# princeton-nlp/DensePhrases

Hardware: NVIDIA H100
Metric: queries/sec top-10 over PQ96 phrase index (higher is better)
Workload: dtype f32

## Files before the change

### densephrases_b200/_lib.py

```python
import ctypes as C
import os

_HERE = os.path.dirname(os.path.abspath(__file__))
LIB_PATH = os.path.join(_HERE, "lib", "libdph_b200.so")
_lib = None

MEM_HOST, MEM_DEVICE = 0, 1
SCAN_FAST, SCAN_EXACT, SCAN_PAIR, SCAN_SINGLE, SCAN_QUAD = 0, 1, 2, 3, 4

_vp, _i64, _i32, _u64, _f32 = C.c_void_p, C.c_int64, C.c_int, C.c_uint64, C.c_float
_SIGS = {
    "dph_last_error": (C.c_char_p, []),
    "dph_version": (_i32, []),
    "dph_index_create": (_i32, [C.POINTER(_vp), _i32, _i64, _i32, _i32, _i32]),
    "dph_index_free": (None, [_vp]),
    "dph_index_set_stream": (_i32, [_vp, _vp]),
    "dph_index_set_opq": (_i32, [_vp, _vp, _i32]),
    "dph_index_set_centroids": (_i32, [_vp, _vp, _i32]),
    "dph_index_set_pq": (_i32, [_vp, _vp, _i32]),
    "dph_index_gen_centroids": (_i32, [_vp, _u64, _f32]),
    "dph_index_gen_pq": (_i32, [_vp, _u64, _f32]),
    "dph_index_set_shard": (_i32, [_vp, _i64, _i64]),
    "dph_index_set_lists": (_i32, [_vp, _vp, _vp, _vp]),
    "dph_index_set_lists_synthetic": (_i32, [_vp, _vp, _u64]),
    "dph_index_ntotal": (_i64, [_vp]),
    "dph_index_ntotal_local": (_i64, [_vp]),
    "dph_index_d": (_i32, [_vp]),
    "dph_index_nlist": (_i64, [_vp]),
    "dph_index_nprobe": (_i32, [_vp]),
    "dph_index_set_nprobe": (_i32, [_vp, _i32]),
    "dph_index_set_scan_mode": (_i32, [_vp, _i32]),
    "dph_index_set_coarse_tc": (_i32, [_vp, _i32]),
    "dph_index_get_opq": (_i32, [_vp, _vp, _i32]),
    "dph_index_device_bytes": (_i64, [_vp]),
    "dph_index_set_profile": (_i32, [_vp, _i32]),
    "dph_index_last_scan_ms": (_i32, [_vp, C.POINTER(C.c_float)]),
    "dph_index_profile_scan_ms": (_i32, [_vp, _vp, _i32]),
    "dph_index_profile_count": (_i32, [_vp]),
    "dph_index_search": (_i32, [_vp, _vp, _i64, _i32, _vp, _vp, _i32]),
    "dph_index_search_partial": (_i32, [_vp, _vp, _i64, _i32, _vp, _vp, _vp]),
    "dph_index_coarse_local": (_i32, [_vp, _vp, _i64, _vp]),
    "dph_index_search_preassigned": (_i32, [_vp, _vp, _i32, _i64, _i32, _vp, _vp, _vp]),
    "dph_index_record_floats": (_i32, [_vp]),
    "dph_index_coarse_split": (_i32, [_vp, _vp, _i64, _vp]),
    "dph_index_search_assigned": (_i32, [_vp, _vp, _i64, _i32, _vp, _vp, _vp]),
    "dph_merge_shards": (_i32, [_vp, _vp, _vp, _i32, _i64, _i32, _vp, _vp, _vp]),
    "dph_pack_topk": (_i32, [_vp, _vp, _vp, _i64, _i32, _vp, _vp]),
    "dph_merge_shards_packed": (_i32, [_vp, _i32, _i64, _i32, _vp, _vp, _vp]),
    "dph_index_last_flags": (_vp, [_vp]),
    "dph_index_last_probes": (_vp, [_vp]),
    "dph_index_last_coarse": (_vp, [_vp]),
    "dph_index_last_xr": (_vp, [_vp]),
    "dph_index_last_used_pair_mode": (_i32, [_vp]),
    "dph_index_last_group_size": (_i32, [_vp]),
    "dph_index_copy_last": (_i32, [_vp, _i32, _vp, _i64]),
    "dph_index_reconstruct_batch": (_i32, [_vp, _vp, _i64, _vp, _vp, _i32]),
    "dph_encoder_create": (_i32, [C.POINTER(_vp), _i32, _i32, _i32, _i32]),
    "dph_encoder_free": (None, [_vp]),
    "dph_encoder_set_stream": (_i32, [_vp, _vp]),
    "dph_encoder_tower_floats": (_i64, [_vp]),
    "dph_encoder_load_tower": (_i32, [_vp, _i32, _vp, _i32]),
    "dph_encoder_embed_query": (_i32, [_vp, _vp, _vp, _vp, _i32, _i32, _vp, _vp, _i32]),
    "dph_sgemm_nt_seq": (_i32, [_vp, _i64, _vp, _i64, _i64, _vp, _vp]),
    "dph_gemm_tf32_nt": (_i32, [_vp, _vp, _vp, _vp, _vp, _i64, _i64, _i64, _i32, _i32, _vp]),
    "dph_encoder_set_precision": (_i32, [_vp, _i32]),
    "dph_gemm_tf32_set_mode": (_i32, [_i32]),
    "dph_set_tuning": (_i32, [_i32, _i32]),
    "dph_encoder_set_attention": (_i32, [_vp, _i32]),
    "dph_attention_bert": (_i32, [_vp, _vp, _i32, _i32, _vp, _i32, _vp]),
    "dph_index_window_scores": (_i32, [_vp, _vp, _vp, _i64, _i32, _vp, _i32]),
    "dph_index_encode": (_i32, [_vp, _vp, _i64, _vp, _vp, _i32]),
    "dph_index_add_with_ids": (_i32, [_vp, _vp, _i64, _vp, _i32]),
    "dph_index_copy_lists": (_i32, [_vp, _vp, _vp]),
    "dph_index_get_list_len": (_i32, [_vp, _vp]),
    "dph_index_last_add_ms": (_i32, [_vp, _vp]),
    "dph_index_remove_ids": (_i32, [_vp, _vp, _i64, _i64, _i64, _i32, _vp, _vp]),
    "dph_index_sync_list_len": (_i32, [_vp, _vp]),
    "dph_index_last_remove_ms": (_i32, [_vp, _vp]),
    "dph_index_last_remove_tmp_bytes": (_i64, [_vp]),
    "dph_index_train_coarse": (_i32, [_vp, _vp, _i64, _i32, _u64, _i64, _i32, _i32, _vp, _vp]),
    "dph_index_train_pq": (_i32, [_vp, _vp, _i64, _i32, _u64, _i64, _i32, _i32, _i32]),
    "dph_index_encode_pq": (_i32, [_vp, _vp, _i64, _vp, _i32]),
    "dph_index_get_centroids": (_i32, [_vp, _vp, _i32]),
    "dph_index_get_pq": (_i32, [_vp, _vp, _i32]),
    "dph_index_last_train_ms": (_i32, [_vp, _vp]),
}
EXPORTS = tuple(_SIGS)


def lib():
    global _lib
    if _lib is None:
        if not os.path.exists(LIB_PATH):
            raise RuntimeError(f"{LIB_PATH} not built: run `make` (or __graft_entry__.build()). There is no CPU fallback.")
        L = C.CDLL(LIB_PATH)
        for name, (res, args) in _SIGS.items():
            fn = getattr(L, name)
            fn.restype, fn.argtypes = res, args
        _lib = L
    return _lib


def check(rc):
    if rc != 0:
        raise RuntimeError("libdph_b200: " + lib().dph_last_error().decode())
```

### densephrases_b200/csrc/common.cuh

```cuda
#pragma once
#include <cuda_runtime.h>
#include <stdint.h>
#include <stdio.h>
#include <string>

#define DPH_D 768
#define DPH_M 96
#define DPH_KSUB 256
#define DPH_DSUB 8
#define DPH_CODE 96
#define DPH_BLK_VECS 32
#define DPH_BLK_BYTES 3072
#define DPH_NEUTRAL (-3.402823466e+38f)

#define DPH_API extern "C" __attribute__((visibility("default")))
void dph_set_error(const std::string& msg);

#define DPH_CUDA(call)                                                                              \
    do {                                                                                            \
        cudaError_t e__ = (call);                                                                   \
        if (e__ != cudaSuccess) {                                                                   \
            dph_set_error(std::string(#call) + ": " + cudaGetErrorString(e__) + " @" + __FILE__ + ":" + \
                          std::to_string(__LINE__));                                                \
            return 1;                                                                               \
        }                                                                                           \
    } while (0)
#define DPH_CHECK(cond, msg)                                                        \
    do {                                                                            \
        if (!(cond)) { dph_set_error(std::string(msg) + " (" #cond ")"); return 1; } \
    } while (0)
#define DPH_TRY(call)            \
    do {                         \
        int r__ = (call);        \
        if (r__) return r__;     \
    } while (0)

struct DphPerDeviceOnce {
    bool done[64] = {};
    bool first() {
        int d = 0;
        cudaGetDevice(&d);
        d &= 63;
        if (done[d]) return false;
        done[d] = true;
        return true;
    }
};

__device__ __forceinline__ float2 dph_ffma2(float2 a, float2 b, float2 c) { return make_float2(fmaf(a.x, b.x, c.x), fmaf(a.y, b.y, c.y)); }
__device__ __forceinline__ float2 dph_fadd2(float2 a, float2 b) { return make_float2(__fadd_rn(a.x, b.x), __fadd_rn(a.y, b.y)); }

__host__ __device__ __forceinline__ uint64_t dph_mix64(uint64_t x) {
    x += 0x9E3779B97F4A7C15ull;
    x = (x ^ (x >> 30)) * 0xBF58476D1CE4E5B9ull;
    x = (x ^ (x >> 27)) * 0x94D049BB133111EBull;
    return x ^ (x >> 31);
}
__host__ __device__ __forceinline__ uint64_t dph_rnd64(uint64_t seed, uint64_t stream, uint64_t a, uint64_t b) {
    return dph_mix64(dph_mix64(dph_mix64(seed ^ (stream * 0xA24BAED4963EE407ull)) + a) + b);
}
__host__ __device__ __forceinline__ float dph_approx_normal(uint64_t u, float sigma_over_std) {
    int32_t s = (int32_t)(u & 0xFFFF) + (int32_t)((u >> 16) & 0xFFFF) + (int32_t)((u >> 32) & 0xFFFF) + (int32_t)(u >> 48) - 131070;
    return (float)s * sigma_over_std;
}
#define DPH_IH4_STD 37837.227f
enum { DPH_STREAM_CODES = 1, DPH_STREAM_CENTROIDS = 2, DPH_STREAM_PQ = 3 };

__host__ __device__ __forceinline__ uint32_t dph_fkey(float f) {
    uint32_t b;
#ifdef __CUDA_ARCH__
    b = __float_as_uint(f);
#else
    memcpy(&b, &f, 4);
#endif
    return (b & 0x80000000u) ? ~b : (b | 0x80000000u);
}
__host__ __device__ __forceinline__ float dph_fkey_inv(uint32_t k) {
    uint32_t b = (k & 0x80000000u) ? (k & 0x7FFFFFFFu) : ~k;
#ifdef __CUDA_ARCH__
    return __uint_as_float(b);
#else
    float f; memcpy(&f, &b, 4); return f;
#endif
}
__host__ __device__ __forceinline__ uint64_t dph_ckey(float score, uint32_t gidx) {
    return ((uint64_t)dph_fkey(score) << 32) | (uint64_t)(0xFFFFFFFFu - gidx);
}
__host__ __device__ __forceinline__ float dph_ckey_score(uint64_t k) { return dph_fkey_inv((uint32_t)(k >> 32)); }
__host__ __device__ __forceinline__ uint32_t dph_ckey_gidx(uint64_t k) { return 0xFFFFFFFFu - (uint32_t)k; }

__host__ __device__ __forceinline__ int dph_blk_addr(int lane, int m) {
    int seg = m >> 5, s = ((m & 31) - lane) & 31;
    int t = seg * 32 + s;
    return (t >> 4) * 512 + lane * 16 + (t & 15);
}

struct __align__(16) DphSeg {
    long long blk;
    int len;
    unsigned gstart;
    float dis0;
    unsigned wrel;
    unsigned wend;
    int list;
};

struct DphWork {
    long long total_blocks;
};
struct DphPairWork {
    long long total_blocks;
    long long per;
    int total_units;
    int next_unit;
};
#define DPH_QUAD_ITEM_Q 8
struct __align__(16) DphUnit {
    long long blk;
    int len;
    unsigned bi0, bend;
    int nq;
    int list, pad;
    unsigned q[DPH_QUAD_ITEM_Q];
    unsigned gs[DPH_QUAD_ITEM_Q];
    float base[DPH_QUAD_ITEM_Q];
    float step[DPH_QUAD_ITEM_Q];
};
#define DPH_PAIR_SEG_MIN 128
#define DPH_PAIR_UNITS_PER_CTA 16
```

### densephrases_b200/csrc/index.cu

```cuda
#include "index_internal.cuh"
#include <algorithm>
#include <numeric>
#include <stdlib.h>
#include <string.h>
#include <thrust/device_ptr.h>
#include <thrust/execution_policy.h>
#include <thrust/sequence.h>
#include <thrust/sort.h>

static thread_local std::string g_err;
void dph_set_error(const std::string& msg) { g_err = msg; }
DPH_API const char* dph_last_error(void) { return g_err.c_str(); }
DPH_API int dph_version(void) { return 103; }
int g_dph_tune[8] = {1, 0, 0, 0, 0, 0, 0, 0};
DPH_API int dph_set_tuning(int knob, int value) {
    DPH_CHECK(knob >= 0 && knob < 8, "dph_set_tuning: unknown knob");
    g_dph_tune[knob] = value;
    return 0;
}

int DevBuf::ensure(size_t bytes) {
    if (bytes <= cap) return 0;
    if (p) cudaFree(p);
    p = nullptr; cap = 0;
    size_t want = bytes + bytes / 8 + 256;
    DPH_CUDA(cudaMalloc(&p, want));
    cap = want;
    return 0;
}
void DevBuf::release() { if (p) cudaFree(p); p = nullptr; cap = 0; }

template <class T> static int dev_alloc(T** out, size_t count, dph_index* ix) {
    if (*out) { cudaFree(*out); *out = nullptr; }
    size_t bytes = std::max<size_t>(count, 1) * sizeof(T);
    DPH_CUDA(cudaMalloc((void**)out, bytes));
    ix->bytes += (int64_t)bytes;
    return 0;
}

__global__ void gen_normal_kernel(float* out, long long rows, int cols, uint64_t seed, uint64_t stream, float sc) {
    long long i = (long long)blockIdx.x * blockDim.x + threadIdx.x;
    if (i >= rows * cols) return;
    long long r = i / cols; int t = (int)(i % cols);
    out[i] = dph_approx_normal(dph_rnd64(seed, stream, (uint64_t)r, (uint64_t)t), sc);
}

int64_t dph_chunk_rows() {
    int64_t chunk_rows = (256ll << 20) / DPH_CODE;
    if (const char* ev = getenv("DPH_UPLOAD_CHUNK_ROWS")) chunk_rows = std::max<int64_t>(1, atoll(ev));
    return chunk_rows;
}

__global__ void __launch_bounds__(192) fill_blocks_kernel(uint8_t* codes, long long nblocks, const long long* blk_off, const int* list_len,
                                                          long long list_lo, long long list_hi, const uint8_t* raw,
                                                          const long long* local_row_start, uint64_t seed, long long blk0, long long raw_row0) {
    const long long blk = blk0 + blockIdx.x;
    if (blk >= nblocks) return;
    const int lane = threadIdx.x & 31, c = threadIdx.x >> 5;
    __shared__ long long s_l;
    if (threadIdx.x == 0) s_l = list_of_block(blk_off, list_lo, list_hi, blk);
    __syncthreads();
    const long long l = s_l;
    const long long j = (blk - blk_off[l]) * 32 + lane;
    const bool valid = j < (long long)list_len[l];
    const int seg = c >> 1;
    unsigned char bytes[16];
    if (!valid) {
#pragma unroll
        for (int b = 0; b < 16; b++) bytes[b] = 0;
    } else if (raw) {
        const uint8_t* row = raw + (local_row_start[l - list_lo] + j - raw_row0) * DPH_CODE;
#pragma unroll
        for (int b = 0; b < 16; b++) { int t = c * 16 + b; int m = seg * 32 + ((lane + (t & 31)) & 31); bytes[b] = row[m]; }
    } else {
        uint64_t w[4];
#pragma unroll
        for (int i = 0; i < 4; i++) w[i] = dph_rnd64(seed, DPH_STREAM_CODES, (uint64_t)l, (uint64_t)(j * 12 + seg * 4 + i));
#pragma unroll
        for (int b = 0; b < 16; b++) {
            int t = c * 16 + b; int ml = (lane + (t & 31)) & 31;
            bytes[b] = (unsigned char)(w[ml >> 3] >> (8 * (ml & 7)));
        }
    }
    uint4 v;
    memcpy(&v, bytes, 16);
    *reinterpret_cast<uint4*>(codes + blk * DPH_BLK_BYTES + c * 512 + lane * 16) = v;
}

__global__ void fill_ids_kernel(long long* ids, long long nblocks, const long long* blk_off, const int* list_len, long long list_lo,
                                long long list_hi, const long long* raw_ids, const long long* local_row_start, long long blk0, long long raw_row0,
                                long long* dm_ids, long long* dm_rows) {
    const long long blk = blk0 + blockIdx.x;
    if (blk >= nblocks) return;
    const long long l = list_of_block(blk_off, list_lo, list_hi, blk);
    const long long j = (blk - blk_off[l]) * 32 + threadIdx.x;
    const bool real = j < (long long)list_len[l];
    const long long row = local_row_start[l - list_lo] + j;
    const long long id = real ? raw_ids[row - raw_row0] : -1;
    ids[blk * 32 + threadIdx.x] = id;
    if (real) { dm_ids[row] = id; dm_rows[row] = blk * 32 + threadIdx.x; }
}

DPH_API int dph_index_create(dph_index** out, int d, int64_t nlist, int M, int nbits, int device) {
    DPH_CHECK(out != nullptr, "null out");
    DPH_CHECK(d == DPH_D && M == DPH_M && nbits == 8, "only d=768, M=96, nbits=8 (OPQ96/PQ96 of build_phrase_index.py:113-116) is built");
    DPH_CHECK(nlist >= 1 && nlist < (1ll << 31), "bad nlist");
    DPH_CUDA(cudaSetDevice(device));
    dph_index* ix = new dph_index();
    ix->device = device; ix->nlist = nlist; ix->list_lo = 0; ix->list_hi = nlist;
    cudaDeviceProp prop;
    DPH_CUDA(cudaGetDeviceProperties(&prop, device));
    ix->num_sms = prop.multiProcessorCount;
    if (prop.major != 9 || prop.minor != 0) { delete ix; dph_set_error("libdph_b200 is built for sm_90a (H100) only; found sm_" + std::to_string(prop.major) + std::to_string(prop.minor)); return 1; }
    *out = ix;
    return 0;
}
DPH_API void dph_index_free(dph_index* ix) {
    if (!ix) return;
    cudaSetDevice(ix->device);
    void* ptrs[] = {ix->A, ix->C, ix->pq, ix->list_len, ix->list_start, ix->blk_off, ix->codes, ix->ids, ix->dm_ids, ix->dm_rows};
    for (void* p : ptrs) if (p) cudaFree(p);
    DevBuf* bufs[] = {&ix->xdev, &ix->xr, &ix->S, &ix->key, &ix->cd, &ix->lut_canon, &ix->lutmax, &ix->segs, &ix->wpre, &ix->qinfo,
                      &ix->cand, &ix->cand_off, &ix->cand_cnt, &ix->gthr, &ix->flags, &ix->work, &ix->Dp, &ix->Ip, &ix->Gp, &ix->Dh, &ix->Ih, &ix->eps, &ix->nseg, &ix->lutmin, &ix->lutmaxv, &ix->lutq, &ix->qparams, &ix->gdense,
                      &ix->pl_cnt, &ix->pl_fill, &ix->pl_off, &ix->pl_blockpre, &ix->pl_entries, &ix->pl_unitpre, &ix->pl_units, &ix->pl_udesc, &ix->pairwork, &ix->csplit, &ix->xsplit, &ix->candkeys, &ix->cflags, &ix->selkeys, &ix->recbuf,
                      &ix->rb_ids, &ix->rb_out, &ix->rb_found, &ix->ws_q, &ix->ws_id, &ix->ws_out, &ix->ws_xq, &ix->enc_key, &ix->enc_cd,
                      &ix->enc_list, &ix->enc_codes};
    for (DevBuf* b : bufs) b->release();
    for (int i = 0; i < DPH_PROF_RING; i++) { if (ix->ev0[i]) cudaEventDestroy(ix->ev0[i]); if (ix->ev1[i]) cudaEventDestroy(ix->ev1[i]); }
    for (cudaEvent_t e : ix->aev) if (e) cudaEventDestroy(e);
    delete ix;
}
DPH_API int dph_index_set_stream(dph_index* ix, void* s) { ix->stream = (cudaStream_t)s; return 0; }

static int upload(float** dst, const float* src, size_t count, int mem, dph_index* ix) {
    DPH_CUDA(cudaSetDevice(ix->device));
    DPH_TRY(dev_alloc(dst, count, ix));
    DPH_CUDA(cudaMemcpyAsync(*dst, src, count * sizeof(float), mem == DPH_MEM_HOST ? cudaMemcpyHostToDevice : cudaMemcpyDeviceToDevice, ix->stream));
    DPH_CUDA(cudaStreamSynchronize(ix->stream));
    return 0;
}
DPH_API int dph_index_set_opq(dph_index* ix, const float* A, int mem) { return upload(&ix->A, A, (size_t)ix->d * ix->d, mem, ix); }
DPH_API int dph_index_set_centroids(dph_index* ix, const float* C, int mem) { ix->csplit_lo = -1; return upload(&ix->C, C, (size_t)ix->nlist * ix->d, mem, ix); }
DPH_API int dph_index_set_pq(dph_index* ix, const float* pq, int mem) { return upload(&ix->pq, pq, (size_t)DPH_M * 256 * DPH_DSUB, mem, ix); }

DPH_API int dph_index_gen_centroids(dph_index* ix, uint64_t seed, float sigma) {
    DPH_CUDA(cudaSetDevice(ix->device));
    ix->csplit_lo = -1;
    DPH_TRY(dev_alloc(&ix->C, (size_t)ix->nlist * ix->d, ix));
    long long tot = (long long)ix->nlist * ix->d;
    gen_normal_kernel<<<(unsigned)((tot + 255) / 256), 256, 0, ix->stream>>>(ix->C, ix->nlist, ix->d, seed, DPH_STREAM_CENTROIDS, sigma / DPH_IH4_STD);
    DPH_CUDA(cudaGetLastError());
    return 0;
}
DPH_API int dph_index_gen_pq(dph_index* ix, uint64_t seed, float sigma) {
    DPH_CUDA(cudaSetDevice(ix->device));
    DPH_TRY(dev_alloc(&ix->pq, (size_t)DPH_M * 256 * DPH_DSUB, ix));
    long long rows = DPH_M * 256;
    gen_normal_kernel<<<(unsigned)((rows * DPH_DSUB + 255) / 256), 256, 0, ix->stream>>>(ix->pq, rows, DPH_DSUB, seed, DPH_STREAM_PQ, sigma / DPH_IH4_STD);
    DPH_CUDA(cudaGetLastError());
    return 0;
}
DPH_API int dph_index_set_shard(dph_index* ix, int64_t lo, int64_t hi) {
    DPH_CHECK(0 <= lo && lo <= hi && hi <= ix->nlist, "bad shard range");
    DPH_CHECK(ix->codes == nullptr, "set_shard must precede set_lists");
    ix->list_lo = lo; ix->list_hi = hi;
    return 0;
}

static int set_lists_common(dph_index* ix, const int64_t* list_len, const uint8_t* codes, const int64_t* ids, bool synthetic, uint64_t seed) {
    DPH_CUDA(cudaSetDevice(ix->device));
    const int64_t nlist = ix->nlist, lo = ix->list_lo, hi = ix->list_hi;
    ix->h_list_len.assign(list_len, list_len + nlist);
    ix->h_list_start.assign(nlist + 1, 0);
    for (int64_t l = 0; l < nlist; l++) {
        DPH_CHECK(list_len[l] >= 0 && list_len[l] < (1ll << 31), "bad list length");
        ix->h_list_start[l + 1] = ix->h_list_start[l] + list_len[l];
    }
    ix->ntotal = ix->h_list_start[nlist];
    std::vector<int32_t> len32(nlist);
    std::vector<int64_t> blk_off(nlist, -1), local_row_start(std::max<int64_t>(hi - lo, 1), 0);
    int64_t nb = 0, rows = 0;
    for (int64_t l = 0; l < nlist; l++) len32[l] = (int32_t)list_len[l];
    for (int64_t l = lo; l < hi; l++) {
        blk_off[l] = nb; local_row_start[l - lo] = rows;
        nb += (list_len[l] + 31) / 32; rows += list_len[l];
    }
    ix->nblocks_local = nb; ix->ntotal_local = rows; ix->blk_cap = -1;
    DPH_TRY(dev_alloc(&ix->list_len, (size_t)nlist, ix));
    DPH_TRY(dev_alloc(&ix->list_start, (size_t)nlist + 1, ix));
    DPH_TRY(dev_alloc(&ix->blk_off, (size_t)nlist, ix));
    DPH_CUDA(cudaMemcpy(ix->list_len, len32.data(), nlist * 4, cudaMemcpyHostToDevice));
    DPH_CUDA(cudaMemcpy(ix->list_start, ix->h_list_start.data(), (nlist + 1) * 8, cudaMemcpyHostToDevice));
    DPH_CUDA(cudaMemcpy(ix->blk_off, blk_off.data(), nlist * 8, cudaMemcpyHostToDevice));
    DPH_TRY(dev_alloc(&ix->codes, (size_t)nb * DPH_BLK_BYTES, ix));
    if (nb == 0) return 0;
    int64_t* d_lrs = nullptr;
    DPH_CUDA(cudaMalloc((void**)&d_lrs, local_row_start.size() * 8));
    DPH_CUDA(cudaMemcpy(d_lrs, local_row_start.data(), local_row_start.size() * 8, cudaMemcpyHostToDevice));
    if (synthetic) {
        for (int64_t b0 = 0; b0 < nb; b0 += (1ll << 30)) {
            const unsigned g = (unsigned)std::min<int64_t>(nb - b0, 1ll << 30);
            fill_blocks_kernel<<<g, 192, 0, ix->stream>>>(ix->codes, std::min<int64_t>(nb, b0 + g), (const long long*)ix->blk_off, ix->list_len, lo, hi, nullptr,
                                                         (const long long*)d_lrs, seed, b0, 0);
        }
        DPH_CUDA(cudaGetLastError());
    } else {
        DPH_CHECK(codes != nullptr, "codes is null");
        const int64_t chunk_rows = dph_chunk_rows();
        auto chunk_end = [&](int64_t l0, int64_t& acc) {
            int64_t l1 = l0;
            acc = 0;
            while (l1 < hi && (acc == 0 || acc + list_len[l1] <= chunk_rows)) { acc += list_len[l1]; l1++; }
            return l1;
        };
        int64_t max_rows = 0;
        for (int64_t l0 = lo, acc = 0; l0 < hi;) { const int64_t l1 = chunk_end(l0, acc); max_rows = std::max(max_rows, acc); l0 = l1; }
        uint8_t* d_raw = nullptr; int64_t* d_rawids = nullptr;
        DPH_CUDA(cudaMalloc((void**)&d_raw, std::max<size_t>((size_t)max_rows * DPH_CODE, 1)));
        if (ids) {
            DPH_CUDA(cudaMalloc((void**)&d_rawids, std::max<size_t>((size_t)max_rows * 8, 8)));
            DPH_TRY(dev_alloc(&ix->ids, (size_t)nb * 32, ix));
            DPH_TRY(dev_alloc(&ix->dm_ids, (size_t)rows, ix));
            DPH_TRY(dev_alloc(&ix->dm_rows, (size_t)rows, ix));
        }
        int64_t l0 = lo;
        while (l0 < hi) {
            int64_t acc = 0;
            const int64_t l1 = chunk_end(l0, acc);
            const int64_t r0 = local_row_start[l0 - lo];
            const int64_t b0 = blk_off[l0], b1 = (l1 < hi) ? blk_off[l1] : nb;
            if (acc > 0 && b1 > b0) {
                DPH_CUDA(cudaMemcpyAsync(d_raw, codes + (size_t)r0 * DPH_CODE, (size_t)acc * DPH_CODE, cudaMemcpyHostToDevice, ix->stream));
                fill_blocks_kernel<<<(unsigned)(b1 - b0), 192, 0, ix->stream>>>(ix->codes, b1, (const long long*)ix->blk_off, ix->list_len, lo, hi, d_raw,
                                                                                 (const long long*)d_lrs, 0, b0, r0);
                if (ids) {
                    DPH_CUDA(cudaMemcpyAsync(d_rawids, ids + r0, (size_t)acc * 8, cudaMemcpyHostToDevice, ix->stream));
                    fill_ids_kernel<<<(unsigned)(b1 - b0), 32, 0, ix->stream>>>((long long*)ix->ids, b1, (const long long*)ix->blk_off, ix->list_len, lo, hi,
                                                                                 (const long long*)d_rawids, (const long long*)d_lrs, b0, r0,
                                                                                 (long long*)ix->dm_ids, (long long*)ix->dm_rows);
                }
                DPH_CUDA(cudaGetLastError());
                DPH_CUDA(cudaStreamSynchronize(ix->stream));
            }
            l0 = l1;
        }
        cudaFree(d_raw);
        if (d_rawids) cudaFree(d_rawids);
        if (ids) {
            thrust::device_ptr<long long> kp((long long*)ix->dm_ids), vp((long long*)ix->dm_rows);
            thrust::sort_by_key(thrust::cuda::par.on(ix->stream), kp, kp + rows, vp);
            ix->dm_n = rows;
        }
    }
    DPH_CUDA(cudaStreamSynchronize(ix->stream));
    cudaFree(d_lrs);
    return 0;
}
DPH_API int dph_index_set_lists(dph_index* ix, const int64_t* list_len, const uint8_t* codes, const int64_t* ids) {
    return set_lists_common(ix, list_len, codes, ids, false, 0);
}
DPH_API int dph_index_set_lists_synthetic(dph_index* ix, const int64_t* list_len, uint64_t seed) {
    return set_lists_common(ix, list_len, nullptr, nullptr, true, seed);
}

static int check_ready(dph_index* ix, int k);

__global__ void iota_kernel(long long* out, long long n, long long base) {
    const long long i = (long long)blockIdx.x * blockDim.x + threadIdx.x;
    if (i < n) out[i] = base + i;
}
__global__ void add_validate_kernel(const long long* list_no, const long long* ids, long long n, int* flag, int* cnt) {
    const long long i = (long long)blockIdx.x * blockDim.x + threadIdx.x;
    if (i >= n) return;
    const long long l = list_no[i];
    if (l < 0) atomicOr(flag, 4);
    else atomicAdd(&cnt[l], 1);
    if (ids[i] < 0) atomicOr(flag, 2);
}

__global__ void __launch_bounds__(192) relayout_codes_kernel(uint8_t* dst, long long blk0, const long long* boff_new, const long long* boff_old,
                                                             const int* len_old, long long lo, long long hi, const uint8_t* codes_old) {
    const long long blk = blk0 + blockIdx.x;
// ... 121 lines not shown
    const bool prof = ix->profile && ix->aev[0];
    if (prof) DPH_CUDA(cudaEventRecord(ix->aev[4], st));
    const long long *bo_new = (const long long*)d_boff_new, *bo_old = (const long long*)ix->blk_off;
    if (nb > 0) {
        relayout_codes_kernel<<<(unsigned)nb, 192, 0, st>>>(codes_new, 0, bo_new, bo_old, ix->list_len, lo, hi, ix->codes);
        relayout_ids_kernel<<<(unsigned)nb, 32, 0, st>>>((long long*)ids_new, 0, bo_new, bo_old, ix->list_len, lo, hi, (const long long*)ix->ids,
                                                       (const long long*)ix->list_start, (const long long*)d_lrs, (long long*)dm_ids_new,
                                                       (long long*)dm_rows_new);
    }
    if (was_explicit && ix->dm_n > 0)
        remap_dm_kernel<<<(unsigned)((ix->dm_n + 255) / 256), 256, 0, st>>>((const long long*)ix->dm_ids, (const long long*)ix->dm_rows, ix->dm_n,
                                                                           bo_old, bo_new, lo, hi, (long long*)dm_ids_new, (long long*)dm_rows_new);
    DPH_CUDA(cudaGetLastError());
    try {
        thrust::device_ptr<long long> kp((long long*)list_all), pp((long long*)perm);
        thrust::sequence(thrust::cuda::par.on(st), pp, pp + n);
        thrust::stable_sort_by_key(thrust::cuda::par.on(st), kp, kp + n, pp);
        add_scatter_kernel<<<(unsigned)((n + 127) / 128), 128, 0, st>>>(n, (const long long*)list_all, (const long long*)perm, (const long long*)d_bstart,
                                                                       ix->list_len, bo_new, lo, hi, codes_all, (const long long*)ids_all, codes_new,
                                                                       (long long*)ids_new, (long long*)dm_ids_new, (long long*)dm_rows_new, dm_old);
        DPH_CUDA(cudaGetLastError());
        thrust::device_ptr<long long> dk((long long*)dm_ids_new), dv((long long*)dm_rows_new);
        thrust::stable_sort_by_key(thrust::cuda::par.on(st), dk, dk + dm_cap, dv);
    } catch (const std::exception& e) {
        cudaGetLastError();
        dph_set_error(std::string("add_with_ids: device sort failed; the index is unchanged: ") + e.what());
        return 1;
    }
    if (prof) DPH_CUDA(cudaEventRecord(ix->aev[5], st));
    DPH_CUDA(cudaStreamSynchronize(st));

    DPH_CUDA(cudaMemcpy(ix->blk_off, d_boff_new, nlist * 8, cudaMemcpyDeviceToDevice));
    DPH_CUDA(cudaMemcpy(ix->list_len, len32.data(), nlist * 4, cudaMemcpyHostToDevice));
    DPH_CUDA(cudaMemcpy(ix->list_start, start_new.data(), (nlist + 1) * 8, cudaMemcpyHostToDevice));
    const int64_t nb_old = ix->blk_cap < 0 ? ix->nblocks_local : ix->blk_cap;
    int64_t old_bytes = std::max<int64_t>(nb_old * DPH_BLK_BYTES, 1);
    if (ix->ids) old_bytes += std::max<int64_t>(nb_old * 32, 1) * 8;
    if (ix->dm_ids) old_bytes += 2 * std::max<int64_t>(ix->dm_cap < 0 ? ix->ntotal_local : ix->dm_cap, 1) * 8;
    const int64_t new_bytes = std::max<int64_t>(nb * DPH_BLK_BYTES, 1) + std::max<int64_t>(nb * 32, 1) * 8 + 2 * std::max<int64_t>(dm_cap, 1) * 8;
    void* olds[] = {ix->codes, ix->ids, ix->dm_ids, ix->dm_rows};
    for (void* p : olds) if (p) cudaFree(p);
    ix->codes = codes_new; ix->ids = ids_new; ix->dm_ids = dm_ids_new; ix->dm_rows = dm_rows_new;
    for (void* p : {(void*)codes_new, (void*)ids_new, (void*)dm_ids_new, (void*)dm_rows_new}) tmp.release(p);
    ix->bytes += new_bytes - old_bytes;
    ix->dm_n = dm_old + in_shard; ix->dm_cap = dm_cap;
    ix->h_list_len = len_new; ix->h_list_start = start_new;
    ix->ntotal = start_new[nlist]; ix->ntotal_local = rows; ix->nblocks_local = nb; ix->blk_cap = -1;
    if (prof) DPH_CUDA(cudaEventElapsedTime(&ix->add_ms[3], ix->aev[4], ix->aev[5]));
    return 0;
}

__global__ void __launch_bounds__(192) read_blocks_kernel(const uint8_t* codes, long long nblocks, const long long* blk_off, const int* list_len,
                                                          long long list_lo, long long list_hi, const long long* ids, const long long* list_start,
                                                          const long long* local_row_start, long long blk0, long long raw_row0, uint8_t* raw,
                                                          long long* raw_ids) {
    const long long blk = blk0 + blockIdx.x;
    if (blk >= nblocks) return;
    const int lane = threadIdx.x & 31, c = threadIdx.x >> 5;
    __shared__ long long s_l;
    if (threadIdx.x == 0) s_l = list_of_block(blk_off, list_lo, list_hi, blk);
    __syncthreads();
    const long long l = s_l;
    const long long j = (blk - blk_off[l]) * 32 + lane;
    if (j >= (long long)list_len[l]) return;
    const long long row = local_row_start[l - list_lo] + j - raw_row0;
    const uint4 v = *reinterpret_cast<const uint4*>(codes + blk * DPH_BLK_BYTES + c * 512 + lane * 16);
    unsigned char bytes[16];
    memcpy(bytes, &v, 16);
    const int seg = c >> 1;
#pragma unroll
    for (int b = 0; b < 16; b++) { const int t = c * 16 + b; raw[row * DPH_CODE + seg * 32 + ((lane + (t & 31)) & 31)] = bytes[b]; }
    if (c == 0 && raw_ids) raw_ids[row] = ids ? ids[blk * 32 + lane] : list_start[l] + j;
}

DPH_API int dph_index_copy_lists(dph_index* ix, uint8_t* codes_out, int64_t* ids_out) {
    DPH_CHECK(ix && ix->list_len, "copy_lists: lists are not set");
    DPH_CUDA(cudaSetDevice(ix->device));
    const int64_t lo = ix->list_lo, hi = ix->list_hi;
    const std::vector<int64_t>& len = ix->h_list_len;
    if (ix->ntotal_local == 0) return 0;
    std::vector<int64_t> boff(hi - lo), lrs(hi - lo);
    for (int64_t l = lo, nb = 0, rows = 0; l < hi; l++) { boff[l - lo] = nb; lrs[l - lo] = rows; nb += (len[l] + 31) / 32; rows += len[l]; }
    const int64_t chunk_rows = dph_chunk_rows();
    auto chunk_end = [&](int64_t l0, int64_t& acc) {
        int64_t l1 = l0;
        acc = 0;
        while (l1 < hi && (acc == 0 || acc + len[l1] <= chunk_rows)) { acc += len[l1]; l1++; }
        return l1;
    };
    int64_t max_rows = 0;
    for (int64_t l0 = lo, acc = 0; l0 < hi;) { const int64_t l1 = chunk_end(l0, acc); max_rows = std::max(max_rows, acc); l0 = l1; }
    DevTmp tmp;
    uint8_t* d_raw; int64_t *d_ids, *d_lrs;
    DPH_TRY(tmp.alloc(&d_raw, (size_t)max_rows * DPH_CODE, "copy_lists: staging"));
    DPH_TRY(tmp.alloc(&d_ids, (size_t)max_rows, "copy_lists: staging"));
    DPH_TRY(tmp.alloc(&d_lrs, lrs.size(), "copy_lists: staging"));
    DPH_CUDA(cudaMemcpyAsync(d_lrs, lrs.data(), lrs.size() * 8, cudaMemcpyHostToDevice, ix->stream));
    for (int64_t l0 = lo; l0 < hi;) {
        int64_t acc = 0;
        const int64_t l1 = chunk_end(l0, acc);
        const int64_t r0 = lrs[l0 - lo], b0 = boff[l0 - lo], b1 = l1 < hi ? boff[l1 - lo] : ix->nblocks_local;
        if (acc > 0 && b1 > b0) {
            read_blocks_kernel<<<(unsigned)(b1 - b0), 192, 0, ix->stream>>>(ix->codes, b1, (const long long*)ix->blk_off, ix->list_len, lo, hi,
                                                                           (const long long*)ix->ids, (const long long*)ix->list_start,
                                                                           (const long long*)d_lrs, b0, r0, d_raw, ids_out ? (long long*)d_ids : nullptr);
            DPH_CUDA(cudaGetLastError());
            DPH_CUDA(cudaMemcpyAsync(codes_out + (size_t)r0 * DPH_CODE, d_raw, (size_t)acc * DPH_CODE, cudaMemcpyDeviceToHost, ix->stream));
            if (ids_out) DPH_CUDA(cudaMemcpyAsync(ids_out + r0, d_ids, (size_t)acc * 8, cudaMemcpyDeviceToHost, ix->stream));
            DPH_CUDA(cudaStreamSynchronize(ix->stream));
        }
        l0 = l1;
    }
    return 0;
}

DPH_API int dph_index_get_list_len(const dph_index* ix, int64_t* list_len_out) {
    DPH_CHECK(ix && ix->list_len, "lists are not set");
    std::copy(ix->h_list_len.begin(), ix->h_list_len.end(), list_len_out);
    return 0;
}
DPH_API int dph_index_last_add_ms(const dph_index* ix, float* ms_out) {
    DPH_CHECK(ix->aev[0] != nullptr, "profiling was never enabled");
    std::copy(ix->add_ms, ix->add_ms + 4, ms_out);
    return 0;
}

DPH_API int64_t dph_index_ntotal(const dph_index* ix) { return ix->ntotal; }
DPH_API int64_t dph_index_ntotal_local(const dph_index* ix) { return ix->ntotal_local; }
DPH_API int dph_index_d(const dph_index* ix) { return ix->d; }
DPH_API int64_t dph_index_nlist(const dph_index* ix) { return ix->nlist; }
DPH_API int dph_index_nprobe(const dph_index* ix) { return ix->nprobe; }
DPH_API int dph_index_set_nprobe(dph_index* ix, int nprobe) {
    DPH_CHECK(nprobe >= 1 && nprobe <= DPH_MAX_NPROBE, "nprobe must be in [1,1024]");
    ix->nprobe = nprobe;
    return 0;
}
DPH_API int dph_index_set_coarse_tc(dph_index* ix, int on) { ix->coarse_tc = on ? 1 : 0; return 0; }
DPH_API int dph_index_set_scan_mode(dph_index* ix, int mode) {
    DPH_CHECK(mode >= 0 && mode <= 4, "bad scan mode");
    ix->scan_mode = mode;
    return 0;
}
DPH_API int dph_index_get_opq(const dph_index* ix, float* A_out, int mem) {
    DPH_CHECK(ix->A != nullptr, "OPQ matrix not set");
    DPH_CUDA(cudaMemcpy(A_out, ix->A, (size_t)ix->d * ix->d * 4, mem == DPH_MEM_HOST ? cudaMemcpyDeviceToHost : cudaMemcpyDeviceToDevice));
    return 0;
}
DPH_API int dph_index_set_profile(dph_index* ix, int on) {
    DPH_CUDA(cudaSetDevice(ix->device));
    if (on && !ix->ev0[0])
        for (int i = 0; i < DPH_PROF_RING; i++) { DPH_CUDA(cudaEventCreate(&ix->ev0[i])); DPH_CUDA(cudaEventCreate(&ix->ev1[i])); }
    if (on && !ix->aev[0])
        for (cudaEvent_t& e : ix->aev) DPH_CUDA(cudaEventCreate(&e));
    ix->profile = on != 0;
    ix->prof_n = 0;
    return 0;
}
DPH_API int dph_index_last_scan_ms(dph_index* ix, float* ms) {
    DPH_CHECK(ix->ev0[0] && ix->prof_n > 0, "no profiled search");
    int i = (int)((ix->prof_n - 1) % DPH_PROF_RING);
    DPH_CUDA(cudaEventSynchronize(ix->ev1[i]));
    DPH_CUDA(cudaEventElapsedTime(ms, ix->ev0[i], ix->ev1[i]));
    return 0;
}
DPH_API int dph_index_profile_scan_ms(dph_index* ix, float* ms_out, int max_out) {
    DPH_CHECK(ix->ev0[0] != nullptr, "profiling was never enabled");
    int n = (int)std::min<int64_t>(std::min<int64_t>(ix->prof_n, DPH_PROF_RING), max_out);
    for (int j = 0; j < n; j++) {
        int i = (int)((ix->prof_n - n + j) % DPH_PROF_RING);
        DPH_CUDA(cudaEventSynchronize(ix->ev1[i]));
        DPH_CUDA(cudaEventElapsedTime(ms_out + j, ix->ev0[i], ix->ev1[i]));
    }
    return n < 0 ? 0 : 0 * n;
}
DPH_API int dph_index_profile_count(const dph_index* ix) { return (int)std::min<int64_t>(ix->prof_n, DPH_PROF_RING); }
DPH_API int64_t dph_index_device_bytes(const dph_index* ix) { return ix->bytes; }
DPH_API const int32_t* dph_index_last_flags(const dph_index* ix) { return ix->flags.as<int32_t>(); }
DPH_API const int32_t* dph_index_last_probes(const dph_index* ix) { return ix->key.as<int32_t>(); }
DPH_API const float* dph_index_last_coarse(const dph_index* ix) { return ix->cd.as<float>(); }
DPH_API const float* dph_index_last_xr(const dph_index* ix) { return ix->xr.as<float>(); }
DPH_API int dph_index_last_used_pair_mode(const dph_index* ix) { return ix->last_group > 1 ? 1 : 0; }
DPH_API int dph_index_last_group_size(const dph_index* ix) { return ix->last_group; }
DPH_API int dph_index_copy_last(dph_index* ix, int which, void* dst_host, int64_t bytes) {
    const void* src = which == 0 ? ix->flags.p : which == 1 ? ix->key.p : which == 2 ? ix->cd.p : which == 3 ? ix->xr.p : nullptr;
    DPH_CHECK(src != nullptr, "copy_last: nothing to copy");
    DPH_CUDA(cudaStreamSynchronize(ix->stream));
    DPH_CUDA(cudaMemcpy(dst_host, src, (size_t)bytes, cudaMemcpyDeviceToHost));
    return 0;
}

static int search_chunk(dph_index* ix, const float* x_dev, int64_t n, int k, float* D, int64_t* I, uint32_t* G, int stage = 0,
                        unsigned long long* keys64 = nullptr) {
    cudaStream_t st = ix->stream;
    const int nprobe = ix->nprobe;
    const int grid = ix->num_sms;
    const int keep_single = k + DPH_KEEP_SLACK;
    const int keep_pair = k + (k / 2 > DPH_KEEP_SLACK ? k / 2 : DPH_KEEP_SLACK);
    const int keep_quad = k + (2 * k > 100 ? 2 * k : 100);
    const int keep_max = keep_quad > keep_pair ? keep_quad : keep_pair;
    DPH_TRY(ix->xr.ensure((size_t)n * ix->d * 4));
    DPH_TRY(ix->S.ensure((size_t)n * ix->nlist * 4));
    DPH_TRY(ix->key.ensure((size_t)n * nprobe * 4));
    DPH_TRY(ix->cd.ensure((size_t)n * nprobe * 4));
    DPH_TRY(ix->lut_canon.ensure((size_t)n * DPH_LUT_CANON_FLOATS * 4));
    DPH_TRY(ix->lutmax.ensure((size_t)n * DPH_M * 4));
    DPH_TRY(ix->segs.ensure((size_t)n * nprobe * sizeof(DphSeg)));
    DPH_TRY(ix->wpre.ensure((size_t)(n + 1) * 8));
    DPH_TRY(ix->qinfo.ensure((size_t)n * 4));
    DPH_TRY(ix->eps.ensure((size_t)n * 4));
    DPH_TRY(ix->nseg.ensure((size_t)n * 4));
    const int64_t eff_probe = std::min<int64_t>(nprobe, ix->nlist);
    const int64_t nl_local = std::max<int64_t>(ix->list_hi - ix->list_lo, 1);
    const bool long_lists = ix->ntotal_local / nl_local >= 4096;
    const bool shared = long_lists && n * eff_probe * 2 >= ix->nlist * 3;
    int group = 1;
    if (ix->scan_mode == DPH_SCAN_PAIR) group = 2;
    else if (ix->scan_mode == DPH_SCAN_QUAD) group = 4;
    else if (ix->scan_mode == DPH_SCAN_FAST && shared) group = 4;
    if (group == 4 && keep_quad > DPH_QUAD_KEEP_MAX) group = 2;
    if (group == 2 && keep_pair > 1536 - DPH_SCAN_THREADS) group = 1;
    const bool pair = group > 1;
    const int keep_fast = group == 4 ? keep_quad : (group == 2 ? keep_pair : keep_single);
    const size_t item_q = group == 4 ? DPH_QUAD_ITEM_Q : 2;
    DPH_TRY(ix->cand.ensure(((size_t)(2 * grid + 2 * n + 2) + (pair ? (size_t)(n * nprobe + item_q * DPH_PAIR_UNITS_PER_CTA * grid + 2 * n + 16) : 0)) * keep_max * 8));
    DPH_TRY(ix->cand_off.ensure((size_t)(n + 1) * 8));
    DPH_TRY(ix->cand_cnt.ensure((size_t)n * 4));
    DPH_TRY(ix->gthr.ensure((size_t)n * 4));
    DPH_TRY(ix->flags.ensure((size_t)n * 4));
    DPH_TRY(ix->work.ensure(sizeof(DphWork)));
    DPH_TRY(ix->lutmin.ensure((size_t)n * DPH_M * 4));
    DPH_TRY(ix->lutmaxv.ensure((size_t)n * DPH_M * 4));
    if (pair) {
        DPH_TRY(ix->lutq.ensure((size_t)n * DPH_LUT_SCAN_FLOATS * 2));
        DPH_TRY(ix->qparams.ensure((size_t)n * 8));
        DPH_TRY(ix->gdense.ensure((size_t)n * nprobe * 4));
        DPH_TRY(ix->pl_cnt.ensure((size_t)ix->nlist * 4));
        DPH_TRY(ix->pl_fill.ensure((size_t)ix->nlist * 4));
        DPH_TRY(ix->pl_off.ensure((size_t)(ix->nlist + 1) * 4));
        DPH_TRY(ix->pl_blockpre.ensure((size_t)(ix->nlist + 1) * 8));
        DPH_TRY(ix->pl_entries.ensure((size_t)n * nprobe * 4));
        DPH_TRY(ix->pl_unitpre.ensure((size_t)(ix->nlist + 1) * 4));
        DPH_TRY(ix->pl_units.ensure((size_t)(n * nprobe + DPH_PAIR_UNITS_PER_CTA * grid + 16) * 8));
        if (group == 4) DPH_TRY(ix->pl_udesc.ensure((size_t)(n * nprobe + DPH_PAIR_UNITS_PER_CTA * grid + 16) * sizeof(DphUnit)));
        DPH_TRY(ix->pairwork.ensure(sizeof(DphPairWork)));
    }
    ix->last_n = n;
    if (stage != 1 && stage != 3) ix->last_group = group;
    if (stage == 1) ix->last_coarse_n = n;

    if (stage == 1) {
        const int64_t nl = ix->list_hi - ix->list_lo;
        DPH_TRY(dph_launch_sgemm_nt_seq(x_dev, n, ix->A, ix->d, ix->d, ix->xr.as<float>(), st));
        if (ix->coarse_tc) {
            int rc = dph_coarse_tc(ix, n, ix->list_lo, nl, nprobe, keys64, nullptr, nullptr, st);
            if (rc == 0) return 0;
            if (rc != 1) return rc;
        }
        DPH_TRY(dph_launch_sgemm_nt_seq(ix->xr.as<float>(), n, ix->C + ix->list_lo * ix->d, nl, ix->d, ix->S.as<float>(), st));
        DPH_TRY(dph_launch_coarse_select(ix->S.as<float>(), n, nl, nprobe, nullptr, nullptr, st, keys64, (unsigned)ix->list_lo));
        return 0;
    }
    if (stage == 0 || stage == 3) {
        DPH_TRY(dph_launch_sgemm_nt_seq(x_dev, n, ix->A, ix->d, ix->d, ix->xr.as<float>(), st));
        int rc = ix->coarse_tc ? dph_coarse_tc(ix, n, 0, ix->nlist, nprobe, nullptr, ix->key.as<int32_t>(), ix->cd.as<float>(), st) : 1;
        if (rc > 1) return rc;
        if (rc == 1) {
            DPH_TRY(dph_launch_sgemm_nt_seq(ix->xr.as<float>(), n, ix->C, ix->nlist, ix->d, ix->S.as<float>(), st));
            DPH_TRY(dph_launch_coarse_select(ix->S.as<float>(), n, ix->nlist, nprobe, ix->key.as<int32_t>(), ix->cd.as<float>(), st, nullptr, 0u, nullptr, 0,
                                             &ix->selkeys));
        }
        if (stage == 3) return 0;
    }
    DPH_TRY(dph_launch_lut(ix->xr.as<float>(), n, ix->pq, ix->lut_canon.as<float>(), ix->lutmax.as<float>(),
                           ix->lutmin.as<float>(), ix->lutmaxv.as<float>(), pair ? ix->lutq.p : nullptr,
                           pair ? ix->qparams.as<float2>() : nullptr, st, group));
    if (ix->scan_mode != DPH_SCAN_EXACT) {
        DPH_TRY(dph_launch_plan(ix, n, k, keep_fast, grid, nullptr, st, group));
        if (ix->profile) DPH_CUDA(cudaEventRecord(ix->ev0[ix->prof_n % DPH_PROF_RING], st));
        if (pair) DPH_TRY(dph_launch_scan_pair(ix, n, keep_fast, grid, st, group));
        else DPH_TRY(dph_launch_scan(ix, n, k, keep_fast, DPH_SCAN_FAST, grid, st));
        if (ix->profile) { DPH_CUDA(cudaEventRecord(ix->ev1[ix->prof_n % DPH_PROF_RING], st)); ix->prof_n++; }
        DPH_TRY(dph_launch_merge(ix, n, k, DPH_SCAN_FAST, nullptr, D, I, G, st));
        DPH_TRY(dph_launch_plan(ix, n, k, k, grid, ix->flags.as<int32_t>(), st, 1));
        DPH_TRY(dph_launch_scan(ix, n, k, k, DPH_SCAN_EXACT, grid, st));
        DPH_TRY(dph_launch_merge(ix, n, k, DPH_SCAN_EXACT, ix->flags.as<int32_t>(), D, I, G, st));
    } else {
        DPH_CUDA(cudaMemsetAsync(ix->flags.p, 0, (size_t)n * 4, st));
        DPH_TRY(dph_launch_plan(ix, n, k, k, grid, nullptr, st, 1));
        if (ix->profile) DPH_CUDA(cudaEventRecord(ix->ev0[ix->prof_n % DPH_PROF_RING], st));
        DPH_TRY(dph_launch_scan(ix, n, k, k, DPH_SCAN_EXACT, grid, st));
        if (ix->profile) { DPH_CUDA(cudaEventRecord(ix->ev1[ix->prof_n % DPH_PROF_RING], st)); ix->prof_n++; }
        DPH_TRY(dph_launch_merge(ix, n, k, DPH_SCAN_EXACT, nullptr, D, I, G, st));
    }
    return 0;
}

static int check_ready(dph_index* ix, int k) {
    DPH_CHECK(ix && ix->A && ix->C && ix->pq && ix->list_len, "index is not fully constructed (opq/centroids/pq/lists)");
    DPH_CHECK(k >= 1 && k <= DPH_MAX_K, "k must be in [1,1024]");
    return 0;
}
static int64_t chunk_size(const dph_index* ix, int64_t n) {
    int64_t c = (1ll << 28) / std::max<int64_t>(ix->nlist, 1);
    c = std::max<int64_t>(1, std::min<int64_t>(c, 4096));
    return std::min(c, n);
}

DPH_API int dph_index_search_partial(dph_index* ix, const float* x_dev, int64_t n, int k, float* D, int64_t* I, uint32_t* G) {
    DPH_TRY(check_ready(ix, k));
    DPH_CUDA(cudaSetDevice(ix->device));
    const int64_t cs = chunk_size(ix, n);
    for (int64_t o = 0; o < n; o += cs) {
        int64_t m = std::min(cs, n - o);
        DPH_TRY(search_chunk(ix, x_dev + o * ix->d, m, k, D + o * k, I + o * k, G + o * k));
    }
    return 0;
}

DPH_API int dph_index_coarse_local(dph_index* ix, const float* x_dev, int64_t n, uint64_t* keys_dev) {
    DPH_TRY(check_ready(ix, 1));
    DPH_CUDA(cudaSetDevice(ix->device));
    DPH_CHECK(n <= chunk_size(ix, n), "coarse_local: batch too large for one chunk");
    return search_chunk(ix, x_dev, n, 1, nullptr, nullptr, nullptr, 1, (unsigned long long*)keys_dev);
}
DPH_API int dph_index_search_preassigned(dph_index* ix, const uint64_t* keys_gathered_dev, int nshards, int64_t n, int k, float* D_dev,
                                         int64_t* I_dev, uint32_t* G_dev) {
    DPH_TRY(check_ready(ix, k));
    DPH_CUDA(cudaSetDevice(ix->device));
    DPH_CHECK(n == ix->last_coarse_n, "search_preassigned must follow coarse_local with the same batch");
    DPH_TRY(ix->key.ensure((size_t)n * ix->nprobe * 4));
    DPH_TRY(ix->cd.ensure((size_t)n * ix->nprobe * 4));
    DPH_TRY(dph_launch_coarse_merge((const unsigned long long*)keys_gathered_dev, nshards, n, ix->nprobe, ix->key.as<int32_t>(), ix->cd.as<float>(),
                                    ix->stream));
    return search_chunk(ix, nullptr, n, k, D_dev, I_dev, G_dev, 2, nullptr);
}

__global__ void pack_records_kernel(const float* __restrict__ xr, const int* __restrict__ key, const float* __restrict__ cd, int nprobe, float* __restrict__ rec) {
    const long long q = blockIdx.x;
    const int R = DPH_D + 2 * nprobe;
    float* o = rec + q * R;
    for (int t = threadIdx.x; t < R; t += blockDim.x)
        o[t] = t < DPH_D ? xr[q * DPH_D + t] : (t < DPH_D + nprobe ? __int_as_float(key[q * nprobe + t - DPH_D]) : cd[q * nprobe + t - DPH_D - nprobe]);
}
__global__ void unpack_records_kernel(const float* __restrict__ rec, int nprobe, float* __restrict__ xr, int* __restrict__ key, float* __restrict__ cd) {
    const long long q = blockIdx.x;
    const int R = DPH_D + 2 * nprobe;
    const float* r = rec + q * R;
    for (int t = threadIdx.x; t < R; t += blockDim.x) {
        const float v = r[t];
        if (t < DPH_D) xr[q * DPH_D + t] = v;
        else if (t < DPH_D + nprobe) key[q * nprobe + t - DPH_D] = __float_as_int(v);
        else cd[q * nprobe + t - DPH_D - nprobe] = v;
    }
}
DPH_API int dph_index_record_floats(const dph_index* ix) { return ix->d + 2 * ix->nprobe; }
DPH_API int dph_index_coarse_split(dph_index* ix, const float* x_dev, int64_t n_local, float* rec_dev) {
    DPH_TRY(check_ready(ix, 1));
    DPH_CUDA(cudaSetDevice(ix->device));
    if (n_local == 0) return 0;
    DPH_CHECK(n_local <= chunk_size(ix, n_local), "coarse_split: slice too large for one chunk");
    DPH_TRY(search_chunk(ix, x_dev, n_local, 1, nullptr, nullptr, nullptr, 3, nullptr));
    pack_records_kernel<<<(unsigned)n_local, 256, 0, ix->stream>>>(ix->xr.as<float>(), ix->key.as<int>(), ix->cd.as<float>(), ix->nprobe, rec_dev);
    DPH_CUDA(cudaGetLastError());
    return 0;
}
DPH_API int dph_index_search_assigned(dph_index* ix, const float* rec_dev, int64_t n, int k, float* D_dev, int64_t* I_dev, uint32_t* G_dev) {
    DPH_TRY(check_ready(ix, k));
    DPH_CUDA(cudaSetDevice(ix->device));
    if (n == 0) return 0;
    DPH_TRY(ix->xr.ensure((size_t)n * ix->d * 4));
    DPH_TRY(ix->key.ensure((size_t)n * ix->nprobe * 4));
    DPH_TRY(ix->cd.ensure((size_t)n * ix->nprobe * 4));
    unpack_records_kernel<<<(unsigned)n, 256, 0, ix->stream>>>(rec_dev, ix->nprobe, ix->xr.as<float>(), ix->key.as<int>(), ix->cd.as<float>());
    DPH_CUDA(cudaGetLastError());
    return search_chunk(ix, nullptr, n, k, D_dev, I_dev, G_dev, 2, nullptr);
}

DPH_API int dph_index_search(dph_index* ix, const float* x, int64_t n, int k, float* D, int64_t* I, int mem) {
    DPH_TRY(check_ready(ix, k));
    DPH_CUDA(cudaSetDevice(ix->device));
    if (n == 0) return 0;
    DPH_TRY(ix->Gp.ensure((size_t)n * k * 4));
    if (mem == DPH_MEM_DEVICE) return dph_index_search_partial(ix, x, n, k, D, I, ix->Gp.as<uint32_t>());
    DPH_TRY(ix->xdev.ensure((size_t)n * ix->d * 4));
    DPH_TRY(ix->Dp.ensure((size_t)n * k * 4));
    DPH_TRY(ix->Ip.ensure((size_t)n * k * 8));
    DPH_CUDA(cudaMemcpyAsync(ix->xdev.p, x, (size_t)n * ix->d * 4, cudaMemcpyHostToDevice, ix->stream));
    DPH_TRY(dph_index_search_partial(ix, ix->xdev.as<float>(), n, k, ix->Dp.as<float>(), ix->Ip.as<int64_t>(), ix->Gp.as<uint32_t>()));
    DPH_CUDA(cudaMemcpyAsync(D, ix->Dp.p, (size_t)n * k * 4, cudaMemcpyDeviceToHost, ix->stream));
    DPH_CUDA(cudaMemcpyAsync(I, ix->Ip.p, (size_t)n * k * 8, cudaMemcpyDeviceToHost, ix->stream));
    DPH_CUDA(cudaStreamSynchronize(ix->stream));
    return 0;
}

struct LocateArgs {
    const long long* list_start; long long nlist; long long list_lo, list_hi; const long long* blk_off; const int* list_len;
    const long long* dm_ids; const long long* dm_rows; long long dm_n; bool explicit_ids;
};
__device__ __forceinline__ bool locate_label(const LocateArgs& a, long long id, long long& l, long long& prow) {
    if (!a.explicit_ids) {
        if (id < 0 || id >= a.list_start[a.nlist]) return false;
        long long lo = 0, hi = a.nlist;
        while (hi - lo > 1) { long long mid = (lo + hi) >> 1; if (a.list_start[mid] <= id) lo = mid; else hi = mid; }
        l = lo;
        if (l < a.list_lo || l >= a.list_hi) return false;
        long long j = id - a.list_start[l];
        prow = (a.blk_off[l] + (j >> 5)) * 32 + (j & 31);
        return true;
    }
    long long lo = 0, hi = a.dm_n;
    if (hi == 0) return false;
    while (hi - lo > 1) { long long mid = (lo + hi) >> 1; if (a.dm_ids[mid] <= id) lo = mid; else hi = mid; }
    if (a.dm_ids[lo] != id) return false;
    prow = a.dm_rows[lo];
    l = list_of_block(a.blk_off, a.list_lo, a.list_hi, prow >> 5);
    return true;
}

__global__ void __launch_bounds__(96) reconstruct_kernel(LocateArgs la, const long long* ids, long long m, const uint8_t* codes, const float* C,
                                                          const float* pq, float* out, unsigned char* found) {
    const long long i = blockIdx.x;
    const int t = threadIdx.x;
    __shared__ long long s_l, s_prow; __shared__ int s_ok;
    if (t == 0) { long long l = 0, pr = 0; s_ok = locate_label(la, ids[i], l, pr) ? 1 : 0; s_l = l; s_prow = pr; }
    __syncthreads();
    float4* o = reinterpret_cast<float4*>(out + i * DPH_D + t * 8);
    if (!s_ok) { o[0] = make_float4(0, 0, 0, 0); o[1] = make_float4(0, 0, 0, 0); if (t == 0 && found) found[i] = 0; return; }
    const long long blk = s_prow >> 5; const int lane = (int)(s_prow & 31);
    const unsigned char code = codes[blk * DPH_BLK_BYTES + dph_blk_addr(lane, t)];
    const float4* cb = reinterpret_cast<const float4*>(pq + ((size_t)t * 256 + code) * 8);
    const float4* ce = reinterpret_cast<const float4*>(C + s_l * DPH_D + t * 8);
    float4 a0 = cb[0], a1 = cb[1], c0 = ce[0], c1 = ce[1];
    o[0] = make_float4(a0.x + c0.x, a0.y + c0.y, a0.z + c0.z, a0.w + c0.w);
    o[1] = make_float4(a1.x + c1.x, a1.y + c1.y, a1.z + c1.z, a1.w + c1.w);
    if (t == 0 && found) found[i] = 1;
}

static LocateArgs make_locate(const dph_index* ix) {
// ... 80 lines not shown
```

### densephrases_b200/csrc/index_internal.cuh

```cuda
#pragma once
#include "common.cuh"
#include "../../include/dph_b200.h"
#include <algorithm>
#include <string.h>
#include <vector>

#define DPH_SCAN_THREADS 512
#define DPH_SCAN_WARPS (DPH_SCAN_THREADS / 32)
#define DPH_CAND_CAP 3072
#define DPH_PAIR_CAP 1280
#define DPH_QUAD_KEEP_MAX 256

#define DPH_KEEP_SLACK 32
#define DPH_MAX_K 1024
#define DPH_PROF_RING 64
#define DPH_MAX_NPROBE 1024
#define DPH_SURV_CAP 2048
#define DPH_LUT_SCAN_FLOATS (3 * 256 * 64)
#define DPH_LUT_CANON_FLOATS (96 * 256)
#define DPH_LUTC_IDX(m, code) ((((m) >> 5) << 13) + ((code) << 5) + ((m) & 31))
#define DPH_SEG_SMEM 256
#define DPH_L2_PREFETCH_ROUNDS 2

struct DevBuf {
    void* p = nullptr;
    size_t cap = 0;
    int ensure(size_t bytes);
    void release();
    template <class T> T* as() const { return (T*)p; }
};

struct dph_index {
    int device = 0;
    int d = DPH_D, M = DPH_M;
    int64_t nlist = 0;
    int nprobe = 256;
    int scan_mode = DPH_SCAN_FAST;
    cudaStream_t stream = 0;
    int num_sms = 132;

    float* A = nullptr;
    float* C = nullptr;
    float* pq = nullptr;
    int64_t list_lo = 0, list_hi = 0;
    int64_t ntotal = 0, ntotal_local = 0, nblocks_local = 0;
    int32_t* list_len = nullptr;
    int64_t* list_start = nullptr;
    int64_t* blk_off = nullptr;
    uint8_t* codes = nullptr;
    int64_t* ids = nullptr;
    int64_t* dm_ids = nullptr;
    int64_t* dm_rows = nullptr;
    int64_t dm_n = 0;
    int64_t dm_cap = -1;
    std::vector<int64_t> h_list_len;
    std::vector<int64_t> h_list_start;
    int64_t bytes = 0;

    DevBuf xdev, xr, S, key, cd, lut_canon, lutmax, segs, wpre, qinfo, cand, cand_off, cand_cnt, gthr, flags,
        work, Dp, Ip, Gp, Dh, Ih, eps, nseg,
        lutmin, lutmaxv, lutq, qparams, gdense, pl_cnt, pl_fill, pl_off, pl_blockpre, pl_entries, pl_unitpre, pl_units, pl_udesc, pairwork,
        csplit, xsplit, candkeys, cflags, selkeys, recbuf,
        rb_ids, rb_out, rb_found, ws_q, ws_id, ws_out, ws_xq,
        enc_key, enc_cd, enc_list, enc_codes;
    int64_t csplit_lo = -1, csplit_nl = -1;
    int coarse_tc = 1;
    int64_t last_n = 0;
    int last_group = 1;
    int64_t last_coarse_n = -1;
    bool profile = false;
    cudaEvent_t ev0[DPH_PROF_RING] = {}, ev1[DPH_PROF_RING] = {};
    int64_t prof_n = 0;
    cudaEvent_t aev[6] = {};
    float add_ms[4] = {};
    float remove_ms[3] = {};
    float train_ms[3] = {};
    int64_t remove_tmp_peak = 0;
    int64_t blk_cap = -1;
};

__device__ __forceinline__ long long list_of_block(const long long* blk_off, long long lo, long long hi, long long blk) {
    while (hi - lo > 1) { long long mid = (lo + hi) >> 1; if (blk_off[mid] <= blk) lo = mid; else hi = mid; }
    return lo;
}
__device__ __forceinline__ void dph_store_row(uint8_t* codes, long long blk, int lane, const unsigned char* row) {
#pragma unroll
    for (int c = 0; c < 6; c++) {
        unsigned char bytes[16];
        const int seg = c >> 1;
#pragma unroll
        for (int b = 0; b < 16; b++) { const int t = c * 16 + b; bytes[b] = row[seg * 32 + ((lane + (t & 31)) & 31)]; }
        uint4 v;
        memcpy(&v, bytes, 16);
        *reinterpret_cast<uint4*>(codes + blk * DPH_BLK_BYTES + c * 512 + lane * 16) = v;
    }
}
__device__ __forceinline__ void dph_load_row(const uint8_t* codes, long long blk, int lane, unsigned char* row) {
#pragma unroll
    for (int c = 0; c < 6; c++) {
        const uint4 v = *reinterpret_cast<const uint4*>(codes + blk * DPH_BLK_BYTES + c * 512 + lane * 16);
        unsigned char bytes[16];
        memcpy(bytes, &v, 16);
        const int seg = c >> 1;
#pragma unroll
        for (int b = 0; b < 16; b++) { const int t = c * 16 + b; row[seg * 32 + ((lane + (t & 31)) & 31)] = bytes[b]; }
    }
}

struct DevTmp {
    std::vector<void*> ps;
    int64_t live = 0, peak = 0;
    ~DevTmp() { for (void* p : ps) if (p) cudaFree(p); }
    template <class T> int alloc(T** out, size_t count, const char* what) {
        const size_t bytes = std::max<size_t>(count, 1) * sizeof(T);
        cudaError_t e = cudaMalloc((void**)out, bytes);
        if (e != cudaSuccess) {
            cudaGetLastError();
            *out = nullptr;
            dph_set_error(std::string(what) + ": " + cudaGetErrorString(e));
            return 1;
        }
        ps.push_back(*out);
        live += (int64_t)bytes; peak = std::max(peak, live);
        return 0;
    }
    void release(void* p) { for (void*& q : ps) if (q == p) q = nullptr; }
};

int64_t dph_chunk_rows();
__global__ void relayout_codes_kernel(uint8_t* dst, long long blk0, const long long* boff_new, const long long* boff_old, const int* len_old,
                                      long long lo, long long hi, const uint8_t* codes_old);
__global__ void relayout_ids_kernel(long long* dst, long long blk0, const long long* boff_new, const long long* boff_old, const int* len_old,
                                    long long lo, long long hi, const long long* ids_old, const long long* list_start_old,
                                    const long long* lrs_old, long long* dm_ids, long long* dm_rows);

extern int g_dph_tune[8];
int dph_launch_sgemm_nt_seq(const float* X, int64_t n, const float* W, int64_t m, int K, float* out, cudaStream_t st);
int dph_launch_coarse_select(const float* S, int64_t n, int64_t nlist, int nprobe, int32_t* key, float* cd, cudaStream_t st,
                             unsigned long long* keys64 = nullptr, unsigned list_base = 0, const int* only_rows = nullptr, int64_t ld = 0,
                             DevBuf* tmp = nullptr);
int dph_coarse_tc(dph_index* ix, int64_t n, int64_t lo, int64_t nl, int nprobe, unsigned long long* keys64, int32_t* key, float* cd, cudaStream_t st,
                  const float* xr = nullptr, const float* C = nullptr);
int dph_launch_coarse_merge(const unsigned long long* keys, int W, int64_t n, int nprobe, int32_t* key, float* cd, cudaStream_t st,
                            unsigned long long* keys64 = nullptr);
int dph_launch_lut(const float* xr, int64_t n, const float* pq, float* lut_canon, float* lutmax, float* lutmin, float* lutmaxv,
                   void* lutq, float2* qparams, cudaStream_t st, int group);
int dph_launch_plan(dph_index* ix, int64_t n, int k, int keep, int grid, const int32_t* only_flagged, cudaStream_t st, int group);
int dph_launch_scan_pair(dph_index* ix, int64_t n, int keep, int grid, cudaStream_t st, int group);
int dph_launch_scan(dph_index* ix, int64_t n, int k, int keep, int mode, int grid, cudaStream_t st);
int dph_launch_merge(dph_index* ix, int64_t n, int k, int mode, const int32_t* only_flagged, float* D, int64_t* I,
                     uint32_t* G, cudaStream_t st);
int dph_scan_setup_attrs();
int64_t dph_encode_chunk(const dph_index* ix);
int dph_encode_rows(dph_index* ix, const float* x_dev, int64_t n, int64_t* list_out, uint8_t* codes_out, int* bad);
int dph_coarse_top1(dph_index* ix, const float* xr, const float* C, int64_t n, int32_t* key, float* cd, cudaStream_t st);
int dph_pq_assign(dph_index* ix, const float* xr, const float* C, const int32_t* key, const float* pq, int64_t n, int64_t* list_out,
                  uint8_t* codes_out, cudaStream_t st);
__global__ void nonfinite_kernel(const float* __restrict__ x, long long count, int* __restrict__ bad);
```

### densephrases_b200/csrc/prep.cu

```cuda
#include "index_internal.cuh"
#include "select.cuh"

#define GBM 128
#define GBN 128
#define GBK 8
__global__ void __launch_bounds__(256) sgemm_nt_seq_kernel(const float* __restrict__ X, long long n, const float* __restrict__ W,
                                                            long long m, int K, float* __restrict__ out) {
    __shared__ __align__(16) float As[2][GBK][GBM];
    __shared__ __align__(16) float Bs[2][GBK][GBN];
    const int tid = threadIdx.x;
    const long long row0 = (long long)blockIdx.y * GBM, col0 = (long long)blockIdx.x * GBN;
    const int lr = tid & 127, lk4 = tid >> 7;
    const long long arow = row0 + lr, brow = col0 + lr;
    const bool aok = arow < n, bok = brow < m;
    const float4* ap = reinterpret_cast<const float4*>(X + (aok ? arow : 0) * K) + lk4;
    const float4* bp = reinterpret_cast<const float4*>(W + (bok ? brow : 0) * K) + lk4;
    const int tx = tid & 15, ty = tid >> 4;
    float2 acc[8][4];
#pragma unroll
    for (int i = 0; i < 8; i++)
#pragma unroll
        for (int j = 0; j < 4; j++) acc[i][j] = make_float2(0.0f, 0.0f);
    const float4 z4 = make_float4(0.f, 0.f, 0.f, 0.f);
    float4 ra = aok ? __ldg(ap) : z4, rb = bok ? __ldg(bp) : z4;
// ... 441 lines not shown
        return 0;
    }
    const int chunk_len = 8192;
    const int64_t nchunks = (nlist + chunk_len - 1) / chunk_len;
    if (tmp && !only_rows && nchunks * nprobe <= 8192 && nprobe <= chunk_len) {
        DPH_TRY(tmp->ensure((size_t)nchunks * n * nprobe * 8));
        const size_t smem = (size_t)chunk_len * 4 + CS_BINS * 4 + DPH_MAX_NPROBE * 8;
        static DphPerDeviceOnce once2;
        if (once2.first()) { DPH_CUDA(cudaFuncSetAttribute(coarse_select_smem_kernel, cudaFuncAttributeMaxDynamicSharedMemorySize, CS_MAX_ROW * 4 + CS_BINS * 4 + DPH_MAX_NPROBE * 8)); }
        coarse_select_smem_kernel<<<dim3((unsigned)n, (unsigned)nchunks), 256, smem, st>>>(S, (int)nlist, nprobe, nullptr, nullptr, tmp->as<unsigned long long>(),
                                                                                       list_base, nullptr, ld, chunk_len);
        DPH_CUDA(cudaGetLastError());
        return dph_launch_coarse_merge(tmp->as<unsigned long long>(), (int)nchunks, n, nprobe, key, cd, st, keys64);
    }
    coarse_select_kernel<<<(unsigned)n, 256, 0, st>>>(S, nlist, nprobe, key, cd, keys64, list_base, only_rows, ld);
    DPH_CUDA(cudaGetLastError());
    return 0;
}

#define LUT_TILE_LD 257
template <int LQ, int MS>
__global__ void __launch_bounds__(256) lut_kernel(const float* __restrict__ xr, const float* __restrict__ pq, long long n,
                                                   float* __restrict__ lut_canon,
                                                   float* __restrict__ lutmax, float* __restrict__ lutmin, float* __restrict__ lutmaxv) {
    extern __shared__ __align__(16) float lut_sm[];
    float* __restrict__ tile = lut_sm;
    __shared__ __align__(16) float xs[LQ * MS * 8];
    const long long q0 = (long long)blockIdx.x * LQ;
    const int m0 = blockIdx.y * MS, j = threadIdx.x, lane = j & 31, warp = j >> 5;
    const int nq = (int)((n - q0) < LQ ? (n - q0) : LQ);
    for (int i = j; i < LQ * MS * 8; i += 256) { const int qi = i / (MS * 8); xs[i] = qi < nq ? xr[(q0 + qi) * DPH_D + m0 * 8 + (i % (MS * 8))] : 0.0f; }
    __syncthreads();
    float4 c0[8], c1[8];
#pragma unroll
    for (int u = 0; u < 8; u++) {
        const float4* cb = reinterpret_cast<const float4*>(pq + ((size_t)(m0 + u) * 256 + j) * 8);
        c0[u] = __ldg(cb); c1[u] = __ldg(cb + 1);
    }
#pragma unroll 1
    for (int ml0 = 0; ml0 < MS; ml0 += 8) {
        float4 n0[8], n1[8];
        if (ml0 + 8 < MS) {
#pragma unroll
            for (int u = 0; u < 8; u++) {
                const float4* cb = reinterpret_cast<const float4*>(pq + ((size_t)(m0 + ml0 + 8 + u) * 256 + j) * 8);
                n0[u] = __ldg(cb); n1[u] = __ldg(cb + 1);
            }
        }
#pragma unroll
        for (int u = 0; u < 8; u++) {
            const int ml = ml0 + u;
#pragma unroll
            for (int qi = 0; qi < LQ; qi++) {
                const float4 x0 = *reinterpret_cast<const float4*>(xs + (qi * MS + ml) * 8);
                const float4 x1 = *reinterpret_cast<const float4*>(xs + (qi * MS + ml) * 8 + 4);
                float acc = 0.0f;
                acc = fmaf(x0.x, c0[u].x, acc); acc = fmaf(x0.y, c0[u].y, acc); acc = fmaf(x0.z, c0[u].z, acc); acc = fmaf(x0.w, c0[u].w, acc);
                acc = fmaf(x1.x, c1[u].x, acc); acc = fmaf(x1.y, c1[u].y, acc); acc = fmaf(x1.z, c1[u].z, acc); acc = fmaf(x1.w, c1[u].w, acc);
                tile[(qi * MS + ml) * LUT_TILE_LD + j] = acc;
            }
        }
#pragma unroll
        for (int u = 0; u < 8; u++) { c0[u] = n0[u]; c1[u] = n1[u]; }
    }
    __syncthreads();
    for (int p = warp; p < nq * MS; p += 8) {
        const float* row = tile + p * LUT_TILE_LD;
        float a = 0.0f, lo = row[lane], hi = lo;
#pragma unroll
        for (int e = 0; e < 8; e++) { const float v = row[lane + 32 * e]; a = fmaxf(a, fabsf(v)); lo = fminf(lo, v); hi = fmaxf(hi, v); }
#pragma unroll
        for (int off = 16; off > 0; off >>= 1) {
            a = fmaxf(a, __shfl_xor_sync(0xffffffffu, a, off));
            lo = fminf(lo, __shfl_xor_sync(0xffffffffu, lo, off));
            hi = fmaxf(hi, __shfl_xor_sync(0xffffffffu, hi, off));
        }
        if (lane == 0) {
            const long long o = (q0 + p / MS) * DPH_M + m0 + (p % MS);
            lutmax[o] = a; lutmin[o] = lo; lutmaxv[o] = hi;
        }
    }
    const int seg = m0 >> 5, mo = m0 & 31;
    for (int qi = 0; qi < nq; qi++) {
        float* dst = lut_canon + (size_t)(q0 + qi) * DPH_LUT_CANON_FLOATS + (size_t)seg * (256 * 32) + mo;
        const float* t = tile + qi * MS * LUT_TILE_LD;
        for (int idx = j; idx < 256 * MS; idx += 256) dst[(idx / MS) * 32 + (idx % MS)] = t[(idx % MS) * LUT_TILE_LD + (idx / MS)];
    }
}

#define DPH_QMAX 682
#define DPH_QMAX8 255
template <class T, int QMAX>
__global__ void __launch_bounds__(256) lutq_kernel(const float* __restrict__ lut_canon, const float* __restrict__ lutmin,
                                                    const float* __restrict__ lutmaxv, T* __restrict__ lutq,
                                                    float2* __restrict__ qparams) {
    __shared__ float tile[256 * 33];
    __shared__ float s_min[32];
    __shared__ float s_step, s_base;
    const long long q = blockIdx.x;
    const int seg = blockIdx.y, j = threadIdx.x, lane = j & 31;
    if (j < 32) {
        float r = 0.f, b = 0.f;
        for (int m = lane; m < DPH_M; m += 32) { r = fmaxf(r, lutmaxv[q * DPH_M + m] - lutmin[q * DPH_M + m]); b += lutmin[q * DPH_M + m]; }
#pragma unroll
        for (int off = 16; off > 0; off >>= 1) { r = fmaxf(r, __shfl_xor_sync(0xffffffffu, r, off)); b += __shfl_xor_sync(0xffffffffu, b, off); }
        if (lane == 0) { s_step = fmaxf(r / (float)QMAX, 1e-30f); s_base = b; }
        s_min[lane] = lutmin[q * DPH_M + seg * 32 + lane];
    }
    const float* src = lut_canon + (size_t)q * DPH_LUT_CANON_FLOATS + (size_t)seg * (256 * 32);
    for (int idx = j; idx < 256 * 32; idx += 256) tile[(idx >> 5) * 33 + (idx & 31)] = __ldg(src + idx);
    __syncthreads();
    const float inv = 1.0f / s_step;
    T* dst = lutq + ((size_t)q * 3 + seg) * (256 * 64);
    for (int idx = j; idx < 256 * 64; idx += 256) {
        const int row = idx >> 6, w = idx & 63, ml = w & 31;
        int qv = (int)((tile[row * 33 + ml] - s_min[ml]) * inv + 0.5f);
        qv = qv < 0 ? 0 : (qv > QMAX ? QMAX : qv);
        dst[idx] = (w < 63) ? (T)qv : (T)0;
    }
    if (seg == 0 && j == 0) qparams[q] = make_float2(s_step, s_base);
}

int dph_launch_lut(const float* xr, int64_t n, const float* pq, float* lut_canon, float* lutmax, float* lutmin, float* lutmaxv,
                   void* lutq, float2* qparams, cudaStream_t st, int group) {
    if (n == 0) return 0;
    static DphPerDeviceOnce lut_once;
    constexpr int lut_smem = 4 * 32 * LUT_TILE_LD * 4;
    if (lut_once.first()) {
        DPH_CUDA(cudaFuncSetAttribute(lut_kernel<4, 32>, cudaFuncAttributeMaxDynamicSharedMemorySize, lut_smem));
        DPH_CUDA(cudaFuncSetAttribute(lut_kernel<8, 16>, cudaFuncAttributeMaxDynamicSharedMemorySize, lut_smem));
    }
    const int lv = g_dph_tune[2];
    if (lv == 2) lut_kernel<8, 16><<<dim3((unsigned)((n + 7) / 8), 6), 256, lut_smem, st>>>(xr, pq, n, lut_canon, lutmax, lutmin, lutmaxv);
    else lut_kernel<4, 32><<<dim3((unsigned)((n + 3) / 4), 3), 256, lut_smem, st>>>(xr, pq, n, lut_canon, lutmax, lutmin, lutmaxv);
    DPH_CUDA(cudaGetLastError());
    if (lutq) {
        if (group == 4) lutq_kernel<unsigned char, DPH_QMAX8><<<dim3((unsigned)n, 3), 256, 0, st>>>(lut_canon, lutmin, lutmaxv, (unsigned char*)lutq, qparams);
        else lutq_kernel<unsigned short, DPH_QMAX><<<dim3((unsigned)n, 3), 256, 0, st>>>(lut_canon, lutmin, lutmaxv, (unsigned short*)lutq, qparams);
        DPH_CUDA(cudaGetLastError());
    }
    return 0;
}

struct PlanArgs {
    const int* key; const float* cd; const int* list_len; const long long* blk_off;
    long long list_lo, list_hi; int nprobe; long long n;
    const int* only_flagged;
    const float* lutmax;
    DphSeg* segs; unsigned* qblocks; int* nseg; float* eps;
    unsigned* gdense;
    const float2* qparams;
};
__global__ void __launch_bounds__(256) plan_segs_kernel(PlanArgs a) {
    const int lane = threadIdx.x & 31;
    const long long q = (long long)blockIdx.x * 8 + (threadIdx.x >> 5);
    if (q >= a.n) return;
    const bool active = a.only_flagged ? (a.only_flagged[q] != 0) : true;
    if (!active) {
        if (lane == 0) { a.qblocks[q] = 0u; a.nseg[q] = 0; }
        return;
    }
    unsigned gacc = 0, wacc = 0;
    int sacc = 0;
    float dmax = 0.0f;
    for (int r0 = 0; r0 < a.nprobe; r0 += 32) {
        const int r = r0 + lane;
        int l = -1, len = 0; float d0 = 0.0f; unsigned nb = 0; long long blk = -1;
        if (r < a.nprobe) {
            l = a.key[q * a.nprobe + r];
            d0 = a.cd[q * a.nprobe + r];
            if (l >= 0) {
                len = a.list_len[l];
                dmax = fmaxf(dmax, fabsf(d0));
                if (active && len > 0 && l >= a.list_lo && l < a.list_hi) { nb = (unsigned)((len + 31) >> 5); blk = a.blk_off[l]; }
            }
        }
        unsigned gl = (unsigned)len, wl = nb;
#pragma unroll
        for (int off = 1; off < 32; off <<= 1) {
            unsigned g2 = __shfl_up_sync(0xffffffffu, gl, off), w2 = __shfl_up_sync(0xffffffffu, wl, off);
            if (lane >= off) { gl += g2; wl += w2; }
        }
        if (a.gdense && r < a.nprobe) a.gdense[q * a.nprobe + r] = gacc + gl - (unsigned)len;
        const unsigned have = __ballot_sync(0xffffffffu, nb > 0);
        if (nb > 0) {
            DphSeg s;
            s.blk = blk; s.len = len; s.gstart = gacc + gl - (unsigned)len; s.dis0 = d0;
            s.wrel = wacc + wl - nb; s.wend = wacc + wl; s.list = l;
            a.segs[q * a.nprobe + sacc + __popc(have & ((1u << lane) - 1u))] = s;
        }
        sacc += __popc(have);
        gacc += __shfl_sync(0xffffffffu, gl, 31);
        wacc += __shfl_sync(0xffffffffu, wl, 31);
    }
#pragma unroll
    for (int off = 16; off > 0; off >>= 1) dmax = fmaxf(dmax, __shfl_xor_sync(0xffffffffu, dmax, off));
    float lsum = 0.0f;
    for (int m = lane; m < DPH_M; m += 32) lsum += a.lutmax[q * DPH_M + m];
#pragma unroll
    for (int off = 16; off > 0; off >>= 1) lsum += __shfl_xor_sync(0xffffffffu, lsum, off);
    if (lane == 0) {
        a.qblocks[q] = wacc;
        a.nseg[q] = sacc;
        const float gamma96 = 5.7221e-6f;
        float e = 2.0f * gamma96 * (dmax + lsum) * 1.01f;
        if (a.qparams) e += 96.0f * 0.502f * a.qparams[q].x + 8e-6f * (dmax + lsum);
        a.eps[q] = e;
    }
}

struct PlanScanArgs {
    const unsigned* qblocks; long long n; int keep; int grid;
    long long* qpre; long long* cand_off; int* cand_cnt; unsigned* gthr; DphWork* work;
    const DphPairWork* pairwork; const int* nseg;
};
__global__ void __launch_bounds__(1024) plan_scan_kernel(PlanScanArgs a) {
    __shared__ long long wsum[32];
    __shared__ long long carry, total;
    const int tid = threadIdx.x, lane = tid & 31, warp = tid >> 5;
    if (tid == 0) carry = 0;
    __syncthreads();
    for (long long base = 0; base < a.n; base += 1024) {
        long long q = base + tid;
        long long v = q < a.n ? (long long)a.qblocks[q] : 0, incl = v;
#pragma unroll
        for (int off = 1; off < 32; off <<= 1) { long long t = __shfl_up_sync(0xffffffffu, incl, off); if (lane >= off) incl += t; }
        if (lane == 31) wsum[warp] = incl;
        __syncthreads();
        if (warp == 0) {
            long long w = wsum[lane], wi = w;
#pragma unroll
            for (int off = 1; off < 32; off <<= 1) { long long t = __shfl_up_sync(0xffffffffu, wi, off); if (lane >= off) wi += t; }
            wsum[lane] = wi - w;
        }
        __syncthreads();
        long long excl = carry + wsum[warp] + incl - v;
        if (q < a.n) { a.qpre[q] = excl; a.cand_cnt[q] = 0; a.gthr[q] = 0u; }
        __syncthreads();
        if (tid == 1023) carry = excl + v;
        __syncthreads();
    }
    if (tid == 0) { total = carry; a.qpre[a.n] = carry; a.work->total_blocks = carry; carry = 0; }
    __syncthreads();
    const long long T = total;
    const long long per = a.pairwork ? a.pairwork->per : (T / a.grid > 0 ? T / a.grid : 1);
    for (long long base = 0; base < a.n; base += 1024) {
        long long q = base + tid;
        long long v = 0;
        if (q < a.n) {
            long long qb = (long long)a.qblocks[q];
            if (qb > 0) {
                long long parts = qb / per + 2;
                if (a.pairwork) parts = (long long)a.nseg[q] + qb / per + 1;
                else if (parts > a.grid) parts = a.grid;
                v = parts * a.keep;
            }
        }
        long long incl = v;
#pragma unroll
        for (int off = 1; off < 32; off <<= 1) { long long t = __shfl_up_sync(0xffffffffu, incl, off); if (lane >= off) incl += t; }
        if (lane == 31) wsum[warp] = incl;
        __syncthreads();
        if (warp == 0) {
            long long w = wsum[lane], wi = w;
#pragma unroll
            for (int off = 1; off < 32; off <<= 1) { long long t = __shfl_up_sync(0xffffffffu, wi, off); if (lane >= off) wi += t; }
            wsum[lane] = wi - w;
        }
        __syncthreads();
        long long excl = carry + wsum[warp] + incl - v;
        if (q < a.n) a.cand_off[q] = excl;
        __syncthreads();
        if (tid == 1023) carry = excl + v;
        __syncthreads();
    }
    if (tid == 0) a.cand_off[a.n] = carry;
}

struct PairPlanArgs {
    const int* key; long long nq_probes; int nprobe; const int* list_len; long long list_lo, list_hi, nlist; int grid;
    int* cnt; int* fill; int* off; long long* blockpre; unsigned* entries; DphPairWork* work;
    int* unitpre; unsigned long long* units;
    int gsz;
    DphUnit* udesc;
    const long long* blk_off; const float* cd; const unsigned* gdense; const float2* qparams;
};
__global__ void pair_count_kernel(PairPlanArgs a) {
    const long long i = (long long)blockIdx.x * blockDim.x + threadIdx.x;
    if (i >= a.nq_probes) return;
    const int l = a.key[i];
    if (l >= a.list_lo && l < a.list_hi && a.list_len[l] > 0) atomicAdd(&a.cnt[l], 1);
}
__global__ void __launch_bounds__(1024) pair_scan_kernel(PairPlanArgs a) {
    __shared__ long long wsa[32], wsb[32];
    __shared__ long long ca, cb;
    const int tid = threadIdx.x, lane = tid & 31, warp = tid >> 5;
    if (tid == 0) { ca = 0; cb = 0; }
    __syncthreads();
    for (long long base = a.list_lo; base < a.list_hi; base += 1024) {
        const long long l = base + tid;
        long long va = 0, vb = 0;
        if (l < a.list_hi) {
            const int c = a.cnt[l];
            va = c;
            vb = (long long)((c + a.gsz - 1) / a.gsz) * (long long)((a.list_len[l] + 31) >> 5);
        }
        long long ia = va, ib = vb;
#pragma unroll
        for (int off = 1; off < 32; off <<= 1) {
            long long t1 = __shfl_up_sync(0xffffffffu, ia, off), t2 = __shfl_up_sync(0xffffffffu, ib, off);
            if (lane >= off) { ia += t1; ib += t2; }
        }
        if (lane == 31) { wsa[warp] = ia; wsb[warp] = ib; }
        __syncthreads();
        if (warp == 0) {
            long long w1 = wsa[lane], w2 = wsb[lane], i1 = w1, i2 = w2;
#pragma unroll
            for (int off = 1; off < 32; off <<= 1) {
                long long t1 = __shfl_up_sync(0xffffffffu, i1, off), t2 = __shfl_up_sync(0xffffffffu, i2, off);
                if (lane >= off) { i1 += t1; i2 += t2; }
            }
            wsa[lane] = i1 - w1; wsb[lane] = i2 - w2;
        }
        __syncthreads();
        const long long ea = ca + wsa[warp] + ia - va, eb = cb + wsb[warp] + ib - vb;
        if (l < a.list_hi) { a.off[l] = (int)ea; a.blockpre[l] = eb; }
        __syncthreads();
        if (tid == 1023) { ca = ea + va; cb = eb + vb; }
        __syncthreads();
    }
    __shared__ long long segb_s;
    if (tid == 0) {
        a.off[a.list_hi] = (int)ca; a.blockpre[a.list_hi] = cb;
        long long segb = (cb + (long long)a.grid * DPH_PAIR_UNITS_PER_CTA - 1) / ((long long)a.grid * DPH_PAIR_UNITS_PER_CTA);
        if (segb < DPH_PAIR_SEG_MIN) segb = DPH_PAIR_SEG_MIN;
        a.work->total_blocks = cb;
        a.work->per = segb;
        segb_s = segb; ca = 0;
    }
    __syncthreads();
    const long long segb = segb_s;
    for (long long base = a.list_lo; base < a.list_hi; base += 1024) {
        const long long l = base + tid;
        long long va = 0;
        if (l < a.list_hi) {
            const long long nb = (a.list_len[l] + 31) >> 5;
            va = (long long)((a.cnt[l] + a.gsz - 1) / a.gsz) * ((nb + segb - 1) / segb);
        }
        long long ia = va;
#pragma unroll
        for (int off = 1; off < 32; off <<= 1) { long long t1 = __shfl_up_sync(0xffffffffu, ia, off); if (lane >= off) ia += t1; }
        if (lane == 31) wsa[warp] = ia;
        __syncthreads();
        if (warp == 0) {
            long long w1 = wsa[lane], i1 = w1;
#pragma unroll
            for (int off = 1; off < 32; off <<= 1) { long long t1 = __shfl_up_sync(0xffffffffu, i1, off); if (lane >= off) i1 += t1; }
            wsa[lane] = i1 - w1;
        }
        __syncthreads();
        const long long ea = ca + wsa[warp] + ia - va;
        if (l < a.list_hi) a.unitpre[l] = (int)ea;
        __syncthreads();
        if (tid == 1023) ca = ea + va;
        __syncthreads();
    }
    if (tid == 0) { a.work->total_units = (int)ca; a.work->next_unit = 0; }
}
__global__ void pair_units_kernel(PairPlanArgs a) {
    const long long l = a.list_lo + (long long)blockIdx.x * blockDim.x + threadIdx.x;
    if (l >= a.list_hi) return;
    const int cnt = a.cnt[l];
    const int items = (cnt + a.gsz - 1) / a.gsz;
    if (items == 0) return;
    const long long segb = a.work->per, nb = (a.list_len[l] + 31) >> 5;
    const int nsegs = (int)((nb + segb - 1) / segb);
    const long long u0 = a.unitpre[l];
    for (int it = 0; it < items; it++) {
        DphUnit d;
        if (a.udesc) {
            d.blk = a.blk_off[l]; d.len = a.list_len[l]; d.list = (int)l; d.pad = 0;
            d.nq = min(a.gsz, cnt - a.gsz * it);
            const int e0 = a.off[l] + a.gsz * it;
#pragma unroll
            for (int i = 0; i < DPH_QUAD_ITEM_Q; i++) {
                const unsigned e = a.entries[e0 + (i < d.nq ? i : 0)];
                const long long q = e >> 10; const int r = (int)(e & 1023u);
                const float2 pp = a.qparams[q];
                d.q[i] = (unsigned)q; d.gs[i] = a.gdense[q * a.nprobe + r];
                d.base[i] = a.cd[q * a.nprobe + r] + pp.y; d.step[i] = pp.x;
            }
        }
        for (int s = 0; s < nsegs; s++) {
            const long long u = u0 + (long long)s * items + it;
            a.units[u] = (unsigned long long)l | ((unsigned long long)it << 32) | ((unsigned long long)s << 48);
            if (a.udesc) {
                d.bi0 = (unsigned)(s * segb);
                d.bend = (unsigned)((nb - (long long)d.bi0 < segb) ? nb : (long long)d.bi0 + segb);
                a.udesc[u] = d;
            }
        }
    }
}
__global__ void pair_fill_kernel(PairPlanArgs a) {
    const long long i = (long long)blockIdx.x * blockDim.x + threadIdx.x;
    if (i >= a.nq_probes) return;
    const int l = a.key[i];
    if (l >= a.list_lo && l < a.list_hi && a.list_len[l] > 0) {
        const int pos = a.off[l] + atomicAdd(&a.fill[l], 1);
        a.entries[pos] = (unsigned)((i / a.nprobe) << 10) | (unsigned)(i % a.nprobe);
    }
}

int dph_launch_plan(dph_index* ix, int64_t n, int k, int keep, int grid, const int32_t* only_flagged, cudaStream_t st, int group) {
    const bool pair = group > 1;
    (void)k;
    if (n == 0) return 0;
    PlanArgs a;
    a.key = ix->key.as<int>(); a.cd = ix->cd.as<float>(); a.list_len = ix->list_len; a.blk_off = (const long long*)ix->blk_off;
    a.list_lo = ix->list_lo; a.list_hi = ix->list_hi; a.nprobe = ix->nprobe; a.n = n; a.only_flagged = only_flagged;
    a.lutmax = ix->lutmax.as<float>(); a.segs = ix->segs.as<DphSeg>(); a.qblocks = ix->qinfo.as<unsigned>(); a.nseg = ix->nseg.as<int>(); a.eps = ix->eps.as<float>();
    a.gdense = pair ? ix->gdense.as<unsigned>() : nullptr; a.qparams = pair ? ix->qparams.as<float2>() : nullptr;
    plan_segs_kernel<<<(unsigned)((n + 7) / 8), 256, 0, st>>>(a);
    DPH_CUDA(cudaGetLastError());
    if (pair) {
        PairPlanArgs p;
        p.key = ix->key.as<int>(); p.nq_probes = n * ix->nprobe; p.nprobe = ix->nprobe; p.list_len = ix->list_len; p.list_lo = ix->list_lo;
        p.list_hi = ix->list_hi; p.nlist = ix->nlist; p.grid = grid; p.cnt = ix->pl_cnt.as<int>(); p.fill = ix->pl_fill.as<int>();
        p.off = ix->pl_off.as<int>(); p.blockpre = ix->pl_blockpre.as<long long>(); p.entries = ix->pl_entries.as<unsigned>();
        p.work = ix->pairwork.as<DphPairWork>(); p.unitpre = ix->pl_unitpre.as<int>(); p.units = ix->pl_units.as<unsigned long long>();
        p.gsz = group == 4 ? DPH_QUAD_ITEM_Q : group;
        p.udesc = group == 4 ? ix->pl_udesc.as<DphUnit>() : nullptr;
        p.blk_off = (const long long*)ix->blk_off; p.cd = ix->cd.as<float>(); p.gdense = ix->gdense.as<unsigned>(); p.qparams = ix->qparams.as<float2>();
        DPH_CUDA(cudaMemsetAsync(p.cnt, 0, (size_t)ix->nlist * 4, st));
        DPH_CUDA(cudaMemsetAsync(p.fill, 0, (size_t)ix->nlist * 4, st));
        const unsigned nb = (unsigned)((p.nq_probes + 255) / 256);
        pair_count_kernel<<<nb, 256, 0, st>>>(p);
        pair_scan_kernel<<<1, 1024, 0, st>>>(p);
        pair_fill_kernel<<<nb, 256, 0, st>>>(p);
        if (ix->list_hi > ix->list_lo) pair_units_kernel<<<(unsigned)((ix->list_hi - ix->list_lo + 255) / 256), 256, 0, st>>>(p);
        DPH_CUDA(cudaGetLastError());
    }
    PlanScanArgs b;
    b.pairwork = pair ? ix->pairwork.as<DphPairWork>() : nullptr; b.nseg = ix->nseg.as<int>();
    b.qblocks = ix->qinfo.as<unsigned>(); b.n = n; b.keep = keep; b.grid = grid; b.qpre = ix->wpre.as<long long>();
    b.cand_off = ix->cand_off.as<long long>(); b.cand_cnt = ix->cand_cnt.as<int>(); b.gthr = ix->gthr.as<unsigned>();
    b.work = ix->work.as<DphWork>();
    plan_scan_kernel<<<1, 1024, 0, st>>>(b);
    DPH_CUDA(cudaGetLastError());
    return 0;
}

DPH_API int dph_sgemm_nt_seq(const float* X, int64_t n, const float* W, int64_t m, int64_t K, float* out, void* cuda_stream) {
    return dph_launch_sgemm_nt_seq(X, n, W, m, (int)K, out, (cudaStream_t)cuda_stream);
}
```

### densephrases_b200/csrc/scan.cu

```cuda
#include "index_internal.cuh"
#include "select.cuh"

struct ScanArgs {
    const uint8_t* codes; const long long* qpre; const DphSeg* segs; const int* nseg; const DphWork* work;
    const float* lut_canon;
    unsigned* gthr; unsigned long long* cand; const long long* cand_off; int* cand_cnt;
    long long n; int nprobe; int keep;
};

#define NT DPH_SCAN_THREADS
#define NW DPH_SCAN_WARPS
#define SMEM_LUT_FAST (DPH_LUT_SCAN_FLOATS * 4)
#define SMEM_LUT_EXACT (DPH_LUT_CANON_FLOATS * 4 + NW * DPH_BLK_BYTES)

struct ScanShared {
    unsigned long long cbuf[DPH_CAND_CAP];
    DphSeg segtab[DPH_SEG_SMEM];
    SelectScratch sc;
    int cnt; unsigned thr; int base; int ndone; int ndone_snap; int pad[3];
};

__device__ __forceinline__ uint4 ldg_stream(const uint4* p) {
    uint4 r;
    asm volatile("ld.global.nc.L1::no_allocate.v4.u32 {%0,%1,%2,%3}, [%4];" : "=r"(r.x), "=r"(r.y), "=r"(r.z), "=r"(r.w) : "l"(p));
    return r;
}
__device__ __forceinline__ void l2_prefetch_block(const void* p) {
    asm volatile("cp.async.bulk.prefetch.L2.global [%0], %1;" :: "l"(p), "n"(DPH_BLK_BYTES) : "memory");
}

extern __shared__ __align__(1024) unsigned char dph_smem[];
#define DPH_DYN_SMEM_BASE 0x400

template <int IMM> __device__ __forceinline__ float lds_imm(unsigned addr) {
    float v;
    asm volatile("ld.shared.f32 %0, [%1+%2];" : "=f"(v) : "r"(addr), "n"(IMM));
    return v;
}
template <int T0> __device__ __forceinline__ void fast_word(unsigned wv, unsigned y, float2& a01, float2& a23) {
    constexpr int TB = DPH_DYN_SMEM_BASE + (T0 >> 5) * 65536 + (T0 & 31) * 4;
    const float v0 = lds_imm<TB + 0>(__byte_perm(wv, y, 0x7504));
    const float v1 = lds_imm<TB + 4>(__byte_perm(wv, y, 0x7514));
    const float v2 = lds_imm<TB + 8>(__byte_perm(wv, y, 0x7524));
    const float v3 = lds_imm<TB + 12>(__byte_perm(wv, y, 0x7534));
    a01 = dph_fadd2(a01, make_float2(v0, v1));
    a23 = dph_fadd2(a23, make_float2(v2, v3));
}
template <int C> __device__ __forceinline__ void fast_chunk(const uint4& v, unsigned y, float2& a01, float2& a23) {
    fast_word<C * 16 + 0>(v.x, y, a01, a23);
    fast_word<C * 16 + 4>(v.y, y, a01, a23);
    fast_word<C * 16 + 8>(v.z, y, a01, a23);
    fast_word<C * 16 + 12>(v.w, y, a01, a23);
}

struct SegCursor {
    int seg; unsigned wrel, wend; const uint4* base; int len; unsigned gstart; float dis0;
    __device__ __forceinline__ void init() { seg = -1; wrel = 0; wend = 0; base = nullptr; len = 0; gstart = 0; dis0 = 0.f; }
    __device__ __forceinline__ void seek(const DphSeg* __restrict__ tab, unsigned b, const uint8_t* codes) {
        if (b < wend) return;
        do { seg++; } while (b >= tab[seg].wend);
        const uint4 u0 = *reinterpret_cast<const uint4*>(tab + seg);
        const uint4 u1 = *(reinterpret_cast<const uint4*>(tab + seg) + 1);
        base = reinterpret_cast<const uint4*>(codes + (long long)(((unsigned long long)u0.y << 32) | u0.x) * DPH_BLK_BYTES);
        len = (int)u0.z; gstart = u0.w; dis0 = __uint_as_float(u1.x); wrel = u1.y; wend = u1.z;
    }
    __device__ __forceinline__ const uint4* ptr(unsigned b) const { return base + (size_t)(b - wrel) * (DPH_BLK_BYTES / 16); }
};

__device__ __forceinline__ void block_compact(ScanShared* sh, int keep, unsigned* gthr_q) {
    const int tid = threadIdx.x;
    const int n = sh->cnt;
    unsigned long long* cb = sh->cbuf;
    unsigned long long pivot = block_radix_select([&](int i) { return cb[i]; }, n, keep, &sh->sc);
    unsigned long long mine[DPH_CAND_CAP / NT];
#pragma unroll
    for (int e = 0; e < DPH_CAND_CAP / NT; e++) { int i = tid + e * NT; mine[e] = (i < n) ? cb[i] : 0ull; }
    __syncthreads();
    if (tid == 0) sh->cnt = 0;
    __syncthreads();
#pragma unroll
    for (int e = 0; e < DPH_CAND_CAP / NT; e++)
        if (mine[e] >= pivot && mine[e] != 0ull) { int p = atomicAdd(&sh->cnt, 1); cb[p] = mine[e]; }
    if (tid == 0) {
        unsigned t = (unsigned)(pivot >> 32);
        unsigned old = atomicMax(gthr_q, t);
        sh->thr = t > old ? t : old;
        sh->ndone_snap = sh->ndone;
    }
    __syncthreads();
}

template <int MODE>
__global__ void __launch_bounds__(NT, 1) scan_kernel(ScanArgs a) {
    unsigned char* const smem = dph_smem;
    constexpr int LUT_BYTES = (MODE == DPH_SCAN_FAST) ? SMEM_LUT_FAST : SMEM_LUT_EXACT;
    ScanShared* sh = reinterpret_cast<ScanShared*>(smem + LUT_BYTES);
    const int tid = threadIdx.x, lane = tid & 31, warp = tid >> 5;
    const long long T = a.work->total_blocks;
    const long long G = gridDim.x, c = blockIdx.x;
    const long long g0 = T * c / G, g1 = T * (c + 1) / G;
    if (g0 >= g1) return;
    long long lo = 0, hi = a.n;
    while (hi - lo > 1) { long long mid = (lo + hi) >> 1; if (a.qpre[mid] <= g0) lo = mid; else hi = mid; }
    long long q = lo, g = g0;
    const unsigned ywin = (((unsigned)__cvta_generic_to_shared(dph_smem)) & 0xFF000000u) | ((unsigned)lane * 4u);

    while (g < g1) {
        while (a.qpre[q + 1] <= g) q++;
        const long long qstart = a.qpre[q];
        const long long gend = (a.qpre[q + 1] < g1) ? a.qpre[q + 1] : g1;
        const unsigned b0 = (unsigned)(g - qstart), b1 = (unsigned)(gend - qstart);
        __syncthreads();
        {
            const int nsg0 = a.nseg[q];
            if (nsg0 <= DPH_SEG_SMEM) {
                const uint4* src = reinterpret_cast<const uint4*>(a.segs + q * a.nprobe);
                uint4* dst = reinterpret_cast<uint4*>(sh->segtab);
                for (int i = tid; i < nsg0 * 2; i += NT) dst[i] = __ldg(src + i);
            }
        }
        if (tid == 0) { sh->cnt = 0; sh->ndone = 0; sh->ndone_snap = 0; sh->thr = *((volatile unsigned*)(a.gthr + q)); }
        __syncthreads();

        const DphSeg* tab = (a.nseg[q] <= DPH_SEG_SMEM) ? sh->segtab : (a.segs + q * a.nprobe);
        SegCursor cc, pc;
        cc.init(); pc.init();
        unsigned b = b0 + warp;
        unsigned bp = b0 + warp;
        uint4 nxt[6];
        int n_len = 0; unsigned n_gstart = 0, n_j0 = 0; float n_dis0 = 0.f;
#pragma unroll 1
        for (int r = 0; r < DPH_L2_PREFETCH_ROUNDS && bp < b1; r++, bp += NW) {
            pc.seek(tab, bp, a.codes);
            if (lane == 0) l2_prefetch_block(pc.ptr(bp));
        }
        bool more = b < b1;
        if (more) {
            cc.seek(tab, b, a.codes);
            const uint4* p = cc.ptr(b) + lane;
#pragma unroll
            for (int c6 = 0; c6 < 6; c6++) nxt[c6] = ldg_stream(p + c6 * 32);
            n_len = cc.len; n_gstart = cc.gstart; n_dis0 = cc.dis0; n_j0 = (b - cc.wrel) * 32u;
        }
        {
            const float4* src = reinterpret_cast<const float4*>(a.lut_canon + (size_t)q * DPH_LUT_CANON_FLOATS);
            constexpr int PER_T = DPH_LUT_CANON_FLOATS / 4 / NT;
            constexpr int LB = 12;
            static_assert(PER_T % LB == 0, "LUT staging batches");
            if (MODE == DPH_SCAN_FAST) {
                float* dstf = reinterpret_cast<float*>(smem);
#pragma unroll 1
                for (int i0 = tid; i0 < DPH_LUT_CANON_FLOATS / 4; i0 += NT * LB) {
                    float4 v[LB];
#pragma unroll
                    for (int e = 0; e < LB; e++) v[e] = __ldg(src + i0 + e * NT);
#pragma unroll
                    for (int e = 0; e < LB; e++) {
                        const int i = i0 + e * NT;
                        const int row = i >> 3, w = (i & 7) * 4;
                        float* r = dstf + row * 64;
                        *reinterpret_cast<float4*>(r + w) = v[e];
                        if (w < 28) *reinterpret_cast<float4*>(r + 32 + w) = v[e];
                        else { r[60] = v[e].x; r[61] = v[e].y; r[62] = v[e].z; r[63] = 0.0f; }
                    }
                }
            } else {
                float4* dst = reinterpret_cast<float4*>(smem);
#pragma unroll 8
                for (int i = tid; i < DPH_LUT_CANON_FLOATS / 4; i += NT) dst[i] = __ldg(src + i);
            }
        }
        __syncthreads();
        bool counted = false;
        while (true) {
            while (more) {
                if (*((volatile int*)&sh->cnt) > DPH_CAND_CAP - NT) break;
                uint4 cur[6];
#pragma unroll
                for (int c6 = 0; c6 < 6; c6++) cur[c6] = nxt[c6];
                const int c_len = n_len; const unsigned c_gstart = n_gstart, c_j0 = n_j0; const float c_dis0 = n_dis0;
                if (bp < b1) {
                    pc.seek(tab, bp, a.codes);
                    if (lane == 0) l2_prefetch_block(pc.ptr(bp));
                    bp += NW;
                }
                b += NW;
                more = b < b1;
                if (more) {
                    cc.seek(tab, b, a.codes);
                    const uint4* p = cc.ptr(b) + lane;
#pragma unroll
                    for (int c6 = 0; c6 < 6; c6++) nxt[c6] = ldg_stream(p + c6 * 32);
                    n_len = cc.len; n_gstart = cc.gstart; n_dis0 = cc.dis0; n_j0 = (b - cc.wrel) * 32u;
                }
                float score;
                if (MODE == DPH_SCAN_FAST) {
                    float2 a01 = make_float2(c_dis0, 0.f), a23 = make_float2(0.f, 0.f);
                    fast_chunk<0>(cur[0], ywin, a01, a23);
                    fast_chunk<1>(cur[1], ywin, a01, a23);
                    fast_chunk<2>(cur[2], ywin, a01, a23);
                    fast_chunk<3>(cur[3], ywin, a01, a23);
                    fast_chunk<4>(cur[4], ywin, a01, a23);
                    fast_chunk<5>(cur[5], ywin, a01, a23);
                    score = (a01.x + a01.y) + (a23.x + a23.y);
                } else {
                    unsigned char* stage = smem + DPH_LUT_CANON_FLOATS * 4 + warp * DPH_BLK_BYTES;
                    const float* lutc = reinterpret_cast<const float*>(smem);
#pragma unroll
                    for (int c6 = 0; c6 < 6; c6++) *reinterpret_cast<uint4*>(stage + c6 * 512 + lane * 16) = cur[c6];
                    __syncwarp();
                    float dis = c_dis0;
#pragma unroll 8
                    for (int m = 0; m < DPH_M; m++) dis += lutc[DPH_LUTC_IDX(m, (int)stage[dph_blk_addr(lane, m)])];
                    score = dis;
                    __syncwarp();
                }
                const unsigned j = c_j0 + lane;
                const unsigned sk = dph_fkey(score);
                const bool pass = ((int)j < c_len) && (sk >= *((volatile unsigned*)&sh->thr));
                const unsigned pm = __ballot_sync(0xffffffffu, pass);
                if (pm) {
                    int basep = 0;
                    if (lane == 0) basep = atomicAdd(&sh->cnt, __popc(pm));
                    basep = __shfl_sync(0xffffffffu, basep, 0);
                    if (pass) {
                        int p = basep + __popc(pm & ((1u << lane) - 1u));
                        if (p < DPH_CAND_CAP) sh->cbuf[p] = ((unsigned long long)sk << 32) | (unsigned long long)(0xFFFFFFFFu - (c_gstart + j));
                    }
                }
            }
            if (!more && !counted) { counted = true; if (lane == 0) atomicAdd(&sh->ndone, 1); }
            __syncthreads();
            if (sh->cnt > a.keep) block_compact(sh, a.keep, a.gthr + q);
            else {
                if (tid == 0) {
                    unsigned gt = *((volatile unsigned*)(a.gthr + q));
                    if (gt > sh->thr) sh->thr = gt;
                    sh->ndone_snap = sh->ndone;
                }
                __syncthreads();
            }
            if (sh->ndone_snap == NW) break;
        }
        __syncthreads();
        const int cnt = sh->cnt;
        if (tid == 0) sh->base = atomicAdd(a.cand_cnt + q, cnt);
// ... 127 lines not shown
        const unsigned gs_a = a.gdense[qa * a.nprobe + ra], gs_b = a.gdense[qb * a.nprobe + rb];
        const uint4* lbase = reinterpret_cast<const uint4*>(a.codes + a.blk_off[l] * DPH_BLK_BYTES);

        unsigned b = bi0 + warp, bp = bi0 + warp;
        uint4 nxt[6];
#pragma unroll 1
        for (int r = 0; r < DPH_L2_PREFETCH_ROUNDS && bp < bend; r++, bp += NW)
            if (lane == 0) l2_prefetch_block(lbase + (size_t)bp * (DPH_BLK_BYTES / 16));
        bool more = b < bend;
        if (more) {
            const uint4* p = lbase + (size_t)b * (DPH_BLK_BYTES / 16) + lane;
#pragma unroll
            for (int c6 = 0; c6 < 6; c6++) nxt[c6] = ldg_stream(p + c6 * 32);
        }
        bool counted = false;
        while (true) {
            while (more) {
                if (*((volatile int*)&sh->cnt[0]) > PCAP - NT || *((volatile int*)&sh->cnt[1]) > PCAP - NT) break;
                uint4 cur[6];
#pragma unroll
                for (int c6 = 0; c6 < 6; c6++) cur[c6] = nxt[c6];
                const unsigned bcur = b;
                if (bp < bend) { if (lane == 0) l2_prefetch_block(lbase + (size_t)bp * (DPH_BLK_BYTES / 16)); bp += NW; }
                b += NW;
                more = b < bend;
                if (more) {
                    const uint4* p = lbase + (size_t)b * (DPH_BLK_BYTES / 16) + lane;
#pragma unroll
                    for (int c6 = 0; c6 < 6; c6++) nxt[c6] = ldg_stream(p + c6 * 32);
                }
                unsigned s0 = 0, s1 = 0, s2 = 0, s3 = 0;
                pair_chunk<0>(cur[0], ywin, s0, s1, s2, s3);
                pair_chunk<1>(cur[1], ywin, s0, s1, s2, s3);
                pair_chunk<2>(cur[2], ywin, s0, s1, s2, s3);
                pair_chunk<3>(cur[3], ywin, s0, s1, s2, s3);
                pair_chunk<4>(cur[4], ywin, s0, s1, s2, s3);
                pair_chunk<5>(cur[5], ywin, s0, s1, s2, s3);
                const unsigned tot = (s0 + s1) + (s2 + s3);
                const float sc_a = fmaf(pa.x, (float)(tot & 0xFFFFu), base_a);
                const float sc_b = fmaf(pb.x, (float)(tot >> 16), base_b);
                const unsigned j = bcur * 32u + lane;
                const bool valid = (int)j < len;
                const unsigned ka = dph_fkey(sc_a), kb = dph_fkey(sc_b);
                warp_append(valid && ka >= *((volatile unsigned*)&sh->thr[0]), ((unsigned long long)ka << 32) | (unsigned long long)(0xFFFFFFFFu - (gs_a + j)),
                            sh->cbuf[0], &sh->cnt[0], PCAP, lane);
                warp_append(valid && kb >= *((volatile unsigned*)&sh->thr[1]), ((unsigned long long)kb << 32) | (unsigned long long)(0xFFFFFFFFu - (gs_b + j)),
                            sh->cbuf[1], &sh->cnt[1], PCAP, lane);
            }
            if (!more && !counted) { counted = true; if (lane == 0) atomicAdd(&sh->ndone, 1); }
            __syncthreads();
            if (sh->cnt[0] > a.keep) compact_buffer<PCAP, NT>(sh->cbuf[0], &sh->cnt[0], &sh->thr[0], a.keep, a.gthr + qa, &sh->sc);
            if (sh->cnt[1] > a.keep) compact_buffer<PCAP, NT>(sh->cbuf[1], &sh->cnt[1], &sh->thr[1], a.keep, a.gthr + qb, &sh->sc);
            if (tid == 0) {
                unsigned ga = *((volatile unsigned*)(a.gthr + qa));
                if (ga > sh->thr[0]) sh->thr[0] = ga;
                if (has_b) { unsigned gb = *((volatile unsigned*)(a.gthr + qb)); if (gb > sh->thr[1]) sh->thr[1] = gb; }
                sh->ndone_snap = sh->ndone;
            }
            __syncthreads();
            if (sh->ndone_snap == NW) break;
        }
        for (int s2i = 0; s2i < (has_b ? 2 : 1); s2i++) {
            const long long q = s2i ? qb : qa;
            const int cnt = sh->cnt[s2i];
            if (tid == 0) sh->base[s2i] = atomicAdd(a.cand_cnt + q, cnt);
            __syncthreads();
            const long long off = a.cand_off[q], cap = a.cand_off[q + 1] - off;
            const int basep = sh->base[s2i];
            for (int i = tid; i < cnt; i += NT)
                if (basep + i < cap) a.cand[off + basep + i] = sh->cbuf[s2i][i];
        }
    }
}


#define QNT 256
#define QNW (QNT / 32)
#define QCAP 512
#define SMEM_QUAD_TABLES (3 * 65536)
static_assert(QCAP - QNT == DPH_QUAD_KEEP_MAX, "quad latch margin");
struct QuadShared {
    unsigned long long cbuf[DPH_QUAD_ITEM_Q][QCAP];
    SelectScratch sc;
    DphUnit desc[2];
    int cnt[DPH_QUAD_ITEM_Q]; unsigned thr[DPH_QUAD_ITEM_Q]; int base[DPH_QUAD_ITEM_Q]; int ndone; int ndone_snap; int unit; int full;
    long long qs[DPH_QUAD_ITEM_Q];
};
__device__ __forceinline__ unsigned imad_add(unsigned x, unsigned one, unsigned c) {
    unsigned d;
    asm("mad.lo.u32 %0, %1, %2, %3;" : "=r"(d) : "r"(x), "r"(one), "r"(c));
    return d;
}
template <int T0, int TAB, int IMADL> __device__ __forceinline__ void quad_gather(const unsigned (&ad)[4], unsigned one, unsigned (&sr)[4], unsigned (&ab)[4]) {
    constexpr int S = T0 >> 5;
    constexpr int TB = DPH_DYN_SMEM_BASE + (S < 2 ? TAB : 2) * 65536 + (S < 2 ? S : TAB) * 128;
    constexpr int A = (T0 >> 2) & 1;
    const unsigned w0 = lds_imm_u32<TB>(ad[0]);
    const unsigned w1 = lds_imm_u32<TB>(ad[1]);
    const unsigned w2 = lds_imm_u32<TB>(ad[2]);
    const unsigned w3 = lds_imm_u32<TB>(ad[3]);
    if (IMADL >= 1) {
        sr[2 * A] = imad_add(w1, one, imad_add(w0, one, sr[2 * A]));
        sr[2 * A + 1] = imad_add(w3, one, imad_add(w2, one, sr[2 * A + 1]));
    } else {
        sr[2 * A] += w0 + w1;
        sr[2 * A + 1] += w2 + w3;
    }
    const unsigned e0 = __byte_perm(w0, 0u, 0x4341), e1 = __byte_perm(w1, 0u, 0x4341);
    const unsigned e2 = __byte_perm(w2, 0u, 0x4341), e3 = __byte_perm(w3, 0u, 0x4341);
    if (IMADL >= 3 || (IMADL == 2 && A == 1)) {
        ab[2 * A] = imad_add(e1, one, imad_add(e0, one, ab[2 * A]));
        ab[2 * A + 1] = imad_add(e3, one, imad_add(e2, one, ab[2 * A + 1]));
    } else {
        ab[2 * A] += e0 + e1;
        ab[2 * A + 1] += e2 + e3;
    }
}
template <int T> struct RotSel { static constexpr int reg = (T & 31) / 3, sel = 0x7700 | (4 + (T & 31) % 3); };
template <int T0, int NTAB, int IMADL> __device__ __forceinline__ void quad_word(unsigned wv, const unsigned (&rot)[11], unsigned one,
                                                                                  unsigned (&sr)[2][4], unsigned (&ab)[2][4]) {
    const unsigned ad[4] = {__byte_perm(wv, rot[RotSel<T0>::reg], RotSel<T0>::sel | 0x00),
                            __byte_perm(wv, rot[RotSel<T0 + 1>::reg], RotSel<T0 + 1>::sel | 0x10),
                            __byte_perm(wv, rot[RotSel<T0 + 2>::reg], RotSel<T0 + 2>::sel | 0x20),
                            __byte_perm(wv, rot[RotSel<T0 + 3>::reg], RotSel<T0 + 3>::sel | 0x30)};
    quad_gather<T0, 0, IMADL>(ad, one, sr[0], ab[0]);
    if (NTAB == 2) quad_gather<T0, 1, IMADL>(ad, one, sr[1], ab[1]);
}
template <int C, int NTAB, int IMADL> __device__ __forceinline__ void quad_chunk(const uint4& v, const unsigned (&rot)[11], unsigned one,
                                                                                   unsigned (&sr)[2][4], unsigned (&ab)[2][4]) {
    quad_word<C * 16 + 0, NTAB, IMADL>(v.x, rot, one, sr, ab);
    quad_word<C * 16 + 4, NTAB, IMADL>(v.y, rot, one, sr, ab);
    quad_word<C * 16 + 8, NTAB, IMADL>(v.z, rot, one, sr, ab);
    quad_word<C * 16 + 12, NTAB, IMADL>(v.w, rot, one, sr, ab);
}
__device__ __forceinline__ void warp_append_latch(bool pass, unsigned long long key, unsigned long long* cb, int* cnt, int* full, int lane) {
    const unsigned pm = __ballot_sync(0xffffffffu, pass);
    if (pm) {
        int basep = 0;
        const int np = __popc(pm);
        if (lane == 0) { basep = atomicAdd(cnt, np); if (basep + np > QCAP - QNT) *((volatile int*)full) = 1; }
        basep = __shfl_sync(0xffffffffu, basep, 0);
        if (pass) { int p = basep + __popc(pm & ((1u << lane) - 1u)); if (p < QCAP) cb[p] = key; }
    }
}
__device__ __forceinline__ void cp_async16(void* smem_dst, const void* gsrc) {
    asm volatile("cp.async.ca.shared.global [%0], [%1], 16;" :: "r"((unsigned)__cvta_generic_to_shared(smem_dst)), "l"(gsrc) : "memory");
}
__device__ __forceinline__ float quad_thr_f(unsigned t) {
    return t == 0xFFFFFFFFu ? __int_as_float(0x7f800000) : (t == 0u ? -__int_as_float(0x7f800000) : dph_fkey_inv(t));
}

#ifdef DPH_SCAN_PHASES
__device__ unsigned long long g_quad_phase_ns[4];
__device__ unsigned g_quad_phase_ctas;
__device__ __forceinline__ unsigned long long globaltimer_ns() { unsigned long long t; asm volatile("mov.u64 %0, %globaltimer;" : "=l"(t)); return t; }
#define QPH_MARK(i) do { if (threadIdx.x == 0) { const unsigned long long t_ = globaltimer_ns(); ph[i] += t_ - ph_t; ph_t = t_; } } while (0)
#else
#define QPH_MARK(i) do { } while (0)
#endif

template <int NTAB, int IMADL>
__device__ __forceinline__ void quad_item_rounds(const PairScanArgs& a, QuadShared* sh, const DphUnit* dsc, const uint4* lbase, unsigned b,
                                                 unsigned bp, uint4 (&nxt)[6], const unsigned (&rot)[11], unsigned one, unsigned long long* ph,
                                                 unsigned long long& ph_t) {
    (void)ph; (void)ph_t;
    const int lane = threadIdx.x & 31;
    const int len = dsc->len, nq = dsc->nq;
    const unsigned bend = dsc->bend;
    constexpr int NS = 4 * NTAB;
    unsigned gsv[NS]; float stepv[NS], basev[NS], tf[NS]; unsigned thr[NS];
#pragma unroll
    for (int i = 0; i < NS; i++) { gsv[i] = dsc->gs[i]; basev[i] = dsc->base[i]; stepv[i] = dsc->step[i]; thr[i] = sh->thr[i]; tf[i] = quad_thr_f(thr[i]); }
    bool more = b < bend, counted = false;
    while (true) {
        while (more) {
            if (*((volatile int*)&sh->full)) break;
            uint4 cur6[6];
#pragma unroll
            for (int c6 = 0; c6 < 6; c6++) cur6[c6] = nxt[c6];
            const unsigned bcur = b;
            if (bp < bend) { if (lane == 0) l2_prefetch_block(lbase + (size_t)bp * (DPH_BLK_BYTES / 16)); bp += QNW; }
            b += QNW;
            more = b < bend;
            if (more) {
                const uint4* p = lbase + (size_t)b * (DPH_BLK_BYTES / 16) + lane;
#pragma unroll
                for (int c6 = 0; c6 < 6; c6++) nxt[c6] = ldg_stream(p + c6 * 32);
            }
            unsigned sr[2][4] = {}, ab[2][4] = {};
            quad_chunk<0, NTAB, IMADL>(cur6[0], rot, one, sr, ab);
            quad_chunk<1, NTAB, IMADL>(cur6[1], rot, one, sr, ab);
            quad_chunk<2, NTAB, IMADL>(cur6[2], rot, one, sr, ab);
            quad_chunk<3, NTAB, IMADL>(cur6[3], rot, one, sr, ab);
            quad_chunk<4, NTAB, IMADL>(cur6[4], rot, one, sr, ab);
            quad_chunk<5, NTAB, IMADL>(cur6[5], rot, one, sr, ab);
            const unsigned j = bcur * 32u + lane;
            const bool valid = (int)j < len;
            float f[NS]; bool p[NS]; bool any = false;
#pragma unroll
            for (int tb = 0; tb < NTAB; tb++) {
                const unsigned SR = (sr[tb][0] + sr[tb][1]) + (sr[tb][2] + sr[tb][3]);
                const unsigned AB = (ab[tb][0] + ab[tb][1]) + (ab[tb][2] + ab[tb][3]);
                const unsigned AE = SR - (AB << 8);
                f[4 * tb + 0] = fmaf(stepv[4 * tb + 0], (float)(unsigned short)(AE), basev[4 * tb + 0]);
                f[4 * tb + 1] = fmaf(stepv[4 * tb + 1], (float)(unsigned short)(AB), basev[4 * tb + 1]);
                f[4 * tb + 2] = fmaf(stepv[4 * tb + 2], (float)(unsigned short)(AE >> 16), basev[4 * tb + 2]);
                f[4 * tb + 3] = fmaf(stepv[4 * tb + 3], (float)(unsigned short)(AB >> 16), basev[4 * tb + 3]);
            }
#pragma unroll
            for (int i = 0; i < NS; i++) { p[i] = valid && f[i] >= tf[i]; any = any || p[i]; }
            if (__any_sync(0xffffffffu, any)) {
#pragma unroll
                for (int i = 0; i < NS; i++) {
                    const unsigned k = dph_fkey(f[i]);
                    warp_append_latch(p[i] && k >= thr[i], ((unsigned long long)k << 32) | (unsigned long long)(0xFFFFFFFFu - (gsv[i] + j)),
                                      sh->cbuf[i], &sh->cnt[i], &sh->full, lane);
                }
            }
        }
        if (!more && !counted) { counted = true; if (lane == 0) atomicAdd(&sh->ndone, 1); }
        __syncthreads();
        QPH_MARK(1);
#pragma unroll 1
        for (int i = 0; i < nq; i++)
            if (sh->cnt[i] > a.keep) compact_buffer<QCAP, QNT>(sh->cbuf[i], &sh->cnt[i], &sh->thr[i], a.keep, a.gthr + sh->qs[i], &sh->sc);
        if (threadIdx.x == 0) {
            for (int i = 0; i < nq; i++) { unsigned g = *((volatile unsigned*)(a.gthr + sh->qs[i])); if (g > sh->thr[i]) sh->thr[i] = g; }
            sh->ndone_snap = sh->ndone;
            sh->full = 0;
        }
        __syncthreads();
        QPH_MARK(2);
#pragma unroll
        for (int i = 0; i < NS; i++) { thr[i] = sh->thr[i]; tf[i] = quad_thr_f(thr[i]); }
        if (sh->ndone_snap == QNW) break;
    }
}

template <int IMADL>
__global__ void __launch_bounds__(QNT, 1) scan_quad_kernel(PairScanArgs a) {
    unsigned char* const smem = dph_smem;
    QuadShared* sh = reinterpret_cast<QuadShared*>(smem + SMEM_QUAD_TABLES);
    const int tid = threadIdx.x, lane = tid & 31, warp = tid >> 5;
    const int total_units = a.work->total_units;
    const unsigned char* lut8 = reinterpret_cast<const unsigned char*>(a.lutq);
    const unsigned one = a.one;
    unsigned rot[11];
#pragma unroll
    for (int r = 0; r < 11; r++) {
        unsigned v = 0;
#pragma unroll
        for (int bb = 0; bb < 3; bb++)
            if (3 * r + bb < 32) v |= (unsigned)(((lane + 3 * r + bb) & 31) * 4) << (8 * bb);
        rot[r] = v;
    }
    unsigned long long ph[4] = {0ull, 0ull, 0ull, 0ull}, ph_t = 0ull;
#ifdef DPH_SCAN_PHASES
    if (tid == 0) ph_t = globaltimer_ns();
#endif

    if (tid == 0) sh->unit = atomicAdd(a.next_unit, 1);
    __syncthreads();
    int cur = 0;
    bool any_unit = sh->unit < total_units;
    if (any_unit && tid < (int)(sizeof(DphUnit) / 16))
        reinterpret_cast<uint4*>(&sh->desc[0])[tid] = __ldg(reinterpret_cast<const uint4*>(a.udesc + sh->unit) + tid);
    __syncthreads();
    while (any_unit) {
        int next_u = 0;
        if (tid == 0) next_u = atomicAdd(a.next_unit, 1);
        const DphUnit* dsc = &sh->desc[cur];
        const int nq = dsc->nq;
        const int ntab = nq > 4 ? 2 : 1;
        const unsigned bi0 = dsc->bi0, bend = dsc->bend;
        const uint4* lbase = reinterpret_cast<const uint4*>(a.codes + dsc->blk * DPH_BLK_BYTES);

        unsigned b = bi0 + warp, bp = bi0 + warp;
        uint4 nxt[6];
#pragma unroll 1
        for (int r = 0; r < DPH_L2_PREFETCH_ROUNDS && bp < bend; r++, bp += QNW)
            if (lane == 0) l2_prefetch_block(lbase + (size_t)bp * (DPH_BLK_BYTES / 16));
        if (b < bend) {
            const uint4* p = lbase + (size_t)b * (DPH_BLK_BYTES / 16) + lane;
#pragma unroll
            for (int c6 = 0; c6 < 6; c6++) nxt[c6] = ldg_stream(p + c6 * 32);
        }
        unsigned gq = 0xFFFFFFFFu;
        if (tid < DPH_QUAD_ITEM_Q && tid < nq) gq = *((volatile unsigned*)(a.gthr + dsc->q[tid]));
        {
            const unsigned* src[DPH_QUAD_ITEM_Q];
#pragma unroll
            for (int i = 0; i < DPH_QUAD_ITEM_Q; i++) src[i] = reinterpret_cast<const unsigned*>(lut8 + (size_t)dsc->q[i] * DPH_LUT_SCAN_FLOATS);
            uint4* dst = reinterpret_cast<uint4*>(smem);
            constexpr int LB = 6, PER_TAB = 768 * 8;
            static_assert(PER_TAB % (QNT * LB) == 0, "a batch of the build stays inside one table");
#pragma unroll 1
            for (int i0 = tid; i0 < ntab * PER_TAB; i0 += QNT * LB) {
                const int tb = i0 >= PER_TAB;
                const unsigned* T0p = tb ? src[4] : src[0];
                const unsigned* T1p = tb ? src[5] : src[1];
                const unsigned* T2p = tb ? src[6] : src[2];
                const unsigned* T3p = tb ? src[7] : src[3];
                const int ib = i0 - tb * PER_TAB;
                unsigned va[LB], vb[LB], vc[LB], vd[LB];
#pragma unroll
                for (int e = 0; e < LB; e++) {
                    const int i = ib + e * QNT, s = (i >> 3) * 16 + (i & 7);
                    va[e] = __ldg(T0p + s); vb[e] = __ldg(T1p + s); vc[e] = __ldg(T2p + s); vd[e] = __ldg(T3p + s);
                }
#pragma unroll
                for (int e = 0; e < LB; e++) {
                    const int i = ib + e * QNT, row = i >> 3, cg = i & 7;
                    const int seg = row >> 8, code = row & 255;
                    const int region = seg < 2 ? tb : 2, half = seg < 2 ? seg : tb;
                    const unsigned t0 = __byte_perm(va[e], vb[e], 0x5140), t1 = __byte_perm(va[e], vb[e], 0x7362);
                    const unsigned u0 = __byte_perm(vc[e], vd[e], 0x5140), u1 = __byte_perm(vc[e], vd[e], 0x7362);
                    uint4 o;
                    o.x = __byte_perm(t0, u0, 0x5410); o.y = __byte_perm(t0, u0, 0x7632);
                    o.z = __byte_perm(t1, u1, 0x5410); o.w = __byte_perm(t1, u1, 0x7632);
                    dst[region * 4096 + code * 16 + half * 8 + cg] = o;
                }
            }
        }
        if (tid < DPH_QUAD_ITEM_Q) { sh->cnt[tid] = 0; sh->qs[tid] = (long long)dsc->q[tid]; sh->thr[tid] = gq; }
        if (tid == 0) { sh->ndone = 0; sh->ndone_snap = 0; sh->full = 0; }
        __syncthreads();
        QPH_MARK(0);
        if (warp == 0) {
            const int nu = __shfl_sync(0xffffffffu, next_u, 0);
            if (lane == 0) sh->unit = nu;
            if (nu < total_units && lane < (int)(sizeof(DphUnit) / 16))
                cp_async16(reinterpret_cast<unsigned char*>(&sh->desc[cur ^ 1]) + lane * 16, reinterpret_cast<const unsigned char*>(a.udesc + nu) + lane * 16);
            asm volatile("cp.async.commit_group;" ::: "memory");
        }
        if (ntab == 2) quad_item_rounds<2, IMADL>(a, sh, dsc, lbase, b, bp, nxt, rot, one, ph, ph_t);
        else quad_item_rounds<1, IMADL>(a, sh, dsc, lbase, b, bp, nxt, rot, one, ph, ph_t);
        if (tid < nq) sh->base[tid] = atomicAdd(a.cand_cnt + sh->qs[tid], sh->cnt[tid]);
        if (warp == 0) asm volatile("cp.async.wait_all;" ::: "memory");
        __syncthreads();
#pragma unroll 1
        for (int i = 0; i < nq; i++) {
            const long long q = sh->qs[i];
            const int cnt = sh->cnt[i];
            const long long off = a.cand_off[q], cap = a.cand_off[q + 1] - off;
            const int basep = sh->base[i];
            for (int c = tid; c < cnt; c += QNT)
                if (basep + c < cap) a.cand[off + basep + c] = sh->cbuf[i][c];
        }
        any_unit = sh->unit < total_units;
        __syncthreads();
        QPH_MARK(3);
        cur ^= 1;
    }
#ifdef DPH_SCAN_PHASES
    if (tid == 0) {
        for (int i = 0; i < 4; i++) atomicAdd(&g_quad_phase_ns[i], ph[i]);
        __threadfence();
        if (atomicAdd(&g_quad_phase_ctas, 1u) == gridDim.x - 1) {
            __threadfence();
            unsigned long long v[4];
            for (int i = 0; i < 4; i++) { v[i] = atomicExch(&g_quad_phase_ns[i], 0ull); }
            printf("scan_quad_kernel phases (ms, summed over %u CTAs): table build %.3f, scan rounds %.3f, compaction barriers %.3f, publish %.3f\n",
                   gridDim.x, v[0] * 1e-6, v[1] * 1e-6, v[2] * 1e-6, v[3] * 1e-6);
            g_quad_phase_ctas = 0;
        }
    }
#endif
}
#undef QPH_MARK

__global__ void smem_base_probe_kernel(unsigned* out) { *out = (unsigned)__cvta_generic_to_shared(dph_smem); }

int dph_scan_setup_attrs() {
    static DphPerDeviceOnce once;
    if (!once.first()) return 0;
    {
        unsigned* d = nullptr; unsigned h = 0;
        DPH_CUDA(cudaMalloc((void**)&d, 4));
        smem_base_probe_kernel<<<1, 32, 1024>>>(d);
        DPH_CUDA(cudaMemcpy(&h, d, 4, cudaMemcpyDeviceToHost));
        cudaFree(d);
        DPH_CHECK(h == DPH_DYN_SMEM_BASE, "dynamic shared memory window does not start at 0x400 on this driver; rebuild with the probed value");
    }
    DPH_CUDA(cudaFuncSetAttribute(scan_kernel<DPH_SCAN_FAST>, cudaFuncAttributeMaxDynamicSharedMemorySize, SMEM_LUT_FAST + (int)sizeof(ScanShared)));
    DPH_CUDA(cudaFuncSetAttribute(scan_kernel<DPH_SCAN_EXACT>, cudaFuncAttributeMaxDynamicSharedMemorySize, SMEM_LUT_EXACT + (int)sizeof(ScanShared)));
    DPH_CUDA(cudaFuncSetAttribute(scan_pair_kernel, cudaFuncAttributeMaxDynamicSharedMemorySize, SMEM_LUT_FAST + (int)sizeof(PairShared)));
    DPH_CUDA(cudaFuncSetAttribute(scan_quad_kernel<0>, cudaFuncAttributeMaxDynamicSharedMemorySize, SMEM_QUAD_TABLES + (int)sizeof(QuadShared)));
    DPH_CUDA(cudaFuncSetAttribute(scan_quad_kernel<1>, cudaFuncAttributeMaxDynamicSharedMemorySize, SMEM_QUAD_TABLES + (int)sizeof(QuadShared)));
    DPH_CUDA(cudaFuncSetAttribute(scan_quad_kernel<2>, cudaFuncAttributeMaxDynamicSharedMemorySize, SMEM_QUAD_TABLES + (int)sizeof(QuadShared)));
    DPH_CUDA(cudaFuncSetAttribute(scan_quad_kernel<3>, cudaFuncAttributeMaxDynamicSharedMemorySize, SMEM_QUAD_TABLES + (int)sizeof(QuadShared)));
    return 0;
}

int dph_launch_scan(dph_index* ix, int64_t n, int k, int keep, int mode, int grid, cudaStream_t st) {
    (void)k;
    if (n == 0) return 0;
    DPH_TRY(dph_scan_setup_attrs());
    ScanArgs a;
    a.codes = ix->codes; a.qpre = ix->wpre.as<long long>(); a.segs = ix->segs.as<DphSeg>(); a.nseg = ix->nseg.as<int>(); a.work = ix->work.as<DphWork>();
    a.lut_canon = ix->lut_canon.as<float>(); a.gthr = ix->gthr.as<unsigned>();
    a.cand = ix->cand.as<unsigned long long>(); a.cand_off = ix->cand_off.as<long long>(); a.cand_cnt = ix->cand_cnt.as<int>();
    a.n = n; a.nprobe = ix->nprobe; a.keep = keep;
    if (mode == DPH_SCAN_FAST)
        scan_kernel<DPH_SCAN_FAST><<<grid, NT, SMEM_LUT_FAST + sizeof(ScanShared), st>>>(a);
    else
        scan_kernel<DPH_SCAN_EXACT><<<grid, NT, SMEM_LUT_EXACT + sizeof(ScanShared), st>>>(a);
    DPH_CUDA(cudaGetLastError());
    return 0;
}

int dph_launch_scan_pair(dph_index* ix, int64_t n, int keep, int grid, cudaStream_t st, int group) {
    if (n == 0) return 0;
    DPH_TRY(dph_scan_setup_attrs());
    PairScanArgs a;
    a.codes = ix->codes; a.blk_off = (const long long*)ix->blk_off; a.list_len = ix->list_len; a.pl_cnt = ix->pl_cnt.as<int>();
    a.pl_off = ix->pl_off.as<int>(); a.units = ix->pl_units.as<unsigned long long>(); a.entries = ix->pl_entries.as<unsigned>();
    a.work = ix->pairwork.as<DphPairWork>(); a.next_unit = &ix->pairwork.as<DphPairWork>()->next_unit; a.lutq = ix->lutq.as<unsigned short>(); a.qparams = ix->qparams.as<float2>();
    a.cd = ix->cd.as<float>(); a.gdense = ix->gdense.as<unsigned>(); a.gthr = ix->gthr.as<unsigned>();
    a.cand = ix->cand.as<unsigned long long>(); a.cand_off = ix->cand_off.as<long long>(); a.cand_cnt = ix->cand_cnt.as<int>();
    a.list_lo = ix->list_lo; a.list_hi = ix->list_hi; a.nprobe = ix->nprobe; a.keep = keep;
    a.udesc = ix->pl_udesc.as<DphUnit>(); a.one = 1u;
    if (group == 4) {
        const size_t sm = SMEM_QUAD_TABLES + sizeof(QuadShared);
        switch (g_dph_tune[0]) {
            case 0: scan_quad_kernel<0><<<grid, QNT, sm, st>>>(a); break;
            case 2: scan_quad_kernel<2><<<grid, QNT, sm, st>>>(a); break;
            case 3: scan_quad_kernel<3><<<grid, QNT, sm, st>>>(a); break;
            default: scan_quad_kernel<1><<<grid, QNT, sm, st>>>(a); break;
        }
    }
    else scan_pair_kernel<<<grid, NT, SMEM_LUT_FAST + sizeof(PairShared), st>>>(a);
    DPH_CUDA(cudaGetLastError());
    return 0;
}

struct MergeArgs {
    const unsigned long long* cand; const long long* cand_off; const int* cand_cnt; const unsigned* gthr; const float* eps;
    const DphSeg* segs; const int* nseg; int nprobe; int k; int mode;
    const uint8_t* codes; const float* lut_canon; const long long* ids; const long long* list_start;
    float* D; long long* I; unsigned* G; int* flags; const int* only_flagged;
};

__device__ __forceinline__ int find_seg(const unsigned* gstart, int nsg, unsigned gidx) {
    int lo = 0, hi = nsg;
    while (hi - lo > 1) { int mid = (lo + hi) >> 1; if (gstart[mid] <= gidx) lo = mid; else hi = mid; }
    return lo;
}

__global__ void __launch_bounds__(256) merge_kernel(MergeArgs a) {
    __shared__ SelectScratch sc;
    __shared__ unsigned long long surv[DPH_SURV_CAP];
    __shared__ unsigned sgs[DPH_MAX_NPROBE];
    __shared__ int scnt, sflag;
    const long long q = blockIdx.x;
    const int tid = threadIdx.x;
    if (a.only_flagged && a.only_flagged[q] == 0) return;
    const unsigned long long* E = a.cand + a.cand_off[q];
    long long cap = a.cand_off[q + 1] - a.cand_off[q];
    int n = a.cand_cnt[q];
    const bool overflow = n > cap;
    if (n > cap) n = (int)cap;
    const DphSeg* segs = a.segs + q * a.nprobe;
    const int nsg = a.nseg[q];
    const int k = a.k;
    if (tid == 0) { scnt = 0; sflag = 0; }
    for (int i = tid; i < nsg; i += blockDim.x) sgs[i] = segs[i].gstart;
    __syncthreads();
    auto get = [&](int i) { return E[i]; };
    unsigned long long pivot = 0ull;
    int flag = overflow ? 1 : 0;
    if (a.mode == DPH_SCAN_FAST) {
        const float eps2 = 2.0f * a.eps[q];
        const unsigned gt = a.gthr[q];
        if (n > k) {
            unsigned long long pk = block_radix_select(get, n, k, &sc);
            const float Tk = dph_ckey_score(pk);
            if (gt != 0u && !(Tk - dph_fkey_inv(gt) > eps2)) flag = 1;
            pivot = (unsigned long long)dph_fkey(Tk - eps2) << 32;
        } else if (gt != 0u) flag = 1;
    } else {
        if (n > DPH_SURV_CAP) pivot = block_radix_select(get, n, k, &sc);
    }
    for (int i = tid; i < n; i += blockDim.x) {
        unsigned long long e = E[i];
        if (e >= pivot) { int p = atomicAdd(&scnt, 1); if (p < DPH_SURV_CAP) surv[p] = e; else sflag = 1; }
    }
    __syncthreads();
    int ns = scnt < DPH_SURV_CAP ? scnt : DPH_SURV_CAP;
    if (sflag) flag = 1;
    if (a.mode == DPH_SCAN_FAST) {
        const float* lutc = a.lut_canon + (size_t)q * DPH_LUT_CANON_FLOATS;
        const int lane = tid & 31, warp = tid >> 5, nwarps = blockDim.x >> 5;
        for (int i = warp; i < ns; i += nwarps) {
            const unsigned gidx = dph_ckey_gidx(surv[i]);
            const DphSeg s = segs[find_seg(sgs, nsg, gidx)];
            const unsigned j = gidx - s.gstart;
            const uint8_t* blk = a.codes + (s.blk + (long long)(j >> 5)) * DPH_BLK_BYTES;
            const int ln = (int)(j & 31u);
            float v[3];
#pragma unroll
            for (int h = 0; h < 3; h++) {
                const int m = h * 32 + lane;
                v[h] = __ldg(lutc + DPH_LUTC_IDX(m, (int)blk[dph_blk_addr(ln, m)]));
            }
            float dis = s.dis0;
#pragma unroll
            for (int h = 0; h < 3; h++)
#pragma unroll
                for (int l2 = 0; l2 < 32; l2++) dis += __shfl_sync(0xffffffffu, v[h], l2);
            __syncwarp();
            if (lane == 0) surv[i] = dph_ckey(dis, gidx);
        }
    }
    const int p2 = dph_next_pow2(ns > 1 ? ns : 1);
    for (int i = ns + tid; i < p2; i += blockDim.x) surv[i] = 0ull;
    __syncthreads();
    block_bitonic_sort_desc(surv, p2);
    for (int i = tid; i < k; i += blockDim.x) {
        float d = DPH_NEUTRAL; long long id = -1; unsigned gi = 0xFFFFFFFFu;
        if (i < ns) {
            const unsigned long long e = surv[i];
            gi = dph_ckey_gidx(e); d = dph_ckey_score(e);
            const DphSeg s = segs[find_seg(sgs, nsg, gi)];
            const unsigned j = gi - s.gstart;
            id = a.ids ? a.ids[s.blk * 32 + j] : a.list_start[s.list] + (long long)j;
        }
        a.D[q * k + i] = d; a.I[q * k + i] = id; a.G[q * k + i] = gi;
    }
    if (a.mode == DPH_SCAN_FAST && tid == 0) a.flags[q] = flag;
}

int dph_launch_merge(dph_index* ix, int64_t n, int k, int mode, const int32_t* only_flagged, float* D, int64_t* I, uint32_t* G,
                     cudaStream_t st) {
    if (n == 0) return 0;
    MergeArgs a;
    a.cand = ix->cand.as<unsigned long long>(); a.cand_off = ix->cand_off.as<long long>(); a.cand_cnt = ix->cand_cnt.as<int>();
    a.gthr = ix->gthr.as<unsigned>(); a.eps = ix->eps.as<float>(); a.segs = ix->segs.as<DphSeg>(); a.nseg = ix->nseg.as<int>(); a.nprobe = ix->nprobe; a.k = k; a.mode = mode;
    a.codes = ix->codes; a.lut_canon = ix->lut_canon.as<float>(); a.ids = (const long long*)ix->ids; a.list_start = (const long long*)ix->list_start;
    a.D = D; a.I = (long long*)I; a.G = G; a.flags = ix->flags.as<int>(); a.only_flagged = only_flagged;
    merge_kernel<<<(unsigned)n, 256, 0, st>>>(a);
    DPH_CUDA(cudaGetLastError());
    return 0;
}

__global__ void pack_topk_kernel(const float* D, const long long* I, const unsigned* G, long long total, longlong2* P) {
    long long i = (long long)blockIdx.x * blockDim.x + threadIdx.x;
    if (i >= total) return;
    longlong2 v;
    v.x = I[i] >= 0 ? (long long)dph_ckey(D[i], G[i]) : 0ll;
    v.y = I[i];
    P[i] = v;
}
__global__ void __launch_bounds__(256) merge_packed_kernel(const longlong2* Pg, int nshards, long long n, int k, float* D, long long* I) {
    extern __shared__ unsigned long long mp[];
    const long long q = blockIdx.x;
    const int tot = nshards * k, p2 = dph_next_pow2(tot);
    unsigned long long* keys = mp;
    for (int i = threadIdx.x; i < p2; i += blockDim.x) {
        unsigned long long key = 0ull;
        if (i < tot) key = (unsigned long long)Pg[((long long)(i / k) * n + q) * k + (i % k)].x;
        keys[i] = key;
    }
    __syncthreads();
    block_bitonic_sort_desc(keys, p2);
    for (int i = threadIdx.x; i < k; i += blockDim.x) {
        float d = DPH_NEUTRAL; long long id = -1;
        const unsigned long long key = keys[i];
        if (key != 0ull) {
            d = dph_ckey_score(key);
            for (int j = 0; j < tot && id < 0; j++) {
                const longlong2 e = Pg[((long long)(j / k) * n + q) * k + (j % k)];
                if ((unsigned long long)e.x == key) id = e.y;
            }
        }
        D[q * k + i] = d; I[q * k + i] = id;
    }
}
DPH_API int dph_pack_topk(const float* D, const int64_t* I, const uint32_t* G, int64_t n, int k, int64_t* P, void* cuda_stream) {
    const long long total = (long long)n * k;
    if (total == 0) return 0;
    pack_topk_kernel<<<(unsigned)((total + 255) / 256), 256, 0, (cudaStream_t)cuda_stream>>>(D, (const long long*)I, G, total, (longlong2*)P);
    DPH_CUDA(cudaGetLastError());
    return 0;
}
DPH_API int dph_merge_shards_packed(const int64_t* Pg, int nshards, int64_t n, int k, float* D, int64_t* I, void* cuda_stream) {
    if (n == 0) return 0;
    DPH_CHECK(nshards >= 1 && k >= 1 && (long long)nshards * k <= 8192, "merge_shards: nshards*k must be <= 8192");
    int p2 = 1; while (p2 < nshards * k) p2 <<= 1;
    static DphPerDeviceOnce once;
    if (once.first()) { DPH_CUDA(cudaFuncSetAttribute(merge_packed_kernel, cudaFuncAttributeMaxDynamicSharedMemorySize, 8192 * 8)); }
    merge_packed_kernel<<<(unsigned)n, 256, p2 * 8, (cudaStream_t)cuda_stream>>>((const longlong2*)Pg, nshards, n, k, D, (long long*)I);
    DPH_CUDA(cudaGetLastError());
    return 0;
}

__global__ void __launch_bounds__(256) merge_shards_kernel(const float* Dg, const long long* Ig, const unsigned* Gg, int nshards, long long n,
                                                            int k, float* D, long long* I) {
    extern __shared__ unsigned long long ms[];
    const long long q = blockIdx.x;
    const int tid = threadIdx.x;
    const int tot = nshards * k;
    const int p2 = dph_next_pow2(tot);
    unsigned long long* keys = ms;
    for (int i = tid; i < p2; i += blockDim.x) {
        unsigned long long key = 0ull;
        if (i < tot) {
            int s = i / k, r = i % k;
            long long id = Ig[((long long)s * n + q) * k + r];
            if (id >= 0) key = dph_ckey(Dg[((long long)s * n + q) * k + r], Gg[((long long)s * n + q) * k + r]);
        }
        keys[i] = key;
    }
    __syncthreads();
    block_bitonic_sort_desc(keys, p2);
    for (int i = tid; i < k; i += blockDim.x) {
        float d = DPH_NEUTRAL; long long id = -1;
        unsigned long long key = keys[i];
        if (key != 0ull) {
            unsigned gi = dph_ckey_gidx(key);
            d = dph_ckey_score(key);
            for (int s = 0; s < nshards && id < 0; s++)
                for (int r = 0; r < k; r++) {
                    long long o = ((long long)s * n + q) * k + r;
                    if (Gg[o] == gi && Ig[o] >= 0) { id = Ig[o]; break; }
                }
        }
        D[q * k + i] = d; I[q * k + i] = id;
    }
}

DPH_API int dph_merge_shards(const float* Dg, const int64_t* Ig, const uint32_t* Gg, int nshards, int64_t n, int k, float* D, int64_t* I,
                                void* cuda_stream) {
    if (n == 0) return 0;
    DPH_CHECK(nshards >= 1 && k >= 1 && (long long)nshards * k <= 8192, "merge_shards: nshards*k must be <= 8192");
    int p2 = 1; while (p2 < nshards * k) p2 <<= 1;
    static DphPerDeviceOnce once;
    if (once.first()) { DPH_CUDA(cudaFuncSetAttribute(merge_shards_kernel, cudaFuncAttributeMaxDynamicSharedMemorySize, 8192 * 8)); }
    merge_shards_kernel<<<(unsigned)n, 256, p2 * 8, (cudaStream_t)cuda_stream>>>(Dg, (const long long*)Ig, Gg, nshards, n, k, D, (long long*)I);
    DPH_CUDA(cudaGetLastError());
    return 0;
}
```

### densephrases_b200/ivfpq.py

```python
import ctypes as C

import numpy as np

from . import _lib as L


def _np_ptr(a):
    return a.ctypes.data_as(C.c_void_p)


class IvfPqIndex:
    def __init__(self, nlist, d=768, M=96, nbits=8, device=0):
        self._h = C.c_void_p()
        L.check(L.lib().dph_index_create(C.byref(self._h), d, nlist, M, nbits, device))
        self.device = device

    def __del__(self):
        h, self._h = getattr(self, "_h", None), None
        if h and L is not None and getattr(L, "_lib", None) is not None:
            L._lib.dph_index_free(h)

    @classmethod
    def from_arrays(cls, A, centroids, pq, list_len, codes, ids=None, device=0, shard=None):
        ix = cls(len(list_len), device=device)
# ... 139 lines not shown
        assert list_len.shape == (self.nlist,)
        L.check(L.lib().dph_index_sync_list_len(self._h, _np_ptr(list_len)))

    def last_remove_ms(self):
        out = np.zeros(3, dtype=np.float32)
        L.check(L.lib().dph_index_last_remove_ms(self._h, _np_ptr(out)))
        return out

    def last_remove_tmp_bytes(self):
        return int(L.lib().dph_index_last_remove_tmp_bytes(self._h))

    def _train_input(self, x):
        if isinstance(x, np.ndarray):
            x = np.ascontiguousarray(x, dtype=np.float32)
            return _np_ptr(x), self._rows(x), L.MEM_HOST, x
        import torch
        if not (x.is_cuda and x.dtype == torch.float32):
            raise TypeError("train: expected a numpy array or a float32 CUDA tensor")
        x = x.contiguous()
        self.set_stream(torch.cuda.current_stream(x.device).cuda_stream)
        return x.data_ptr(), self._rows(x), L.MEM_DEVICE, x

    def train_coarse(self, x, niter=10, seed=1234, max_points_per_centroid=256, hot_start=False):
        p, n, mem, keep = self._train_input(x)
        if n < 39 * self.nlist:
            import warnings
            warnings.warn(f"train_coarse: {n} training points for {self.nlist} centroids; faiss wants at least {39 * self.nlist}")
        obj = np.zeros(max(niter, 1), dtype=np.float64)
        nsplit = np.zeros(max(niter, 1), dtype=np.int64)
        L.check(L.lib().dph_index_train_coarse(self._h, p, n, int(niter), C.c_uint64(seed), int(max_points_per_centroid), int(bool(hot_start)),
                                                mem, _np_ptr(obj), _np_ptr(nsplit)))
        del keep
        return obj[:niter], nsplit[:niter]

    def train_pq(self, x, niter=25, seed=1234, max_points_per_centroid=256, hot_start=False, residual=True):
        p, n, mem, keep = self._train_input(x)
        L.check(L.lib().dph_index_train_pq(self._h, p, n, int(niter), C.c_uint64(seed), int(max_points_per_centroid), int(bool(hot_start)),
                                            int(bool(residual)), mem))
        del keep

    def encode_pq(self, x):
        if isinstance(x, np.ndarray):
            x = np.ascontiguousarray(x, dtype=np.float32)
            codes = np.empty((self._rows(x), 96), dtype=np.uint8)
            L.check(L.lib().dph_index_encode_pq(self._h, _np_ptr(x), len(x), _np_ptr(codes), L.MEM_HOST))
            return codes
        import torch
        assert x.is_cuda and x.dtype == torch.float32 and x.is_contiguous()
        codes = torch.empty((self._rows(x), 96), dtype=torch.uint8, device=x.device)
        self.set_stream(torch.cuda.current_stream(x.device).cuda_stream)
        L.check(L.lib().dph_index_encode_pq(self._h, x.data_ptr(), x.shape[0], codes.data_ptr(), L.MEM_DEVICE))
        return codes

    def train_opq(self, x, niter=10, seed=1234, niter_pq=40, niter_pq_hot=4, max_train_points=65536):
        import torch
        dev = torch.device("cuda", self.device)
        n = int(x.shape[0])
        rows = np.arange(n) if n <= max_train_points else np.sort(np.random.default_rng(seed).choice(n, max_train_points, replace=False))
        xs = torch.as_tensor(x[rows] if isinstance(x, np.ndarray) else x[torch.as_tensor(rows, device=x.device)]).to(dev, torch.float32).contiguous()
        g = torch.Generator().manual_seed(seed)
        R = torch.linalg.qr(torch.randn((self.d, self.d), generator=g, dtype=torch.float64))[0].to(dev)
        xd = xs.double()
        for it in range(niter):
            self.set_opq(R.float().cpu().numpy())
            self.train_pq(xs, niter=niter_pq if it == 0 else niter_pq_hot, seed=seed, max_points_per_centroid=max_train_points,
                          hot_start=it > 0, residual=False)
            torch.cuda.current_stream(dev).synchronize()
            codes = self.encode_pq(xs).long()
            pq = torch.from_numpy(self.pq_codebooks()).to(dev)
            y = pq[torch.arange(96, device=dev)[None, :], codes].reshape(len(xs), self.d)
            u, _, vt = torch.linalg.svd(xd.T @ y.double())
            R = (u @ vt).T.contiguous()
        A = R.float().cpu().numpy()
        self.set_opq(A)
        return A

    def train(self, x, niter=10, niter_pq=25, opq_niter=10, seed=1234, max_points_per_centroid=256):
        if self.ntotal:
            raise RuntimeError("train: the index holds vectors")
        if opq_niter > 0:
            self.train_opq(x, niter=opq_niter, seed=seed)
        obj, nsplit = self.train_coarse(x, niter=niter, seed=seed, max_points_per_centroid=max_points_per_centroid)
        self.train_pq(x, niter=niter_pq, seed=seed, max_points_per_centroid=max_points_per_centroid, residual=True)
        self.set_lists(np.zeros(self.nlist, np.int64), np.zeros((0, 96), np.uint8))
        return dict(obj=obj, nsplit=nsplit)

    def centroids(self):
        out = np.empty((self.nlist, self.d), dtype=np.float32)
        L.check(L.lib().dph_index_get_centroids(self._h, _np_ptr(out), L.MEM_HOST))
        return out

    def pq_codebooks(self):
        out = np.empty((96, 256, 8), dtype=np.float32)
        L.check(L.lib().dph_index_get_pq(self._h, _np_ptr(out), L.MEM_HOST))
        return out

    def last_train_ms(self):
        out = np.zeros(3, dtype=np.float32)
        L.check(L.lib().dph_index_last_train_ms(self._h, _np_ptr(out)))
        return out

    @property
    def ntotal(self):
        return L.lib().dph_index_ntotal(self._h)

    @property
    def ntotal_local(self):
        return L.lib().dph_index_ntotal_local(self._h)

    @property
    def d(self):
        return L.lib().dph_index_d(self._h)

    @property
    def nlist(self):
        return L.lib().dph_index_nlist(self._h)

    @property
    def nprobe(self):
        return L.lib().dph_index_nprobe(self._h)

    @nprobe.setter
    def nprobe(self, v):
        L.check(L.lib().dph_index_set_nprobe(self._h, int(v)))

    def set_scan_mode(self, mode):
        L.check(L.lib().dph_index_set_scan_mode(self._h, mode))

    def last_used_pair_mode(self):
        return bool(L.lib().dph_index_last_used_pair_mode(self._h))

    def last_group_size(self):
        return int(L.lib().dph_index_last_group_size(self._h))

    def set_coarse_tc(self, on):
        L.check(L.lib().dph_index_set_coarse_tc(self._h, int(bool(on))))

    def set_stream(self, cuda_stream_ptr):
        L.check(L.lib().dph_index_set_stream(self._h, C.c_void_p(cuda_stream_ptr)))

    def opq_matrix(self):
        A = np.empty((self.d, self.d), dtype=np.float32)
        L.check(L.lib().dph_index_get_opq(self._h, _np_ptr(A), L.MEM_HOST))
        return A

    def set_profile(self, on):
        L.check(L.lib().dph_index_set_profile(self._h, int(bool(on))))

    def last_scan_ms(self):
        ms = C.c_float(0)
        L.check(L.lib().dph_index_last_scan_ms(self._h, C.byref(ms)))
        return ms.value

    def profile_scan_ms(self):
        n = L.lib().dph_index_profile_count(self._h)
        out = np.zeros(max(n, 1), dtype=np.float32)
        L.check(L.lib().dph_index_profile_scan_ms(self._h, _np_ptr(out), n))
        return out[:n]

    @property
    def device_bytes(self):
        return L.lib().dph_index_device_bytes(self._h)

    def search(self, x, k):
        if isinstance(x, np.ndarray):
            x = np.ascontiguousarray(x, dtype=np.float32)
            n = x.shape[0]
            D = np.empty((n, k), dtype=np.float32)
            I = np.empty((n, k), dtype=np.int64)
            L.check(L.lib().dph_index_search(self._h, _np_ptr(x), n, k, _np_ptr(D), _np_ptr(I), L.MEM_HOST))
            return D, I
        import torch
        assert x.is_cuda and x.dtype == torch.float32 and x.is_contiguous()
        n = x.shape[0]
        D = torch.empty((n, k), dtype=torch.float32, device=x.device)
        I = torch.empty((n, k), dtype=torch.int64, device=x.device)
        self.set_stream(torch.cuda.current_stream(x.device).cuda_stream)
        L.check(L.lib().dph_index_search(self._h, x.data_ptr(), n, k, D.data_ptr(), I.data_ptr(), L.MEM_DEVICE))
        return D, I

    def search_partial(self, x, k):
        import torch
        assert x.is_cuda and x.dtype == torch.float32 and x.is_contiguous()
        n = x.shape[0]
        D = torch.empty((n, k), dtype=torch.float32, device=x.device)
        I = torch.empty((n, k), dtype=torch.int64, device=x.device)
        G = torch.empty((n, k), dtype=torch.int32, device=x.device)
        self.set_stream(torch.cuda.current_stream(x.device).cuda_stream)
        L.check(L.lib().dph_index_search_partial(self._h, x.data_ptr(), n, k, D.data_ptr(), I.data_ptr(), G.data_ptr()))
        return D, I, G

    def coarse_local(self, x):
        import torch
        n = x.shape[0]
        keys = torch.empty((n, self.nprobe), dtype=torch.int64, device=x.device)
        self.set_stream(torch.cuda.current_stream(x.device).cuda_stream)
        L.check(L.lib().dph_index_coarse_local(self._h, x.data_ptr(), n, keys.data_ptr()))
        return keys

    def search_preassigned(self, keys_gathered, k):
        import torch
        W, n, _ = keys_gathered.shape
        D = torch.empty((n, k), dtype=torch.float32, device=keys_gathered.device)
        I = torch.empty((n, k), dtype=torch.int64, device=keys_gathered.device)
        G = torch.empty((n, k), dtype=torch.int32, device=keys_gathered.device)
        self.set_stream(torch.cuda.current_stream(keys_gathered.device).cuda_stream)
        L.check(L.lib().dph_index_search_preassigned(self._h, keys_gathered.data_ptr(), W, n, k, D.data_ptr(), I.data_ptr(), G.data_ptr()))
        return D, I, G

    def coarse_split(self, x_local):
        import torch
        n = x_local.shape[0]
        rec = torch.empty((n, L.lib().dph_index_record_floats(self._h)), dtype=torch.float32, device=x_local.device)
        self.set_stream(torch.cuda.current_stream(x_local.device).cuda_stream)
        L.check(L.lib().dph_index_coarse_split(self._h, x_local.data_ptr(), n, rec.data_ptr()))
        return rec

    def search_assigned(self, rec, k):
        import torch
        assert rec.is_cuda and rec.dtype == torch.float32 and rec.is_contiguous()
        n = rec.shape[0]
        D = torch.empty((n, k), dtype=torch.float32, device=rec.device)
        I = torch.empty((n, k), dtype=torch.int64, device=rec.device)
        G = torch.empty((n, k), dtype=torch.int32, device=rec.device)
        self.set_stream(torch.cuda.current_stream(rec.device).cuda_stream)
        L.check(L.lib().dph_index_search_assigned(self._h, rec.data_ptr(), n, k, D.data_ptr(), I.data_ptr(), G.data_ptr()))
        return D, I, G

    def _last(self, which, shape, dtype):
        out = np.empty(shape, dtype=dtype)
        L.check(L.lib().dph_index_copy_last(self._h, which, _np_ptr(out), out.nbytes))
        return out

    def last_flags(self, n):
        return self._last(0, (n,), np.int32)

    def last_probes(self, n):
        return self._last(1, (n, self.nprobe), np.int32)

    def last_coarse(self, n):
        return self._last(2, (n, self.nprobe), np.float32)

    def last_xr(self, n):
        return self._last(3, (n, self.d), np.float32)

    def reconstruct_batch(self, ids):
        if isinstance(ids, np.ndarray) or isinstance(ids, (list, tuple)):
            ids = np.ascontiguousarray(ids, dtype=np.int64)
            out = np.empty((len(ids), self.d), dtype=np.float32)
            found = np.empty(len(ids), dtype=np.uint8)
            L.check(L.lib().dph_index_reconstruct_batch(self._h, _np_ptr(ids), len(ids), _np_ptr(out), _np_ptr(found), L.MEM_HOST))
            return out, found
        import torch
        assert ids.is_cuda and ids.dtype == torch.int64
        out = torch.empty((ids.numel(), self.d), dtype=torch.float32, device=ids.device)
        found = torch.empty(ids.numel(), dtype=torch.uint8, device=ids.device)
        self.set_stream(torch.cuda.current_stream(ids.device).cuda_stream)
        L.check(L.lib().dph_index_reconstruct_batch(self._h, ids.data_ptr(), ids.numel(), out.data_ptr(), found.data_ptr(), L.MEM_DEVICE))
        return out, found


def _window_scores(self, q, first_ids, L):
    q = np.ascontiguousarray(q, dtype=np.float32)
    first_ids = np.ascontiguousarray(first_ids, dtype=np.int64)
    out = np.empty((len(first_ids), L), dtype=np.float32)
    L_.check(L_.lib().dph_index_window_scores(self._h, _np_ptr(q), _np_ptr(first_ids), len(first_ids), L, _np_ptr(out), L_.MEM_HOST))
    return out


L_ = L
IvfPqIndex.window_scores = _window_scores


def merge_shards(Dg, Ig, Gg, k):
    import torch
    nsh, n, kk = Dg.shape
    assert kk == k and Dg.is_contiguous() and Ig.is_contiguous() and Gg.is_contiguous()
    D = torch.empty((n, k), dtype=torch.float32, device=Dg.device)
    I = torch.empty((n, k), dtype=torch.int64, device=Dg.device)
    st = torch.cuda.current_stream(Dg.device).cuda_stream
    L.check(L.lib().dph_merge_shards(Dg.data_ptr(), Ig.data_ptr(), Gg.data_ptr(), nsh, n, k, D.data_ptr(), I.data_ptr(), C.c_void_p(st)))
    return D, I


def pack_topk(D, I, G):
    import torch
    n, k = D.shape
    P = torch.empty((n, k, 2), dtype=torch.int64, device=D.device)
    st = torch.cuda.current_stream(D.device).cuda_stream
    L.check(L.lib().dph_pack_topk(D.data_ptr(), I.data_ptr(), G.data_ptr(), n, k, P.data_ptr(), C.c_void_p(st)))
    return P


def merge_shards_packed(Pg, k):
    import torch
    nsh, n = Pg.shape[0], Pg.shape[1]
    D = torch.empty((n, k), dtype=torch.float32, device=Pg.device)
    I = torch.empty((n, k), dtype=torch.int64, device=Pg.device)
    st = torch.cuda.current_stream(Pg.device).cuda_stream
    L.check(L.lib().dph_merge_shards_packed(Pg.data_ptr(), nsh, n, k, D.data_ptr(), I.data_ptr(), C.c_void_p(st)))
    return D, I
```

### include/dph_b200.h

```cpp
#ifndef DPH_B200_H
#define DPH_B200_H
#include <stdint.h>
#ifdef __cplusplus
extern "C" {
#endif

#define DPH_MEM_HOST 0
#define DPH_MEM_DEVICE 1

#define DPH_SCAN_FAST 0
#define DPH_SCAN_EXACT 1
#define DPH_SCAN_PAIR 2
#define DPH_SCAN_SINGLE 3
#define DPH_SCAN_QUAD 4

typedef struct dph_index dph_index;

const char* dph_last_error(void);
int dph_version(void);

int dph_index_create(dph_index** out, int d, int64_t nlist, int M, int nbits, int device);
void dph_index_free(dph_index* ix);
int dph_index_set_stream(dph_index* ix, void* cuda_stream);
int dph_index_set_opq(dph_index* ix, const float* A, int mem);
int dph_index_set_centroids(dph_index* ix, const float* C, int mem);
int dph_index_set_pq(dph_index* ix, const float* pq, int mem);
int dph_index_gen_centroids(dph_index* ix, uint64_t seed, float sigma);
int dph_index_gen_pq(dph_index* ix, uint64_t seed, float sigma);
int dph_index_set_shard(dph_index* ix, int64_t list_lo, int64_t list_hi);
int dph_index_set_lists(dph_index* ix, const int64_t* list_len, const uint8_t* codes, const int64_t* ids);
int dph_index_set_lists_synthetic(dph_index* ix, const int64_t* list_len, uint64_t seed);

int dph_index_encode(dph_index* ix, const float* x, int64_t n, int64_t* list_no_out, uint8_t* codes_out, int mem);
int dph_index_add_with_ids(dph_index* ix, const float* x, int64_t n, const int64_t* ids, int mem);
int dph_index_copy_lists(dph_index* ix, uint8_t* codes_out, int64_t* ids_out);
int dph_index_get_list_len(const dph_index* ix, int64_t* list_len_out);
int dph_index_last_add_ms(const dph_index* ix, float* ms_out );

int dph_index_remove_ids(dph_index* ix, const int64_t* ids, int64_t n_ids, int64_t range_lo, int64_t range_hi, int mem,
                         int64_t* n_removed_out, int64_t* removed_per_list_out);
int dph_index_sync_list_len(dph_index* ix, const int64_t* list_len);
int dph_index_last_remove_ms(const dph_index* ix, float* ms_out );
int64_t dph_index_last_remove_tmp_bytes(const dph_index* ix);

int dph_index_train_coarse(dph_index* ix, const float* x, int64_t n, int niter, uint64_t seed, int64_t max_points_per_centroid,
                           int hot_start, int mem, double* obj_out, int64_t* nsplit_out);
int dph_index_train_pq(dph_index* ix, const float* x, int64_t n, int niter, uint64_t seed, int64_t max_points_per_centroid,
                       int hot_start, int residual, int mem);
int dph_index_encode_pq(dph_index* ix, const float* x, int64_t n, uint8_t* codes_out, int mem);
int dph_index_get_centroids(const dph_index* ix, float* C_out, int mem);
int dph_index_get_pq(const dph_index* ix, float* pq_out, int mem);
int dph_index_last_train_ms(const dph_index* ix, float* ms_out );

int64_t dph_index_ntotal(const dph_index* ix);
int64_t dph_index_ntotal_local(const dph_index* ix);
int dph_index_d(const dph_index* ix);
int64_t dph_index_nlist(const dph_index* ix);
int dph_index_nprobe(const dph_index* ix);
int dph_index_set_nprobe(dph_index* ix, int nprobe);
int dph_index_set_scan_mode(dph_index* ix, int mode);
int dph_index_set_coarse_tc(dph_index* ix, int on);
int dph_index_get_opq(const dph_index* ix, float* A_out, int mem);
int64_t dph_index_device_bytes(const dph_index* ix);
int dph_index_set_profile(dph_index* ix, int on);
int dph_index_last_scan_ms(dph_index* ix, float* ms);
int dph_index_profile_scan_ms(dph_index* ix, float* ms_out, int max_out);
int dph_index_profile_count(const dph_index* ix);

int dph_index_search(dph_index* ix, const float* x, int64_t n, int k, float* D, int64_t* I, int mem);
int dph_index_search_partial(dph_index* ix, const float* x_dev, int64_t n, int k, float* D_dev, int64_t* I_dev,
                             uint32_t* G_dev);
int dph_index_coarse_local(dph_index* ix, const float* x_dev, int64_t n, uint64_t* keys_dev);
int dph_index_search_preassigned(dph_index* ix, const uint64_t* keys_gathered_dev, int nshards, int64_t n, int k, float* D_dev,
                                 int64_t* I_dev, uint32_t* G_dev);
int dph_index_record_floats(const dph_index* ix);
int dph_index_coarse_split(dph_index* ix, const float* x_dev, int64_t n_local, float* rec_dev);
int dph_index_search_assigned(dph_index* ix, const float* rec_dev, int64_t n, int k, float* D_dev, int64_t* I_dev, uint32_t* G_dev);
int dph_merge_shards(const float* Dg, const int64_t* Ig, const uint32_t* Gg, int nshards, int64_t n, int k, float* D,
                     int64_t* I, void* cuda_stream);
int dph_pack_topk(const float* D, const int64_t* I, const uint32_t* G, int64_t n, int k, int64_t* P, void* cuda_stream);
int dph_merge_shards_packed(const int64_t* Pg, int nshards, int64_t n, int k, float* D, int64_t* I, void* cuda_stream);
const int32_t* dph_index_last_flags(const dph_index* ix);
const int32_t* dph_index_last_probes(const dph_index* ix);
const float* dph_index_last_coarse(const dph_index* ix);
const float* dph_index_last_xr(const dph_index* ix);
int dph_index_last_used_pair_mode(const dph_index* ix);
int dph_index_last_group_size(const dph_index* ix);
int dph_index_copy_last(dph_index* ix, int which, void* dst_host, int64_t bytes);

int dph_index_reconstruct_batch(dph_index* ix, const int64_t* ids, int64_t m, float* out, uint8_t* found, int mem);

int dph_index_window_scores(dph_index* ix, const float* q , const int64_t* first_id , int64_t m, int L,
                            float* out_scores, int mem);

typedef struct dph_encoder dph_encoder;
int dph_encoder_create(dph_encoder** out, int device, int vocab_size, int max_position_embeddings, int type_vocab_size);
void dph_encoder_free(dph_encoder* e);
int dph_encoder_set_stream(dph_encoder* e, void* cuda_stream);
int64_t dph_encoder_tower_floats(const dph_encoder* e);
int dph_encoder_load_tower(dph_encoder* e, int tower, const float* blob, int mem);
int dph_encoder_set_precision(dph_encoder* e, int precise);
int dph_encoder_set_attention(dph_encoder* e, int tensor_core);
int dph_attention_bert(const float* qkv, const int64_t* attention_mask, int B, int S, float* ctx, int tensor_core, void* cuda_stream);
int dph_encoder_embed_query(dph_encoder* e, const int64_t* input_ids, const int64_t* attention_mask, const int64_t* token_type_ids,
                            int B, int S, float* start_out, float* end_out, int mem);

int dph_sgemm_nt_seq(const float* X, int64_t n, const float* W, int64_t m, int64_t K, float* out, void* cuda_stream);

int dph_gemm_tf32_nt(const float* A, const float* W, const float* bias, const float* residual, float* out, int64_t M, int64_t N,
                     int64_t K, int act, int precise ,
                     void* cuda_stream);
int dph_gemm_tf32_set_mode(int mode);
int dph_set_tuning(int knob, int value);

#ifdef __cplusplus
}
#endif
#endif
```

Baseline: 14180.

## Overlap LUT build on side stream, add PDL launches and tail-unit splitting

The LUT build now runs on a side stream concurrently with the coarse quantizer, joined before the plan step. Plan, scan and merge kernels are launched with programmatic dependent launch, and each kernel calls griddepcontrol.wait at entry, to hide launch gaps. The quad scan planner also splits the last lists into shorter segments so the load-imbalance tail at the end of the scan is spread across CTAs, and stage-timing events are added for profiling. Costs include extra stream and event management, more plan bookkeeping and larger candidate buffers.

```diff
diff --git a/densephrases_b200/_lib.py b/densephrases_b200/_lib.py
--- a/densephrases_b200/_lib.py
+++ b/densephrases_b200/_lib.py
@@ -37,6 +37,7 @@
     "dph_index_last_scan_ms": (_i32, [_vp, C.POINTER(C.c_float)]),
     "dph_index_profile_scan_ms": (_i32, [_vp, _vp, _i32]),
     "dph_index_profile_count": (_i32, [_vp]),
+    "dph_index_last_stage_ms": (_i32, [_vp, _vp]),
     "dph_index_search": (_i32, [_vp, _vp, _i64, _i32, _vp, _vp, _i32]),
     "dph_index_search_partial": (_i32, [_vp, _vp, _i64, _i32, _vp, _vp, _vp]),
     "dph_index_coarse_local": (_i32, [_vp, _vp, _i64, _vp]),
diff --git a/densephrases_b200/csrc/common.cuh b/densephrases_b200/csrc/common.cuh
--- a/densephrases_b200/csrc/common.cuh
+++ b/densephrases_b200/csrc/common.cuh
@@ -113,6 +113,7 @@
     long long per;
     int total_units;
     int next_unit;
+    long long tail_lo;
 };
 #define DPH_QUAD_ITEM_Q 8
 struct __align__(16) DphUnit {
@@ -128,3 +129,4 @@
 };
 #define DPH_PAIR_SEG_MIN 128
 #define DPH_PAIR_UNITS_PER_CTA 16
+#define DPH_TAIL_EXTRA_UNITS(grid) (6 * (long long)(grid))
diff --git a/densephrases_b200/csrc/index.cu b/densephrases_b200/csrc/index.cu
--- a/densephrases_b200/csrc/index.cu
+++ b/densephrases_b200/csrc/index.cu
@@ -11,8 +11,8 @@
 static thread_local std::string g_err;
 void dph_set_error(const std::string& msg) { g_err = msg; }
 DPH_API const char* dph_last_error(void) { return g_err.c_str(); }
-DPH_API int dph_version(void) { return 103; }
-int g_dph_tune[8] = {1, 0, 0, 0, 0, 0, 0, 0};
+DPH_API int dph_version(void) { return 104; }
+int g_dph_tune[8] = {1, 0, 0, 1, 1, 0, 0, 0};
 DPH_API int dph_set_tuning(int knob, int value) {
     DPH_CHECK(knob >= 0 && knob < 8, "dph_set_tuning: unknown knob");
     g_dph_tune[knob] = value;
@@ -122,12 +122,15 @@
     for (void* p : ptrs) if (p) cudaFree(p);
     DevBuf* bufs[] = {&ix->xdev, &ix->xr, &ix->S, &ix->key, &ix->cd, &ix->lut_canon, &ix->lutmax, &ix->segs, &ix->wpre, &ix->qinfo,
                       &ix->cand, &ix->cand_off, &ix->cand_cnt, &ix->gthr, &ix->flags, &ix->work, &ix->Dp, &ix->Ip, &ix->Gp, &ix->Dh, &ix->Ih, &ix->eps, &ix->nseg, &ix->lutmin, &ix->lutmaxv, &ix->lutq, &ix->qparams, &ix->gdense,
-                      &ix->pl_cnt, &ix->pl_fill, &ix->pl_off, &ix->pl_blockpre, &ix->pl_entries, &ix->pl_unitpre, &ix->pl_units, &ix->pl_udesc, &ix->pairwork, &ix->csplit, &ix->xsplit, &ix->candkeys, &ix->cflags, &ix->selkeys, &ix->recbuf,
+                      &ix->pl_cnt, &ix->pl_fill, &ix->pl_off, &ix->pl_blockpre, &ix->pl_entries, &ix->pl_unitpre, &ix->pl_units, &ix->pl_udesc,
+                      &ix->pl_segl, &ix->pl_qextra, &ix->pairwork, &ix->csplit, &ix->xsplit, &ix->candkeys, &ix->cflags, &ix->selkeys, &ix->recbuf,
                       &ix->rb_ids, &ix->rb_out, &ix->rb_found, &ix->ws_q, &ix->ws_id, &ix->ws_out, &ix->ws_xq, &ix->enc_key, &ix->enc_cd,
                       &ix->enc_list, &ix->enc_codes};
     for (DevBuf* b : bufs) b->release();
     for (int i = 0; i < DPH_PROF_RING; i++) { if (ix->ev0[i]) cudaEventDestroy(ix->ev0[i]); if (ix->ev1[i]) cudaEventDestroy(ix->ev1[i]); }
     for (cudaEvent_t e : ix->aev) if (e) cudaEventDestroy(e);
+    for (cudaEvent_t e : ix->sev) if (e) cudaEventDestroy(e);
+    if (ix->side) { cudaStreamDestroy(ix->side); cudaEventDestroy(ix->side_fork); cudaEventDestroy(ix->side_join); }
     delete ix;
 }
 DPH_API int dph_index_set_stream(dph_index* ix, void* s) { ix->stream = (cudaStream_t)s; return 0; }
@@ -555,6 +558,8 @@
         for (int i = 0; i < DPH_PROF_RING; i++) { DPH_CUDA(cudaEventCreate(&ix->ev0[i])); DPH_CUDA(cudaEventCreate(&ix->ev1[i])); }
     if (on && !ix->aev[0])
         for (cudaEvent_t& e : ix->aev) DPH_CUDA(cudaEventCreate(&e));
+    if (on && !ix->sev[0])
+        for (cudaEvent_t& e : ix->sev) DPH_CUDA(cudaEventCreate(&e));
     ix->profile = on != 0;
     ix->prof_n = 0;
     return 0;
@@ -564,6 +569,12 @@
     int i = (int)((ix->prof_n - 1) % DPH_PROF_RING);
     DPH_CUDA(cudaEventSynchronize(ix->ev1[i]));
     DPH_CUDA(cudaEventElapsedTime(ms, ix->ev0[i], ix->ev1[i]));
+    return 0;
+}
+DPH_API int dph_index_last_stage_ms(dph_index* ix, float* ms_out) {
+    DPH_CHECK(ix->sev[0] && ix->prof_n > 0, "no profiled search");
+    DPH_CUDA(cudaEventSynchronize(ix->sev[7]));
+    for (int i = 0; i < 7; i++) DPH_CUDA(cudaEventElapsedTime(ms_out + i, ix->sev[i], ix->sev[i + 1]));
     return 0;
 }
 DPH_API int dph_index_profile_scan_ms(dph_index* ix, float* ms_out, int max_out) {
@@ -625,7 +636,9 @@
     const bool pair = group > 1;
     const int keep_fast = group == 4 ? keep_quad : (group == 2 ? keep_pair : keep_single);
     const size_t item_q = group == 4 ? DPH_QUAD_ITEM_Q : 2;
-    DPH_TRY(ix->cand.ensure(((size_t)(2 * grid + 2 * n + 2) + (pair ? (size_t)(n * nprobe + item_q * DPH_PAIR_UNITS_PER_CTA * grid + 2 * n + 16) : 0)) * keep_max * 8));
+    const size_t tail_units = group == 4 ? (size_t)DPH_TAIL_EXTRA_UNITS(grid) : 0;
+    DPH_TRY(ix->cand.ensure(((size_t)(2 * grid + 2 * n + 2) +
+                             (pair ? (size_t)(n * nprobe + item_q * (DPH_PAIR_UNITS_PER_CTA * grid + tail_units) + 2 * n + 16) : 0)) * keep_max * 8));
     DPH_TRY(ix->cand_off.ensure((size_t)(n + 1) * 8));
     DPH_TRY(ix->cand_cnt.ensure((size_t)n * 4));
     DPH_TRY(ix->gthr.ensure((size_t)n * 4));
@@ -643,8 +656,13 @@
         DPH_TRY(ix->pl_blockpre.ensure((size_t)(ix->nlist + 1) * 8));
         DPH_TRY(ix->pl_entries.ensure((size_t)n * nprobe * 4));
         DPH_TRY(ix->pl_unitpre.ensure((size_t)(ix->nlist + 1) * 4));
-        DPH_TRY(ix->pl_units.ensure((size_t)(n * nprobe + DPH_PAIR_UNITS_PER_CTA * grid + 16) * 8));
-        if (group == 4) DPH_TRY(ix->pl_udesc.ensure((size_t)(n * nprobe + DPH_PAIR_UNITS_PER_CTA * grid + 16) * sizeof(DphUnit)));
+        const size_t max_units = (size_t)(n * nprobe + DPH_PAIR_UNITS_PER_CTA * grid + 16) + tail_units;
+        DPH_TRY(ix->pl_units.ensure(max_units * 8));
+        if (group == 4) {
+            DPH_TRY(ix->pl_udesc.ensure(max_units * sizeof(DphUnit)));
+            DPH_TRY(ix->pl_segl.ensure((size_t)ix->nlist * 4));
+            DPH_TRY(ix->pl_qextra.ensure((size_t)n * 4));
+        }
         DPH_TRY(ix->pairwork.ensure(sizeof(DphPairWork)));
     }
     ix->last_n = n;
@@ -663,8 +681,29 @@
         DPH_TRY(dph_launch_coarse_select(ix->S.as<float>(), n, nl, nprobe, nullptr, nullptr, st, keys64, (unsigned)ix->list_lo));
         return 0;
     }
+    const bool stages = ix->profile && ix->sev[0] && stage != 3 && ix->scan_mode != DPH_SCAN_EXACT;
+    auto mark = [&](int i) { return stages ? cudaEventRecord(ix->sev[i], st) : cudaSuccess; };
+    const bool side = pair && g_dph_tune[4] != 0 && stage != 3 && ix->scan_mode != DPH_SCAN_EXACT;
+    if (side && !ix->side) {
+        DPH_CUDA(cudaStreamCreateWithFlags(&ix->side, cudaStreamNonBlocking));
+        DPH_CUDA(cudaEventCreateWithFlags(&ix->side_fork, cudaEventDisableTiming));
+        DPH_CUDA(cudaEventCreateWithFlags(&ix->side_join, cudaEventDisableTiming));
+    }
+    auto launch_lut = [&](cudaStream_t s) {
+        return dph_launch_lut(ix->xr.as<float>(), n, ix->pq, ix->lut_canon.as<float>(), ix->lutmax.as<float>(), ix->lutmin.as<float>(),
+                              ix->lutmaxv.as<float>(), pair ? ix->lutq.p : nullptr, pair ? ix->qparams.as<float2>() : nullptr, s, group);
+    };
+    DPH_CUDA(mark(0));
+    if (stage == 0 || stage == 3)
+        DPH_TRY(dph_launch_sgemm_nt_seq(x_dev, n, ix->A, ix->d, ix->d, ix->xr.as<float>(), st));
+    DPH_CUDA(mark(1));
+    if (side) {
+        DPH_CUDA(cudaEventRecord(ix->side_fork, st));
+        DPH_CUDA(cudaStreamWaitEvent(ix->side, ix->side_fork, 0));
+        DPH_TRY(launch_lut(ix->side));
+        DPH_CUDA(cudaEventRecord(ix->side_join, ix->side));
+    }
     if (stage == 0 || stage == 3) {
-        DPH_TRY(dph_launch_sgemm_nt_seq(x_dev, n, ix->A, ix->d, ix->d, ix->xr.as<float>(), st));
         int rc = ix->coarse_tc ? dph_coarse_tc(ix, n, 0, ix->nlist, nprobe, nullptr, ix->key.as<int32_t>(), ix->cd.as<float>(), st) : 1;
         if (rc > 1) return rc;
         if (rc == 1) {
@@ -674,19 +713,23 @@
         }
         if (stage == 3) return 0;
     }
-    DPH_TRY(dph_launch_lut(ix->xr.as<float>(), n, ix->pq, ix->lut_canon.as<float>(), ix->lutmax.as<float>(),
-                           ix->lutmin.as<float>(), ix->lutmaxv.as<float>(), pair ? ix->lutq.p : nullptr,
-                           pair ? ix->qparams.as<float2>() : nullptr, st, group));
+    DPH_CUDA(mark(2));
+    if (!side) DPH_TRY(launch_lut(st));
+    DPH_CUDA(mark(3));
     if (ix->scan_mode != DPH_SCAN_EXACT) {
-        DPH_TRY(dph_launch_plan(ix, n, k, keep_fast, grid, nullptr, st, group));
+        DPH_TRY(dph_launch_plan(ix, n, k, keep_fast, grid, nullptr, st, group, side ? ix->side_join : nullptr));
+        DPH_CUDA(mark(4));
         if (ix->profile) DPH_CUDA(cudaEventRecord(ix->ev0[ix->prof_n % DPH_PROF_RING], st));
         if (pair) DPH_TRY(dph_launch_scan_pair(ix, n, keep_fast, grid, st, group));
         else DPH_TRY(dph_launch_scan(ix, n, k, keep_fast, DPH_SCAN_FAST, grid, st));
         if (ix->profile) { DPH_CUDA(cudaEventRecord(ix->ev1[ix->prof_n % DPH_PROF_RING], st)); ix->prof_n++; }
+        DPH_CUDA(mark(5));
         DPH_TRY(dph_launch_merge(ix, n, k, DPH_SCAN_FAST, nullptr, D, I, G, st));
+        DPH_CUDA(mark(6));
         DPH_TRY(dph_launch_plan(ix, n, k, k, grid, ix->flags.as<int32_t>(), st, 1));
         DPH_TRY(dph_launch_scan(ix, n, k, k, DPH_SCAN_EXACT, grid, st));
         DPH_TRY(dph_launch_merge(ix, n, k, DPH_SCAN_EXACT, ix->flags.as<int32_t>(), D, I, G, st));
+        DPH_CUDA(mark(7));
     } else {
         DPH_CUDA(cudaMemsetAsync(ix->flags.p, 0, (size_t)n * 4, st));
         DPH_TRY(dph_launch_plan(ix, n, k, k, grid, nullptr, st, 1));
diff --git a/densephrases_b200/csrc/index_internal.cuh b/densephrases_b200/csrc/index_internal.cuh
--- a/densephrases_b200/csrc/index_internal.cuh
+++ b/densephrases_b200/csrc/index_internal.cuh
@@ -3,6 +3,7 @@
 #include "../../include/dph_b200.h"
 #include <algorithm>
 #include <string.h>
+#include <utility>
 #include <vector>
 
 #define DPH_SCAN_THREADS 512
@@ -59,7 +60,8 @@
 
     DevBuf xdev, xr, S, key, cd, lut_canon, lutmax, segs, wpre, qinfo, cand, cand_off, cand_cnt, gthr, flags,
         work, Dp, Ip, Gp, Dh, Ih, eps, nseg,
-        lutmin, lutmaxv, lutq, qparams, gdense, pl_cnt, pl_fill, pl_off, pl_blockpre, pl_entries, pl_unitpre, pl_units, pl_udesc, pairwork,
+        lutmin, lutmaxv, lutq, qparams, gdense, pl_cnt, pl_fill, pl_off, pl_blockpre, pl_entries, pl_unitpre, pl_units, pl_udesc, pl_segl,
+        pl_qextra, pairwork,
         csplit, xsplit, candkeys, cflags, selkeys, recbuf,
         rb_ids, rb_out, rb_found, ws_q, ws_id, ws_out, ws_xq,
         enc_key, enc_cd, enc_list, enc_codes;
@@ -71,6 +73,9 @@
     bool profile = false;
     cudaEvent_t ev0[DPH_PROF_RING] = {}, ev1[DPH_PROF_RING] = {};
     int64_t prof_n = 0;
+    cudaEvent_t sev[8] = {};
+    cudaStream_t side = nullptr;
+    cudaEvent_t side_fork = nullptr, side_join = nullptr;
     cudaEvent_t aev[6] = {};
     float add_ms[4] = {};
     float remove_ms[3] = {};
@@ -78,6 +83,18 @@
     int64_t remove_tmp_peak = 0;
     int64_t blk_cap = -1;
 };
+
+__device__ __forceinline__ void dph_grid_wait() { asm volatile("griddepcontrol.wait;" ::: "memory"); }
+template <typename... KArgs, typename... Args>
+inline cudaError_t dph_launch_pdl(bool pdl, void (*kernel)(KArgs...), dim3 grid, dim3 block, size_t smem, cudaStream_t st, Args&&... args) {
+    cudaLaunchConfig_t cfg = {};
+    cfg.gridDim = grid; cfg.blockDim = block; cfg.dynamicSmemBytes = smem; cfg.stream = st;
+    cudaLaunchAttribute at[1];
+    at[0].id = cudaLaunchAttributeProgrammaticStreamSerialization;
+    at[0].val.programmaticStreamSerializationAllowed = 1;
+    cfg.attrs = at; cfg.numAttrs = pdl ? 1 : 0;
+    return cudaLaunchKernelEx(&cfg, kernel, std::forward<Args>(args)...);
+}
 
 __device__ __forceinline__ long long list_of_block(const long long* blk_off, long long lo, long long hi, long long blk) {
     while (hi - lo > 1) { long long mid = (lo + hi) >> 1; if (blk_off[mid] <= blk) lo = mid; else hi = mid; }
@@ -145,7 +162,8 @@
                             unsigned long long* keys64 = nullptr);
 int dph_launch_lut(const float* xr, int64_t n, const float* pq, float* lut_canon, float* lutmax, float* lutmin, float* lutmaxv,
                    void* lutq, float2* qparams, cudaStream_t st, int group);
-int dph_launch_plan(dph_index* ix, int64_t n, int k, int keep, int grid, const int32_t* only_flagged, cudaStream_t st, int group);
+int dph_launch_plan(dph_index* ix, int64_t n, int k, int keep, int grid, const int32_t* only_flagged, cudaStream_t st, int group,
+                    cudaEvent_t lut_ready = nullptr);
 int dph_launch_scan_pair(dph_index* ix, int64_t n, int keep, int grid, cudaStream_t st, int group);
 int dph_launch_scan(dph_index* ix, int64_t n, int k, int keep, int mode, int grid, cudaStream_t st);
 int dph_launch_merge(dph_index* ix, int64_t n, int k, int mode, const int32_t* only_flagged, float* D, int64_t* I,
diff --git a/densephrases_b200/csrc/prep.cu b/densephrases_b200/csrc/prep.cu
--- a/densephrases_b200/csrc/prep.cu
+++ b/densephrases_b200/csrc/prep.cu
@@ -617,6 +617,7 @@
     const float2* qparams;
 };
 __global__ void __launch_bounds__(256) plan_segs_kernel(PlanArgs a) {
+    dph_grid_wait();
     const int lane = threadIdx.x & 31;
     const long long q = (long long)blockIdx.x * 8 + (threadIdx.x >> 5);
     if (q >= a.n) return;
@@ -678,8 +679,10 @@
     const unsigned* qblocks; long long n; int keep; int grid;
     long long* qpre; long long* cand_off; int* cand_cnt; unsigned* gthr; DphWork* work;
     const DphPairWork* pairwork; const int* nseg;
+    const int* qextra;
 };
 __global__ void __launch_bounds__(1024) plan_scan_kernel(PlanScanArgs a) {
+    dph_grid_wait();
     __shared__ long long wsum[32];
     __shared__ long long carry, total;
     const int tid = threadIdx.x, lane = tid & 31, warp = tid >> 5;
@@ -718,6 +721,7 @@
                 long long parts = qb / per + 2;
                 if (a.pairwork) parts = (long long)a.nseg[q] + qb / per + 1;
                 else if (parts > a.grid) parts = a.grid;
+                if (a.qextra) parts += a.qextra[q];
                 v = parts * a.keep;
             }
         }
@@ -749,7 +753,15 @@
     int gsz;
     DphUnit* udesc;
     const long long* blk_off; const float* cd; const unsigned* gdense; const float2* qparams;
+    int tail;
+    int* segl;
+    int* qextra;
 };
+__device__ __forceinline__ long long tail_seg_len(long long nb, long long segb, long long left, int grid) {
+    const long long ub = nb < segb ? nb : segb, f = left <= grid ? 4 : 2;
+    const long long s = (ub + f - 1) / f;
+    return s > DPH_PAIR_SEG_MIN ? s : DPH_PAIR_SEG_MIN;
+}
 __global__ void pair_count_kernel(PairPlanArgs a) {
     const long long i = (long long)blockIdx.x * blockDim.x + threadIdx.x;
     if (i >= a.nq_probes) return;
@@ -757,10 +769,13 @@
     if (l >= a.list_lo && l < a.list_hi && a.list_len[l] > 0) atomicAdd(&a.cnt[l], 1);
 }
 __global__ void __launch_bounds__(1024) pair_scan_kernel(PairPlanArgs a) {
+    dph_grid_wait();
     __shared__ long long wsa[32], wsb[32];
     __shared__ long long ca, cb;
     const int tid = threadIdx.x, lane = tid & 31, warp = tid >> 5;
     if (tid == 0) { ca = 0; cb = 0; }
+    if (a.tail)
+        for (long long q = tid; q < a.nq_probes / a.nprobe; q += 1024) a.qextra[q] = 0;
     __syncthreads();
     for (long long base = a.list_lo; base < a.list_hi; base += 1024) {
         const long long l = base + tid;
@@ -789,7 +804,7 @@
         }
         __syncthreads();
         const long long ea = ca + wsa[warp] + ia - va, eb = cb + wsb[warp] + ib - vb;
-        if (l < a.list_hi) { a.off[l] = (int)ea; a.blockpre[l] = eb; }
+        if (l < a.list_hi) { a.off[l] = (int)ea; a.blockpre[l] = eb; a.fill[l] = 0; }
         __syncthreads();
         if (tid == 1023) { ca = ea + va; cb = eb + vb; }
         __syncthreads();
@@ -830,15 +845,56 @@
         if (tid == 1023) ca = ea + va;
         __syncthreads();
     }
-    if (tid == 0) { a.work->total_units = (int)ca; a.work->next_unit = 0; }
+    __shared__ long long tail_lo_s;
+    const long long U = ca;
+    if (tid == 0) {
+        long long lo = a.list_hi;
+        if (a.tail) {
+            long long hi = a.list_hi;
+            lo = a.list_lo;
+            while (lo < hi) { const long long mid = (lo + hi) >> 1; if (U - a.unitpre[mid] <= 2ll * a.grid) hi = mid; else lo = mid + 1; }
+        }
+        tail_lo_s = lo; a.work->tail_lo = lo;
+        cb = lo < a.list_hi ? a.unitpre[lo] : U;
+    }
+    __syncthreads();
+    for (long long base = tail_lo_s; base < a.list_hi; base += 1024) {
+        const long long l = base + tid;
+        long long va = 0;
+        if (l < a.list_hi) {
+            const long long nb = (a.list_len[l] + 31) >> 5;
+            const long long sl = tail_seg_len(nb, segb, U - a.unitpre[l], a.grid);
+            va = (long long)((a.cnt[l] + a.gsz - 1) / a.gsz) * ((nb + sl - 1) / sl);
+            a.segl[l] = (int)sl;
+        }
+        long long ia = va;
+#pragma unroll
+        for (int off = 1; off < 32; off <<= 1) { long long t1 = __shfl_up_sync(0xffffffffu, ia, off); if (lane >= off) ia += t1; }
+        if (lane == 31) wsa[warp] = ia;
+        __syncthreads();
+        if (warp == 0) {
+            long long w1 = wsa[lane], i1 = w1;
+#pragma unroll
+            for (int off = 1; off < 32; off <<= 1) { long long t1 = __shfl_up_sync(0xffffffffu, i1, off); if (lane >= off) i1 += t1; }
+            wsa[lane] = i1 - w1;
+        }
+        __syncthreads();
+        const long long ea = cb + wsa[warp] + ia - va;
+        if (l < a.list_hi) a.unitpre[l] = (int)ea;
+        __syncthreads();
+        if (tid == 1023) cb = ea + va;
+        __syncthreads();
+    }
+    if (tid == 0) { a.work->total_units = (int)cb; a.work->next_unit = 0; }
 }
 __global__ void pair_units_kernel(PairPlanArgs a) {
+    dph_grid_wait();
     const long long l = a.list_lo + (long long)blockIdx.x * blockDim.x + threadIdx.x;
     if (l >= a.list_hi) return;
     const int cnt = a.cnt[l];
     const int items = (cnt + a.gsz - 1) / a.gsz;
     if (items == 0) return;
-    const long long segb = a.work->per, nb = (a.list_len[l] + 31) >> 5;
+    const long long segb = l >= a.work->tail_lo ? (long long)a.segl[l] : a.work->per, nb = (a.list_len[l] + 31) >> 5;
     const int nsegs = (int)((nb + segb - 1) / segb);
     const long long u0 = a.unitpre[l];
     for (int it = 0; it < items; it++) {
@@ -868,17 +924,26 @@
     }
 }
 __global__ void pair_fill_kernel(PairPlanArgs a) {
+    dph_grid_wait();
     const long long i = (long long)blockIdx.x * blockDim.x + threadIdx.x;
     if (i >= a.nq_probes) return;
     const int l = a.key[i];
     if (l >= a.list_lo && l < a.list_hi && a.list_len[l] > 0) {
         const int pos = a.off[l] + atomicAdd(&a.fill[l], 1);
         a.entries[pos] = (unsigned)((i / a.nprobe) << 10) | (unsigned)(i % a.nprobe);
-    }
-}
-
-int dph_launch_plan(dph_index* ix, int64_t n, int k, int keep, int grid, const int32_t* only_flagged, cudaStream_t st, int group) {
+        if (l >= a.work->tail_lo) {
+            const long long nb = (a.list_len[l] + 31) >> 5, segb = a.work->per, sl = a.segl[l];
+            const int extra = (int)((nb + sl - 1) / sl - (nb + segb - 1) / segb);
+            if (extra > 0) atomicAdd(&a.qextra[i / a.nprobe], extra);
+        }
+    }
+}
+
+int dph_launch_plan(dph_index* ix, int64_t n, int k, int keep, int grid, const int32_t* only_flagged, cudaStream_t st, int group,
+                    cudaEvent_t lut_ready) {
     const bool pair = group > 1;
+    const bool tail = group == 4 && g_dph_tune[3] != 0;
+    const bool pdl = g_dph_tune[4] != 0;
     (void)k;
     if (n == 0) return 0;
     PlanArgs a;
@@ -886,10 +951,8 @@
     a.list_lo = ix->list_lo; a.list_hi = ix->list_hi; a.nprobe = ix->nprobe; a.n = n; a.only_flagged = only_flagged;
     a.lutmax = ix->lutmax.as<float>(); a.segs = ix->segs.as<DphSeg>(); a.qblocks = ix->qinfo.as<unsigned>(); a.nseg = ix->nseg.as<int>(); a.eps = ix->eps.as<float>();
     a.gdense = pair ? ix->gdense.as<unsigned>() : nullptr; a.qparams = pair ? ix->qparams.as<float2>() : nullptr;
-    plan_segs_kernel<<<(unsigned)((n + 7) / 8), 256, 0, st>>>(a);
-    DPH_CUDA(cudaGetLastError());
+    PairPlanArgs p;
     if (pair) {
-        PairPlanArgs p;
         p.key = ix->key.as<int>(); p.nq_probes = n * ix->nprobe; p.nprobe = ix->nprobe; p.list_len = ix->list_len; p.list_lo = ix->list_lo;
         p.list_hi = ix->list_hi; p.nlist = ix->nlist; p.grid = grid; p.cnt = ix->pl_cnt.as<int>(); p.fill = ix->pl_fill.as<int>();
         p.off = ix->pl_off.as<int>(); p.blockpre = ix->pl_blockpre.as<long long>(); p.entries = ix->pl_entries.as<unsigned>();
@@ -897,22 +960,24 @@
         p.gsz = group == 4 ? DPH_QUAD_ITEM_Q : group;
         p.udesc = group == 4 ? ix->pl_udesc.as<DphUnit>() : nullptr;
         p.blk_off = (const long long*)ix->blk_off; p.cd = ix->cd.as<float>(); p.gdense = ix->gdense.as<unsigned>(); p.qparams = ix->qparams.as<float2>();
+        p.tail = tail ? 1 : 0; p.segl = ix->pl_segl.as<int>(); p.qextra = ix->pl_qextra.as<int>();
         DPH_CUDA(cudaMemsetAsync(p.cnt, 0, (size_t)ix->nlist * 4, st));
-        DPH_CUDA(cudaMemsetAsync(p.fill, 0, (size_t)ix->nlist * 4, st));
         const unsigned nb = (unsigned)((p.nq_probes + 255) / 256);
         pair_count_kernel<<<nb, 256, 0, st>>>(p);
-        pair_scan_kernel<<<1, 1024, 0, st>>>(p);
-        pair_fill_kernel<<<nb, 256, 0, st>>>(p);
-        if (ix->list_hi > ix->list_lo) pair_units_kernel<<<(unsigned)((ix->list_hi - ix->list_lo + 255) / 256), 256, 0, st>>>(p);
-        DPH_CUDA(cudaGetLastError());
-    }
+        DPH_CUDA(dph_launch_pdl(pdl, pair_scan_kernel, 1, 1024, 0, st, p));
+        DPH_CUDA(dph_launch_pdl(pdl, pair_fill_kernel, nb, 256, 0, st, p));
+    }
+    if (lut_ready) DPH_CUDA(cudaStreamWaitEvent(st, lut_ready, 0));
+    DPH_CUDA(dph_launch_pdl(pdl && !lut_ready, plan_segs_kernel, (unsigned)((n + 7) / 8), 256, 0, st, a));
+    if (pair && ix->list_hi > ix->list_lo)
+        DPH_CUDA(dph_launch_pdl(pdl, pair_units_kernel, (unsigned)((ix->list_hi - ix->list_lo + 255) / 256), 256, 0, st, p));
     PlanScanArgs b;
+    b.qextra = tail ? ix->pl_qextra.as<int>() : nullptr;
     b.pairwork = pair ? ix->pairwork.as<DphPairWork>() : nullptr; b.nseg = ix->nseg.as<int>();
     b.qblocks = ix->qinfo.as<unsigned>(); b.n = n; b.keep = keep; b.grid = grid; b.qpre = ix->wpre.as<long long>();
     b.cand_off = ix->cand_off.as<long long>(); b.cand_cnt = ix->cand_cnt.as<int>(); b.gthr = ix->gthr.as<unsigned>();
     b.work = ix->work.as<DphWork>();
-    plan_scan_kernel<<<1, 1024, 0, st>>>(b);
-    DPH_CUDA(cudaGetLastError());
+    DPH_CUDA(dph_launch_pdl(pdl, plan_scan_kernel, 1, 1024, 0, st, b));
     return 0;
 }
 
diff --git a/densephrases_b200/csrc/scan.cu b/densephrases_b200/csrc/scan.cu
--- a/densephrases_b200/csrc/scan.cu
+++ b/densephrases_b200/csrc/scan.cu
@@ -92,6 +92,7 @@
 
 template <int MODE>
 __global__ void __launch_bounds__(NT, 1) scan_kernel(ScanArgs a) {
+    dph_grid_wait();
     unsigned char* const smem = dph_smem;
     constexpr int LUT_BYTES = (MODE == DPH_SCAN_FAST) ? SMEM_LUT_FAST : SMEM_LUT_EXACT;
     ScanShared* sh = reinterpret_cast<ScanShared*>(smem + LUT_BYTES);
@@ -525,6 +526,7 @@
 
 #ifdef DPH_SCAN_PHASES
 __device__ unsigned long long g_quad_phase_ns[4];
+__device__ unsigned long long g_quad_cta_ns_sum, g_quad_cta_ns_max;
 __device__ unsigned g_quad_phase_ctas;
 __device__ __forceinline__ unsigned long long globaltimer_ns() { unsigned long long t; asm volatile("mov.u64 %0, %globaltimer;" : "=l"(t)); return t; }
 #define QPH_MARK(i) do { if (threadIdx.x == 0) { const unsigned long long t_ = globaltimer_ns(); ph[i] += t_ - ph_t; ph_t = t_; } } while (0)
@@ -612,6 +614,7 @@
 
 template <int IMADL>
 __global__ void __launch_bounds__(QNT, 1) scan_quad_kernel(PairScanArgs a) {
+    dph_grid_wait();
     unsigned char* const smem = dph_smem;
     QuadShared* sh = reinterpret_cast<QuadShared*>(smem + SMEM_QUAD_TABLES);
     const int tid = threadIdx.x, lane = tid & 31, warp = tid >> 5;
@@ -630,6 +633,7 @@
     unsigned long long ph[4] = {0ull, 0ull, 0ull, 0ull}, ph_t = 0ull;
 #ifdef DPH_SCAN_PHASES
     if (tid == 0) ph_t = globaltimer_ns();
+    const unsigned long long ph_start = ph_t;
 #endif
 
     if (tid == 0) sh->unit = atomicAdd(a.next_unit, 1);
@@ -727,14 +731,19 @@
     }
 #ifdef DPH_SCAN_PHASES
     if (tid == 0) {
+        const unsigned long long cta_ns = globaltimer_ns() - ph_start;
         for (int i = 0; i < 4; i++) atomicAdd(&g_quad_phase_ns[i], ph[i]);
+        atomicAdd(&g_quad_cta_ns_sum, cta_ns);
+        atomicMax(&g_quad_cta_ns_max, cta_ns);
         __threadfence();
         if (atomicAdd(&g_quad_phase_ctas, 1u) == gridDim.x - 1) {
             __threadfence();
             unsigned long long v[4];
             for (int i = 0; i < 4; i++) { v[i] = atomicExch(&g_quad_phase_ns[i], 0ull); }
-            printf("scan_quad_kernel phases (ms, summed over %u CTAs): table build %.3f, scan rounds %.3f, compaction barriers %.3f, publish %.3f\n",
-                   gridDim.x, v[0] * 1e-6, v[1] * 1e-6, v[2] * 1e-6, v[3] * 1e-6);
+            const double mean = atomicExch(&g_quad_cta_ns_sum, 0ull) * 1e-6 / gridDim.x, mx = atomicExch(&g_quad_cta_ns_max, 0ull) * 1e-6;
+            printf("scan_quad_kernel phases (ms, summed over %u CTAs): table build %.3f, scan rounds %.3f, compaction barriers %.3f, publish %.3f; "
+                   "CTA time mean %.3f, max %.3f, tail %.3f\n",
+                   gridDim.x, v[0] * 1e-6, v[1] * 1e-6, v[2] * 1e-6, v[3] * 1e-6, mean, mx, mx - mean);
             g_quad_phase_ctas = 0;
         }
     }
@@ -774,11 +783,9 @@
     a.lut_canon = ix->lut_canon.as<float>(); a.gthr = ix->gthr.as<unsigned>();
     a.cand = ix->cand.as<unsigned long long>(); a.cand_off = ix->cand_off.as<long long>(); a.cand_cnt = ix->cand_cnt.as<int>();
     a.n = n; a.nprobe = ix->nprobe; a.keep = keep;
-    if (mode == DPH_SCAN_FAST)
-        scan_kernel<DPH_SCAN_FAST><<<grid, NT, SMEM_LUT_FAST + sizeof(ScanShared), st>>>(a);
-    else
-        scan_kernel<DPH_SCAN_EXACT><<<grid, NT, SMEM_LUT_EXACT + sizeof(ScanShared), st>>>(a);
-    DPH_CUDA(cudaGetLastError());
+    const bool pdl = g_dph_tune[4] != 0;
+    if (mode == DPH_SCAN_FAST) DPH_CUDA(dph_launch_pdl(pdl, scan_kernel<DPH_SCAN_FAST>, grid, NT, SMEM_LUT_FAST + sizeof(ScanShared), st, a));
+    else DPH_CUDA(dph_launch_pdl(pdl, scan_kernel<DPH_SCAN_EXACT>, grid, NT, SMEM_LUT_EXACT + sizeof(ScanShared), st, a));
     return 0;
 }
 
@@ -795,11 +802,12 @@
     a.udesc = ix->pl_udesc.as<DphUnit>(); a.one = 1u;
     if (group == 4) {
         const size_t sm = SMEM_QUAD_TABLES + sizeof(QuadShared);
+        const bool pdl = g_dph_tune[4] != 0;
         switch (g_dph_tune[0]) {
-            case 0: scan_quad_kernel<0><<<grid, QNT, sm, st>>>(a); break;
-            case 2: scan_quad_kernel<2><<<grid, QNT, sm, st>>>(a); break;
-            case 3: scan_quad_kernel<3><<<grid, QNT, sm, st>>>(a); break;
-            default: scan_quad_kernel<1><<<grid, QNT, sm, st>>>(a); break;
+            case 0: DPH_CUDA(dph_launch_pdl(pdl, scan_quad_kernel<0>, grid, QNT, sm, st, a)); break;
+            case 2: DPH_CUDA(dph_launch_pdl(pdl, scan_quad_kernel<2>, grid, QNT, sm, st, a)); break;
+            case 3: DPH_CUDA(dph_launch_pdl(pdl, scan_quad_kernel<3>, grid, QNT, sm, st, a)); break;
+            default: DPH_CUDA(dph_launch_pdl(pdl, scan_quad_kernel<1>, grid, QNT, sm, st, a)); break;
         }
     }
     else scan_pair_kernel<<<grid, NT, SMEM_LUT_FAST + sizeof(PairShared), st>>>(a);
@@ -821,6 +829,7 @@
 }
 
 __global__ void __launch_bounds__(256) merge_kernel(MergeArgs a) {
+    dph_grid_wait();
     __shared__ SelectScratch sc;
     __shared__ unsigned long long surv[DPH_SURV_CAP];
     __shared__ unsigned sgs[DPH_MAX_NPROBE];
@@ -911,8 +920,7 @@
     a.gthr = ix->gthr.as<unsigned>(); a.eps = ix->eps.as<float>(); a.segs = ix->segs.as<DphSeg>(); a.nseg = ix->nseg.as<int>(); a.nprobe = ix->nprobe; a.k = k; a.mode = mode;
     a.codes = ix->codes; a.lut_canon = ix->lut_canon.as<float>(); a.ids = (const long long*)ix->ids; a.list_start = (const long long*)ix->list_start;
     a.D = D; a.I = (long long*)I; a.G = G; a.flags = ix->flags.as<int>(); a.only_flagged = only_flagged;
-    merge_kernel<<<(unsigned)n, 256, 0, st>>>(a);
-    DPH_CUDA(cudaGetLastError());
+    DPH_CUDA(dph_launch_pdl(g_dph_tune[4] != 0, merge_kernel, (unsigned)n, 256, 0, st, a));
     return 0;
 }
 
diff --git a/densephrases_b200/ivfpq.py b/densephrases_b200/ivfpq.py
--- a/densephrases_b200/ivfpq.py
+++ b/densephrases_b200/ivfpq.py
@@ -315,6 +315,11 @@
         L.check(L.lib().dph_index_last_scan_ms(self._h, C.byref(ms)))
         return ms.value
 
+    def last_stage_ms(self):
+        out = np.zeros(7, dtype=np.float32)
+        L.check(L.lib().dph_index_last_stage_ms(self._h, _np_ptr(out)))
+        return out
+
     def profile_scan_ms(self):
         n = L.lib().dph_index_profile_count(self._h)
         out = np.zeros(max(n, 1), dtype=np.float32)
diff --git a/include/dph_b200.h b/include/dph_b200.h
--- a/include/dph_b200.h
+++ b/include/dph_b200.h
@@ -66,6 +66,7 @@
 int dph_index_last_scan_ms(dph_index* ix, float* ms);
 int dph_index_profile_scan_ms(dph_index* ix, float* ms_out, int max_out);
 int dph_index_profile_count(const dph_index* ix);
+int dph_index_last_stage_ms(dph_index* ix, float* ms_out );
 
 int dph_index_search(dph_index* ix, const float* x, int64_t n, int k, float* D, int64_t* I, int mem);
 int dph_index_search_partial(dph_index* ix, const float* x_dev, int64_t n, int k, float* D_dev, int64_t* I_dev,
```

Result: faster. 14840 (median of 6 runs) (+4.7%).
